# Acellera/moleculekit

Hardware: AMD Instinct MI355X
Metric: Mvoxel-channels/s (64^3 grid, 8 ch) (higher is better)
Workload: dtype f32; 1 GPU; cfg2: BASELINE.json configs[1]; channels=8, atoms_per_gpu=12800000, periodic=False, tile_k=0, pipelined_steps=True, topology_reuse=False, device=AMD Radeon Graphics, arch=gfx950:sramecc+:xnack-, compute_units=256

## Files before the change

### include/mkamd_voxel.h

```cpp
#ifndef MKAMD_VOXEL_H
#define MKAMD_VOXEL_H

#include <stddef.h>
#include <stdint.h>

#ifdef __cplusplus
extern "C" {
#endif

#define MKAMD_OK 0
#define MKAMD_EINVAL 1
#define MKAMD_EHIP 2
#define MKAMD_ENODEV 3
#define MKAMD_EOVERFLOW 4
#define MKAMD_EBOX 5
#define MKAMD_ENOMEM 6

typedef struct mkamd_ctx mkamd_ctx;

const char* mkamd_version(void);
const char* mkamd_last_error(void);
int mkamd_device_count(int* count);

int mkamd_ctx_create(int device, mkamd_ctx** ctx);
// ... 2 lines not shown
int mkamd_ctx_abandon_pending(mkamd_ctx* ctx);
int mkamd_ctx_synchronize(mkamd_ctx* ctx);
int mkamd_ctx_poll_errors(mkamd_ctx* ctx);
int mkamd_ctx_device_info(mkamd_ctx* ctx, char* name, size_t len, int* compute_units,
                          uint64_t* hbm_bytes, char* arch, size_t arch_len);
int mkamd_ctx_set_tile_k(mkamd_ctx* ctx, int k);
int mkamd_ctx_set_force_general(mkamd_ctx* ctx, int on);
int mkamd_ctx_set_lds_tier(mkamd_ctx* ctx, int tier);
int mkamd_ctx_set_prepass_mode(mkamd_ctx* ctx, int mode);
int mkamd_ctx_set_fine_cells(mkamd_ctx* ctx, int on);
int mkamd_ctx_set_direct_binning(mkamd_ctx* ctx, int mode);
int mkamd_ctx_set_value_tolerance(mkamd_ctx* ctx, double eps);
int mkamd_ctx_set_tile_team(mkamd_ctx* ctx, int mode);
int mkamd_ctx_set_tile_items(mkamd_ctx* ctx, int mode);
int mkamd_ctx_set_exact_redo(mkamd_ctx* ctx, int mode);
int mkamd_ctx_set_pipelining(mkamd_ctx* ctx, int on);
int mkamd_ctx_promise_inputs(mkamd_ctx* ctx, void* hip_event);
int mkamd_ctx_withdraw_promise(mkamd_ctx* ctx);
int mkamd_ctx_pipelined_calls(mkamd_ctx* ctx, int64_t* n);
int mkamd_ctx_last_tile_kernel(mkamd_ctx* ctx, char* name, size_t name_cap);
int mkamd_ctx_enable_kernel_timing(mkamd_ctx* ctx, int enable);
int mkamd_ctx_read_kernel_timing(mkamd_ctx* ctx, double* total_ms, int64_t* launches);
int mkamd_clock_probe_dev(mkamd_ctx* ctx, void* hip_stream, int64_t microseconds, uint64_t* d_ticks2);

int mkamd_calculate_occupancy(mkamd_ctx* ctx, const double* centers, int64_t n_centers,
                              const float* coords, int64_t n_atoms, const double* sigmas,
                              int32_t n_channels, double* results);

int mkamd_calculate_occupancy_cpu(const double* centers, int64_t n_centers, const float* coords, int64_t n_atoms,
                                  const double* sigmas, int32_t n_channels, double* results);
int mkamd_calculate_occupancy_cpu_threads(const double* centers, int64_t n_centers, const float* coords, int64_t n_atoms,
                                          const double* sigmas, int32_t n_channels, double* results, int32_t n_threads);

int mkamd_occupancy_centers_host(mkamd_ctx* ctx, const double* centers, int64_t n_centers,
                                 const float* coords, int64_t n_atoms, const void* sigmas,
                                 int sigmas_are_f64, int32_t n_channels, const double* box,
                                 float* features);
int mkamd_occupancy_centers_dev(mkamd_ctx* ctx, const double* d_centers, int64_t n_centers,
                                const float* d_coords, int64_t n_atoms, const void* d_sigmas,
                                int sigmas_are_f64, int32_t n_channels, const double* box_host,
                                float* d_features);

int mkamd_voxelize_lattice_host(mkamd_ctx* ctx, int32_t n_items, const float* coords,
                                const int64_t* atom_offsets, const void* sigmas,
                                int sigmas_are_f64, int32_t n_channels, const double* origins,
                                const int32_t* nvoxels, double voxelsize, const float* box,
                                int32_t max_images_per_atom, float* features);
int mkamd_voxelize_lattice_host_f64(mkamd_ctx* ctx, int32_t n_items, const float* coords,
                                    const int64_t* atom_offsets, const void* sigmas,
                                    int sigmas_are_f64, int32_t n_channels, const double* origins,
                                    const int32_t* nvoxels, double voxelsize, const float* box,
                                    int32_t max_images_per_atom, double* features);
int mkamd_voxelize_lattice_host_begin(mkamd_ctx* ctx, int32_t n_items, const float* coords,
                                      const int64_t* atom_offsets, const void* sigmas,
                                      int sigmas_are_f64, int32_t n_channels, const double* origins,
                                      const int32_t* nvoxels, double voxelsize, const float* box,
                                      int32_t max_images_per_atom);
int mkamd_voxelize_lattice_host_end(mkamd_ctx* ctx, float* features, double* features_f64, uint64_t n_values);
int mkamd_voxelize_lattice_dev(mkamd_ctx* ctx, int32_t n_items, const float* d_coords,
                               const int64_t* d_atom_offsets, int64_t total_atoms,
                               const void* d_sigmas, int sigmas_are_f64, int32_t n_channels,
                               const double* d_origins, const int32_t* nvoxels, double voxelsize,
                               const float* d_box, int32_t max_images_per_atom,
                               float* d_features);

int mkamd_voxelize_lattice_aug_dev(mkamd_ctx* ctx, int32_t n_items, const float* d_coords,
                                   const int64_t* d_atom_offsets, int64_t total_atoms,
                                   const void* d_sigmas, int sigmas_are_f64, int32_t n_channels,
                                   const double* d_origins, const int32_t* nvoxels, double voxelsize,
                                   const float* d_box, int32_t max_images_per_atom,
                                   const double* d_affine, float* d_features);

typedef struct mkamd_topology mkamd_topology;
int mkamd_topology_create_dev(mkamd_ctx* ctx, const void* d_sigmas, int sigmas_are_f64, int64_t n_atoms, int32_t n_channels,
                              double voxelsize, mkamd_topology** topology);
int mkamd_topology_create_host(mkamd_ctx* ctx, const void* sigmas, int sigmas_are_f64, int64_t n_atoms, int32_t n_channels,
                               double voxelsize, mkamd_topology** topology);
int mkamd_topology_destroy(mkamd_ctx* ctx, mkamd_topology* topology);
int mkamd_topology_info(const mkamd_topology* topology, int64_t* n_atoms, int32_t* n_channels, double* voxelsize, int32_t* has_wide_sigmas);
int mkamd_voxelize_lattice_topo_dev(mkamd_ctx* ctx, int32_t n_items, const float* d_coords, const int64_t* d_atom_offsets,
                                    int64_t total_atoms, const mkamd_topology* topology, const double* d_origins,
                                    const int32_t* nvoxels, double voxelsize, const float* d_box, int32_t max_images_per_atom,
                                    const double* d_affine, float* d_features);

int mkamd_grid_centers_host(mkamd_ctx* ctx, const double* bb_min, const int32_t* nvoxels,
                            double voxelsize, double* centers);
int mkamd_grid_centers_dev(mkamd_ctx* ctx, const double* bb_min, const int32_t* nvoxels,
                           double voxelsize, double* d_centers);

int mkamd_prefault(void* buffer, uint64_t bytes);
int mkamd_copy_to_host(mkamd_ctx* ctx, void* host_dst, const void* device_src, uint64_t bytes);
int mkamd_copy_dev(mkamd_ctx* ctx, void* device_dst, const void* device_src, uint64_t bytes);
int mkamd_frames_to_items_dev(mkamd_ctx* ctx, void* hip_stream, const float* d_src, int64_t rows, int64_t src_pitch,
                              int64_t n_frames, float scale, float* d_dst);

int mkamd_lattice_from_centers(const double* centers, int64_t n_centers, double* bb_min, int32_t* nvoxels, double* voxelsize);

#ifdef __cplusplus
}
#endif
#endif
```

### moleculekit_amd/_lib.py

```python
from __future__ import annotations

import ctypes
import os
import threading

import numpy as np

_HERE = os.path.dirname(os.path.abspath(__file__))
LIB_PATH = os.environ.get("MKAMD_LIB", os.path.join(_HERE, "csrc", "libmkamd.so"))

MKAMD_OK, MKAMD_EINVAL, MKAMD_EHIP, MKAMD_ENODEV, MKAMD_EOVERFLOW, MKAMD_EBOX, MKAMD_ENOMEM = range(7)

_c_int, _c_i32, _c_i64, _c_dbl, _vp = ctypes.c_int, ctypes.c_int32, ctypes.c_int64, ctypes.c_double, ctypes.c_void_p

SIGNATURES = {
    "mkamd_version": (ctypes.c_char_p, []),
    "mkamd_last_error": (ctypes.c_char_p, []),
    "mkamd_device_count": (_c_int, [ctypes.POINTER(_c_int)]),
    "mkamd_ctx_create": (_c_int, [_c_int, ctypes.POINTER(_vp)]),
    "mkamd_ctx_destroy": (_c_int, [_vp]),
    "mkamd_ctx_set_stream": (_c_int, [_vp, _vp]),
    "mkamd_ctx_synchronize": (_c_int, [_vp]),
    "mkamd_ctx_abandon_pending": (_c_int, [_vp]),
    "mkamd_ctx_poll_errors": (_c_int, [_vp]),
    "mkamd_ctx_device_info": (_c_int, [_vp, ctypes.c_char_p, ctypes.c_size_t, ctypes.POINTER(_c_int),
                                       ctypes.POINTER(ctypes.c_uint64), ctypes.c_char_p, ctypes.c_size_t]),
    "mkamd_ctx_set_tile_k": (_c_int, [_vp, _c_int]),
    "mkamd_ctx_set_force_general": (_c_int, [_vp, _c_int]),
    "mkamd_xtc_info": (_c_int, [ctypes.c_char_p, ctypes.POINTER(ctypes.c_int64), ctypes.POINTER(ctypes.c_int64)]),
    "mkamd_xtc_read": (_c_int, [ctypes.c_char_p, _vp, ctypes.c_int64, ctypes.c_int64, _vp, _vp, _vp, _vp, ctypes.c_int32]),
    "mkamd_xtc_chunk_desc": (_c_int, [ctypes.c_char_p, _vp, ctypes.c_int64, ctypes.c_int64, _vp, ctypes.POINTER(ctypes.c_int64),
                                      ctypes.POINTER(ctypes.c_int64), _vp, _vp, _vp]),
    "mkamd_xtc_copy_bytes": (_c_int, [ctypes.c_char_p, ctypes.c_int64, ctypes.c_int64, _vp, ctypes.c_int32]),
    "mkamd_xtc_byte_range": (_c_int, [ctypes.c_char_p, _vp, ctypes.c_int64, ctypes.c_int64, ctypes.POINTER(ctypes.c_int64), ctypes.POINTER(ctypes.c_int64)]),
    "mkamd_xtc_chunk_desc_mem": (_c_int, [ctypes.c_char_p, _vp, ctypes.c_int64, ctypes.c_int64, _vp, ctypes.c_int64, ctypes.c_int64, _vp,
                                          ctypes.POINTER(ctypes.c_int64), ctypes.POINTER(ctypes.c_int64), _vp, _vp, _vp]),
    "mkamd_xtc_decode_work_bytes": (ctypes.c_uint64, [ctypes.c_int64, ctypes.c_int64]),
    "mkamd_xtc_decode_dev": (_c_int, [_vp, _vp, _vp, _vp, ctypes.c_int64, ctypes.c_int64, ctypes.c_float, _vp, _vp, _vp, ctypes.c_uint64]),
    "mkamd_ctx_set_lds_tier": (_c_int, [_vp, _c_int]),
    "mkamd_ctx_set_prepass_mode": (_c_int, [_vp, _c_int]),
    "mkamd_ctx_set_pipelining": (_c_int, [_vp, _c_int]),
    "mkamd_ctx_promise_inputs": (_c_int, [_vp, _vp]),
    "mkamd_ctx_withdraw_promise": (_c_int, [_vp]),
    "mkamd_ctx_pipelined_calls": (_c_int, [_vp, ctypes.POINTER(_c_i64)]),
    "mkamd_ctx_last_tile_kernel": (_c_int, [_vp, ctypes.c_char_p, ctypes.c_size_t]),
    "mkamd_clock_probe_dev": (_c_int, [_vp, _vp, _c_i64, _vp]),
    "mkamd_frames_to_items_dev": (_c_int, [_vp, _vp, _vp, _c_i64, _c_i64, _c_i64, ctypes.c_float, _vp]),
    "mkamd_ctx_set_tile_team": (_c_int, [_vp, _c_int]),
    "mkamd_ctx_set_tile_items": (_c_int, [_vp, _c_int]),
    "mkamd_ctx_set_exact_redo": (_c_int, [_vp, _c_int]),
    "mkamd_ctx_set_fine_cells": (_c_int, [_vp, _c_int]),
    "mkamd_ctx_set_value_tolerance": (_c_int, [_vp, ctypes.c_double]),
    "mkamd_ctx_set_direct_binning": (_c_int, [_vp, _c_int]),
    "mkamd_ctx_enable_kernel_timing": (_c_int, [_vp, _c_int]),
    "mkamd_ctx_read_kernel_timing": (_c_int, [_vp, ctypes.POINTER(_c_dbl), ctypes.POINTER(_c_i64)]),
    "mkamd_calculate_occupancy": (_c_int, [_vp, _vp, _c_i64, _vp, _c_i64, _vp, _c_i32, _vp]),
    "mkamd_calculate_occupancy_cpu": (_c_int, [_vp, _c_i64, _vp, _c_i64, _vp, _c_i32, _vp]),
    "mkamd_calculate_occupancy_cpu_threads": (_c_int, [_vp, _c_i64, _vp, _c_i64, _vp, _c_i32, _vp, _c_i32]),
    "mkamd_occupancy_centers_host": (_c_int, [_vp, _vp, _c_i64, _vp, _c_i64, _vp, _c_int, _c_i32, _vp, _vp]),
    "mkamd_occupancy_centers_dev": (_c_int, [_vp, _vp, _c_i64, _vp, _c_i64, _vp, _c_int, _c_i32, _vp, _vp]),
    "mkamd_voxelize_lattice_host": (_c_int, [_vp, _c_i32, _vp, _vp, _vp, _c_int, _c_i32, _vp, _vp, _c_dbl,
                                             _vp, _c_i32, _vp]),
    "mkamd_voxelize_lattice_host_f64": (_c_int, [_vp, _c_i32, _vp, _vp, _vp, _c_int, _c_i32, _vp, _vp, _c_dbl,
                                                 _vp, _c_i32, _vp]),
    "mkamd_voxelize_lattice_host_begin": (_c_int, [_vp, _c_i32, _vp, _vp, _vp, _c_int, _c_i32, _vp, _vp, _c_dbl, _vp, _c_i32]),
    "mkamd_voxelize_lattice_host_end": (_c_int, [_vp, _vp, _vp, ctypes.c_uint64]),
    "mkamd_voxelize_lattice_dev": (_c_int, [_vp, _c_i32, _vp, _vp, _c_i64, _vp, _c_int, _c_i32, _vp, _vp,
                                            _c_dbl, _vp, _c_i32, _vp]),
    "mkamd_voxelize_lattice_aug_dev": (_c_int, [_vp, _c_i32, _vp, _vp, _c_i64, _vp, _c_int, _c_i32, _vp, _vp,
                                                _c_dbl, _vp, _c_i32, _vp, _vp]),
    "mkamd_topology_create_dev": (_c_int, [_vp, _vp, _c_int, _c_i64, _c_i32, _c_dbl, ctypes.POINTER(_vp)]),
    "mkamd_topology_create_host": (_c_int, [_vp, _vp, _c_int, _c_i64, _c_i32, _c_dbl, ctypes.POINTER(_vp)]),
    "mkamd_topology_destroy": (_c_int, [_vp, _vp]),
    "mkamd_topology_info": (_c_int, [_vp, ctypes.POINTER(_c_i64), ctypes.POINTER(_c_i32), ctypes.POINTER(_c_dbl), ctypes.POINTER(_c_i32)]),
    "mkamd_voxelize_lattice_topo_dev": (_c_int, [_vp, _c_i32, _vp, _vp, _c_i64, _vp, _vp, _vp, _c_dbl, _vp, _c_i32, _vp, _vp]),
    "mkamd_grid_centers_host": (_c_int, [_vp, _vp, _vp, _c_dbl, _vp]),
    "mkamd_grid_centers_dev": (_c_int, [_vp, _vp, _vp, _c_dbl, _vp]),
    "mkamd_lattice_from_centers": (_c_int, [_vp, ctypes.c_int64, _vp, _vp, _vp]),
    "mkamd_prefault": (_c_int, [_vp, ctypes.c_uint64]),
    "mkamd_copy_to_host": (_c_int, [_vp, _vp, _vp, ctypes.c_uint64]),
    "mkamd_copy_dev": (_c_int, [_vp, _vp, _vp, ctypes.c_uint64]),
    "mkamd_dist_count_pairs": (_c_i64, [_c_i64, _c_i64, _c_int]),
    "mkamd_dist_trajectory_host": (_c_int, [_vp, _vp, _c_i64, _c_i64, _vp, _vp, _c_i64, _vp, _c_i64, _vp, _c_int, _c_int,
                                            _c_int, _vp]),
    "mkamd_dist_trajectory_dev": (_c_int, [_vp, _vp, _c_i64, _vp, _vp, _c_i64, _vp, _c_i64, _vp, _c_int, _c_int, _c_int, _vp]),
    "mkamd_contacts_trajectory_host": (_c_int, [_vp, _vp, _c_i64, _c_i64, _vp, _vp, _c_i64, _vp, _c_i64, _vp, _c_int, _c_int,
                                                ctypes.c_float, _vp, ctypes.POINTER(_vp)]),
    "mkamd_dist_reduction_host": (_c_int, [_vp, _vp, _c_i64, _c_i64, _vp, _vp, _vp, _c_i64, _vp, _vp, _c_i64, _vp, _vp,
                                           _c_int, _c_int, _c_int, _vp, _c_int, _c_int, _vp]),
    "mkamd_contacts_trajectory_dev": (_c_int, [_vp, _vp, _c_i64, _vp, _vp, _c_i64, _vp, _c_i64, _vp, _c_int, _c_int, ctypes.c_float, _vp,
                                               ctypes.POINTER(_vp)]),
    "mkamd_dist_reduction_dev": (_c_int, [_vp, _vp, _c_i64, _c_i64, _vp, _vp, _vp, _c_i64, _c_i64, _vp, _vp, _c_i64, _vp, _vp,
                                          _c_int, _c_int, _c_int, _vp, _c_int, _c_int, _vp]),
    "mkamd_cdist_dev": (_c_int, [_vp, _vp, _c_i64, _vp, _c_i64, _c_i32, _vp]),
    "mkamd_pdist_dev": (_c_int, [_vp, _vp, _c_i64, _c_i32, _vp]),
    "mkamd_ctx_set_reduction_block": (_c_int, [_vp, _c_int]),
    "mkamd_selftest_sqrt": (_c_int, [_vp, ctypes.POINTER(ctypes.c_uint64), ctypes.POINTER(ctypes.c_uint32)]),
    "mkamd_ctx_set_dist_kernels": (_c_int, [_vp, _c_int]),
    "mkamd_ctx_last_dist_kernel": (_c_int, [_vp, ctypes.c_char_p, ctypes.c_size_t]),
    "mkamd_cdist_host": (_c_int, [_vp, _vp, _c_i64, _vp, _c_i64, _c_i32, _vp]),
    "mkamd_pdist_host": (_c_int, [_vp, _vp, _c_i64, _c_i32, _vp]),
    "mkamd_align_transforms_dev": (_c_int, [_vp, _vp, _c_i64, _c_i64, _vp, _c_i64, _c_i64, _vp, _vp, _c_i64, _vp, _c_i64, _c_i64, _c_int,
                                            _vp, _vp]),
    "mkamd_align_apply_dev": (_c_int, [_vp, _vp, _c_i64, _vp, _c_i64, _vp, _vp]),
    "mkamd_align_rmsd_dev": (_c_int, [_vp, _vp, _c_i64, _c_i64, _vp, _c_i64, _c_i64, _vp, _vp, _c_i64, _vp, _c_i64, _c_i64, _c_int, _vp,
                                      _vp]),
    "mkamd_align_host": (_c_int, [_vp, _vp, _c_i64, _c_i64, _vp, _c_i64, _c_i64, _vp, _vp, _c_i64, _vp, _c_i64, _c_i64, _c_int]),
    "mkamd_sasa_dev": (_c_int, [_vp, _vp, _c_i64, _c_i64, _vp, _c_i32, _vp, _vp, ctypes.c_float, _vp, _c_i64]),
    "mkamd_sasa_host": (_c_int, [_vp, _vp, _c_i64, _c_i64, _vp, _c_i64, _vp, _c_i32, _vp, _vp, ctypes.c_float, _vp, _c_i64]),
    "mkamd_shell_counts_dev": (_c_int, [_vp, _vp, _c_i64, _c_i64, _vp, _vp, _c_i64, _vp, _c_i64, _vp, _c_int, _c_int, _vp, _c_i64, _vp]),
    "mkamd_shell_counts_host": (_c_int, [_vp, _vp, _c_i64, _c_i64, _vp, _vp, _c_i64, _vp, _c_i64, _vp, _c_int, _c_int, _vp, _c_i64, _vp]),
    "mkamd_dihedrals_dev": (_c_int, [_vp, _vp, _c_i64, _c_i64, _vp, _c_i64, _vp, _c_i64, _c_int, _vp]),
    "mkamd_dihedrals_host": (_c_int, [_vp, _vp, _c_i64, _c_i64, _vp, _c_i64, _vp, _c_i64, _c_int, _vp]),
    "mkamd_group_moments_dev": (_c_int, [_vp, _vp, _c_i64, _c_i64, _vp, _vp, _vp, _vp, _c_i64, _c_i64, _c_i64, _c_int, _vp]),
    "mkamd_fluctuation_dev": (_c_int, [_vp, _vp, _c_i64, _c_i64, _vp, _vp, _c_i64, _vp, _c_i64, _c_i64, _vp, _vp]),
    "mkamd_group_moments_host": (_c_int, [_vp, _vp, _c_i64, _c_i64, _vp, _vp, _c_i64, _vp, _vp, _vp, _c_i64, _c_int, _vp]),
    "mkamd_fluctuation_host": (_c_int, [_vp, _vp, _c_i64, _c_i64, _vp, _vp, _c_i64, _vp, _c_i64, _vp, _c_i64, _vp, _vp]),
}

_lib = None
_lock = threading.Lock()


def load() -> ctypes.CDLL:
    global _lib
    with _lock:
        if _lib is None:
            if not os.path.exists(LIB_PATH):
                raise RuntimeError(
                    f"moleculekit_amd: HIP library not found at {LIB_PATH}. Build it with "
                    f"`python -c 'import __graft_entry__ as g; g.build()'` (hipcc --offload-arch=gfx950). "
                    f"There is no CPU fallback.")
            if os.environ.get("MKAMD_NO_TORCH_PRELOAD", "0") != "1":
                try:
                    import torch
                except Exception:
                    pass
            L = ctypes.CDLL(LIB_PATH)
            for name, (res, args) in SIGNATURES.items():
                fn = getattr(L, name)
                fn.restype, fn.argtypes = res, args
            if b"DIAGNOSTICS" in L.mkamd_version() and os.environ.get("MKAMD_ALLOW_DIAGNOSTICS", "0") != "1":
                raise RuntimeError(f"moleculekit_amd: {LIB_PATH} is a DIAGNOSTICS build ({L.mkamd_version().decode()}); "
                                   f"set MKAMD_ALLOW_DIAGNOSTICS=1 to load it for timing experiments")
            _lib = L
    return _lib


_host_lib = None


def load_host() -> ctypes.CDLL:
    global _host_lib
    with _lock:
        if _host_lib is None:
            from . import _build
            L = ctypes.CDLL(_build.build_host())
            for name in ("mkamd_calculate_occupancy_cpu", "mkamd_calculate_occupancy_cpu_threads"):
# ... 135 lines not shown
        _check(load().mkamd_ctx_last_tile_kernel(self._h, buf, 128))
        return buf.value.decode()

    def selftest_sqrt(self):
        n, first = ctypes.c_uint64(0), ctypes.c_uint32(0)
        _check(load().mkamd_selftest_sqrt(self._h, ctypes.byref(n), ctypes.byref(first)))
        return int(n.value), int(first.value)

    def set_dist_kernels(self, avoid_mask: int = 0):
        _check(load().mkamd_ctx_set_dist_kernels(self._h, int(avoid_mask)))

    def set_reduction_block(self, block: int = 0):
        _check(load().mkamd_ctx_set_reduction_block(self._h, int(block)))

    def last_dist_kernel(self) -> str:
        buf = ctypes.create_string_buffer(128)
        _check(load().mkamd_ctx_last_dist_kernel(self._h, buf, 128))
        return buf.value.decode()

    def pipelined_calls(self) -> int:
        n = _c_i64(0)
        _check(load().mkamd_ctx_pipelined_calls(self._h, ctypes.byref(n)))
        return int(n.value)

    def enable_kernel_timing(self, on=True):
        _check(load().mkamd_ctx_enable_kernel_timing(self._h, int(bool(on))))

    def read_kernel_timing(self):
        ms, n = _c_dbl(0.0), _c_i64(0)
        _check(load().mkamd_ctx_read_kernel_timing(self._h, ctypes.byref(ms), ctypes.byref(n)))
        return ms.value, n.value

    def device_info(self):
        name = ctypes.create_string_buffer(256)
        arch = ctypes.create_string_buffer(256)
        cus, mem = _c_int(0), ctypes.c_uint64(0)
        _check(load().mkamd_ctx_device_info(self._h, name, 256, ctypes.byref(cus), ctypes.byref(mem), arch, 256))
        return dict(name=name.value.decode(), arch=arch.value.decode(), compute_units=cus.value,
                    hbm_bytes=int(mem.value))

    def calculate_occupancy(self, centers, coords, sigmas, results):
        V, N, C = centers.shape[0], coords.shape[0], sigmas.shape[1]
        _check(load().mkamd_calculate_occupancy(self._h, _ptr(centers), V, _ptr(coords), N, _ptr(sigmas), C,
                                                _ptr(results)))

    def occupancy_centers_host(self, centers, coords, sigmas, sig_f64, C, box, out):
        _check(load().mkamd_occupancy_centers_host(self._h, _ptr(centers), centers.shape[0], _ptr(coords),
                                                   coords.shape[0], _ptr(sigmas), int(sig_f64), C, _ptr(box),
                                                   _ptr(out)))

    def occupancy_centers_dev(self, d_centers, V, d_coords, N, d_sigmas, sig_f64, C, box_host, d_out):
        _check(load().mkamd_occupancy_centers_dev(self._h, _ptr(d_centers), V, _ptr(d_coords), N, _ptr(d_sigmas),
                                                  int(sig_f64), C, _ptr(box_host), _ptr(d_out)))

    def voxelize_lattice_host(self, B, coords, offsets, sigmas, sig_f64, C, origins, nvox, voxelsize, box,
                              max_images, out):
        fn = load().mkamd_voxelize_lattice_host_f64 if out.dtype == np.float64 else load().mkamd_voxelize_lattice_host
        _check(fn(self._h, B, _ptr(coords), _ptr(offsets), _ptr(sigmas),
                                                  int(sig_f64), C, _ptr(origins), _ptr(nvox), float(voxelsize),
                                                  _ptr(box), int(max_images), _ptr(out)))

    def voxelize_lattice_host_begin(self, B, coords, offsets, sigmas, sig_f64, C, origins, nvox, voxelsize, box, max_images):
        _check(load().mkamd_voxelize_lattice_host_begin(self._h, B, _ptr(coords), _ptr(offsets), _ptr(sigmas), int(sig_f64), C,
                                                        _ptr(origins), _ptr(nvox), float(voxelsize), _ptr(box), int(max_images)))
        self._begun = getattr(self, "_begun", 0) + 1
        return self._begun

    def voxelize_lattice_host_end(self, out):
        if not isinstance(out, np.ndarray) or out.dtype not in (np.float32, np.float64) or not out.flags["C_CONTIGUOUS"]:
            raise ValueError("out must be a C-contiguous float32 or float64 ndarray")
        if out.dtype == np.float64:
            _check(load().mkamd_voxelize_lattice_host_end(self._h, None, _ptr(out), int(out.size)))
        else:
            _check(load().mkamd_voxelize_lattice_host_end(self._h, _ptr(out), None, int(out.size)))

    def voxelize_lattice_dev(self, B, d_coords, d_offsets, total_atoms, d_sigmas, sig_f64, C, d_origins, nvox,
                             voxelsize, d_box, max_images, d_out, d_affine=None):
        _check(load().mkamd_voxelize_lattice_aug_dev(self._h, B, _ptr(d_coords), _ptr(d_offsets), int(total_atoms),
                                                     _ptr(d_sigmas), int(sig_f64), C, _ptr(d_origins), _ptr(nvox),
                                                     float(voxelsize), _ptr(d_box), int(max_images), _ptr(d_affine),
                                                     _ptr(d_out)))

    def voxelize_lattice_topo_dev(self, B, d_coords, d_offsets, total_atoms, topology, d_origins, nvox, voxelsize, d_box, max_images, d_out,
                                  d_affine=None):
        _check(load().mkamd_voxelize_lattice_topo_dev(self._h, B, _ptr(d_coords), _ptr(d_offsets), int(total_atoms), topology._h,
                                                      _ptr(d_origins), _ptr(nvox), float(voxelsize), _ptr(d_box), int(max_images),
                                                      _ptr(d_affine), _ptr(d_out)))

    def grid_centers_host(self, bb_min, nvox, voxelsize, out):
        _check(load().mkamd_grid_centers_host(self._h, _ptr(bb_min), _ptr(nvox), float(voxelsize), _ptr(out)))

    def dist_trajectory_host(self, coords, box, sel1, sel2, chains, selfdist, pbc, squared, out):
        N, _, F = coords.shape
        _check(load().mkamd_dist_trajectory_host(self._h, _ptr(coords), N, F, _ptr(box), _ptr(sel1), sel1.shape[0], _ptr(sel2),
                                                 sel2.shape[0], _ptr(chains), int(selfdist), int(pbc), int(squared), _ptr(out)))

    def dist_trajectory_dev(self, d_coords, F, d_box, d_sel1, n1, d_sel2, n2, d_chains, selfdist, pbc, squared, d_out):
        _check(load().mkamd_dist_trajectory_dev(self._h, _ptr(d_coords), F, _ptr(d_box), _ptr(d_sel1), n1, _ptr(d_sel2), n2,
                                                _ptr(d_chains), int(selfdist), int(pbc), int(squared), _ptr(d_out)))

    def contacts_trajectory_host(self, coords, box, sel1, sel2, chains, selfdist, pbc, threshold):
        N, _, F = coords.shape
        offs = np.zeros(F + 1, dtype=np.int64)
        ptr = _vp(None)
        _check(load().mkamd_contacts_trajectory_host(self._h, _ptr(coords), N, F, _ptr(box), _ptr(sel1), sel1.shape[0], _ptr(sel2),
                                                     sel2.shape[0], _ptr(chains), int(selfdist), int(pbc), float(threshold),
                                                     _ptr(offs), ctypes.byref(ptr)))
        n = int(offs[-1])
        if n == 0 or not ptr.value:
            return offs, np.zeros((0, 2), dtype=np.uint32)
        buf = (ctypes.c_uint32 * (2 * n)).from_address(ptr.value)
        return offs, np.frombuffer(buf, dtype=np.uint32).reshape(n, 2).copy()

    def dist_reduction_host(self, coords, box, g1a, g1o, g2a, g2o, ch1, ch2, selfdist, pairs, pbc, masses, r1, r2, out):
        N, _, F = coords.shape
        _check(load().mkamd_dist_reduction_host(self._h, _ptr(coords), N, F, _ptr(box), _ptr(g1a), _ptr(g1o), g1o.shape[0] - 1,
                                                _ptr(g2a), _ptr(g2o), g2o.shape[0] - 1, _ptr(ch1), _ptr(ch2), int(selfdist),
                                                int(pairs), int(pbc), _ptr(masses), int(r1), int(r2), _ptr(out)))

    def contacts_trajectory_dev(self, d_coords, F, d_box, d_sel1, n1, d_sel2, n2, d_chains, selfdist, pbc, threshold):
        offs = np.zeros(F + 1, dtype=np.int64)
        ptr = _vp(None)
        _check(load().mkamd_contacts_trajectory_dev(self._h, _ptr(d_coords), F, _ptr(d_box), _ptr(d_sel1), n1, _ptr(d_sel2), n2, _ptr(d_chains),
                                                    int(selfdist), int(pbc), float(threshold), _ptr(offs), ctypes.byref(ptr)))
        return offs, int(ptr.value or 0), int(offs[-1])

    def dist_reduction_dev(self, d_coords, N, F, d_box, d_g1a, d_g1o, ng1, n_g1_atoms, d_g2a, d_g2o, ng2, d_ch1, d_ch2, selfdist, pairs, pbc,
                           d_masses, r1, r2, d_out):
        _check(load().mkamd_dist_reduction_dev(self._h, _ptr(d_coords), N, F, _ptr(d_box), _ptr(d_g1a), _ptr(d_g1o), ng1, n_g1_atoms, _ptr(d_g2a),
                                               _ptr(d_g2o), ng2, _ptr(d_ch1), _ptr(d_ch2), int(selfdist), int(pairs), int(pbc), _ptr(d_masses),
                                               int(r1), int(r2), _ptr(d_out)))

    def cdist_dev(self, d_c1, n1, d_c2, n2, dim, d_out):
        _check(load().mkamd_cdist_dev(self._h, _ptr(d_c1), n1, _ptr(d_c2), n2, dim, _ptr(d_out)))

    def pdist_dev(self, d_c, n, dim, d_out):
        _check(load().mkamd_pdist_dev(self._h, _ptr(d_c), n, dim, _ptr(d_out)))

    def cdist_host(self, c1, c2, out):
        _check(load().mkamd_cdist_host(self._h, _ptr(c1), c1.shape[0], _ptr(c2), c2.shape[0], c1.shape[1], _ptr(out)))

    def pdist_host(self, c, out):
        _check(load().mkamd_pdist_host(self._h, _ptr(c), c.shape[0], c.shape[1], _ptr(out)))

    def grid_centers_dev(self, bb_min, nvox, voxelsize, d_out):
        _check(load().mkamd_grid_centers_dev(self._h, _ptr(bb_min), _ptr(nvox), float(voxelsize), _ptr(d_out)))


class Topology:

    def __init__(self, ctx, sigmas, voxelsize):
        self._h = _vp(None)
        self._ctx = ctx
        h = _vp(None)
        if isinstance(sigmas, np.ndarray) or not hasattr(sigmas, "data_ptr"):
            sig = np.ascontiguousarray(sigmas)
            if sig.dtype not in (np.float32, np.float64):
                sig = sig.astype(np.float64)
            if sig.ndim != 2:
                raise ValueError("sigmas must be (natoms, nchannels)")
            _check(load().mkamd_topology_create_host(ctx._h, _ptr(sig), int(sig.dtype == np.float64), int(sig.shape[0]), int(sig.shape[1]),
                                                     float(voxelsize), ctypes.byref(h)))
            self.n_atoms, self.n_channels = int(sig.shape[0]), int(sig.shape[1])
        else:
            import torch
            if not (sigmas.is_cuda and sigmas.dim() == 2 and sigmas.is_contiguous() and sigmas.dtype in (torch.float32, torch.float64)):
                raise ValueError("sigmas must be a contiguous float32 / float64 CUDA tensor (natoms, nchannels)")
            ctx.set_stream(torch.cuda.current_stream(sigmas.device).cuda_stream)
            _check(load().mkamd_topology_create_dev(ctx._h, int(sigmas.data_ptr()), int(sigmas.dtype == torch.float64), int(sigmas.shape[0]),
                                                    int(sigmas.shape[1]), float(voxelsize), ctypes.byref(h)))
            self.n_atoms, self.n_channels = int(sigmas.shape[0]), int(sigmas.shape[1])
        self._h = h
        self.voxelsize = float(voxelsize)

    @property
    def has_wide_sigmas(self) -> bool:
        w = _c_i32(0)
        _check(load().mkamd_topology_info(self._h, None, None, None, ctypes.byref(w)))
        return bool(w.value)

    def close(self):
        if getattr(self, "_h", None) is not None and self._h.value:
            ctx = getattr(self, "_ctx", None)
            alive = ctx is not None and getattr(ctx, "_h", None) is not None and ctx._h.value
            load().mkamd_topology_destroy(ctx._h if alive else None, self._h)
            self._h = _vp(None)

    def __del__(self):
        try:
            self.close()
        except Exception:
            pass


_tls = threading.local()


def default_context(device: int | None = None) -> Context:
    if device is None:
        device = int(os.environ.get("MKAMD_DEVICE", os.environ.get("LOCAL_RANK", "0")))
        n = device_count()
        if n > 0:
            device %= n
    held = getattr(_tls, "contexts", None)
    if held is None or getattr(_tls, "pid", None) != os.getpid():
        if held:
            for c in held.values():
                c._h = _vp(None)
        held = _tls.contexts = {}
        _tls.pid = os.getpid()
    ctx = held.get(int(device))
    if ctx is None:
        ctx = held[int(device)] = Context(device)
    return ctx
```

### moleculekit_amd/batch.py

```python
from __future__ import annotations

import numpy as np

from . import _lib

CUTOFF = 5.0


def pack_items(coords_list, sigmas_list):
    ns = [int(np.asarray(c).shape[0]) for c in coords_list]
    offs = np.zeros(len(ns) + 1, dtype=np.int64)
    offs[1:] = np.cumsum(ns)
    if len(ns) == 0:
        return np.zeros((0, 3), np.float32), np.zeros((0, 1), np.float64), offs
    coords = np.concatenate([np.asarray(c, dtype=np.float32).reshape(-1, 3) for c in coords_list])
    sig = np.concatenate([np.asarray(s) for s in sigmas_list])
    return coords, sig, offs


def max_images_per_atom(box, nvoxels, voxelsize) -> int:
    box = np.asarray(box, dtype=np.float64).reshape(-1, 3)
    if box.size == 0:
        return 1
    if not np.all(box > 2 * CUTOFF):
# ... 41 lines not shown
    if dtype not in (np.dtype(np.float32), np.dtype(np.float64)):
        raise ValueError("dtype must be float32 or float64 (the library writes 4- or 8-byte floats into the result)")
    coords = np.ascontiguousarray(coords, dtype=np.float32).reshape(-1, 3)
    atom_offsets = np.ascontiguousarray(atom_offsets, dtype=np.int64)
    sigmas, sig64 = _sigma_array(sigmas)
    if sigmas.ndim != 2 or sigmas.shape[0] != coords.shape[0]:
        raise ValueError("sigmas must be (natoms, nchannels) matching coords")
    origins = np.ascontiguousarray(origins, dtype=np.float64).reshape(-1, 3)
    B = origins.shape[0]
    if atom_offsets.shape != (B + 1,) or (B >= 0 and atom_offsets[-1] != coords.shape[0]):
        raise ValueError("atom_offsets must have B+1 entries ending at the total atom count")
    nv = np.ascontiguousarray(nvoxels, dtype=np.int32).reshape(3)
    C = int(sigmas.shape[1])
    V = int(nv[0]) * int(nv[1]) * int(nv[2])
    bx = None if box is None else np.ascontiguousarray(box, dtype=np.float32).reshape(B, 3)
    ticket = ctx.voxelize_lattice_host_begin(B, coords, atom_offsets, sigmas, sig64, C, origins, nv, float(voxelsize), bx, 0)
    return _PendingHostCall(ctx, ticket, (B, V, C), dtype, (coords, atom_offsets, sigmas, origins, nv, bx))


def _abandon_host_call(ctx_ref, ticket):
    ctx = ctx_ref()
    if ctx is not None and getattr(ctx, "_begun", None) == ticket:
        try:
            ctx.abandon_pending()
        except Exception:
            pass


class _PendingHostCall:

    def __init__(self, ctx, ticket, shape, dtype, keep):
        import weakref
        self._ctx, self._shape, self._dtype, self._keep = ctx, shape, dtype, keep
        self._finalizer = weakref.finalize(self, _abandon_host_call, weakref.ref(ctx), ticket)

    def __call__(self):
        self._finalizer.detach()
        out = np.empty(self._shape, dtype=self._dtype)
        self._ctx.voxelize_lattice_host_end(out)
        return out

    def abandon(self):
        if self._finalizer.alive:
            self._finalizer()


def occupancy_centers(centers, coords, sigmas, box=None, ctx=None):
    ctx = ctx or _lib.default_context()
    centers = np.ascontiguousarray(centers, dtype=np.float64)
    coords = np.ascontiguousarray(coords, dtype=np.float32)
    sigmas, sig64 = _sigma_array(sigmas)
    if centers.ndim != 2 or centers.shape[1] != 3 or coords.ndim != 2 or coords.shape[1] != 3:
        raise ValueError("centers and coords must be (n, 3)")
    if sigmas.ndim != 2 or sigmas.shape[0] != coords.shape[0]:
        raise ValueError("sigmas must be (natoms, nchannels) matching coords")
    out = np.empty((centers.shape[0], sigmas.shape[1]), dtype=np.float32)
    bx = None if box is None else np.ascontiguousarray(box, dtype=np.float64).reshape(3)
    ctx.occupancy_centers_host(centers, coords, sigmas, sig64, int(sigmas.shape[1]), bx, out)
    return out


def grid_centers(bb_min, nvoxels, voxelsize, ctx=None):
    ctx = ctx or _lib.default_context()
    bb = np.ascontiguousarray(bb_min, dtype=np.float64).reshape(3)
    nv = np.ascontiguousarray(nvoxels, dtype=np.int32).reshape(3)
    out = np.empty((int(np.prod(nv.astype(np.int64))), 3), dtype=np.float64)
    ctx.grid_centers_host(bb, nv, float(voxelsize), out)
    return out


def rotation_affines(rotations, centers):
    from .util import rotationMatrix
    rotations = np.asarray(rotations, dtype=np.float64).reshape(-1, 3)
    centers = np.broadcast_to(np.asarray(centers, dtype=np.float64).reshape(-1, 3), rotations.shape)
    out = np.empty((rotations.shape[0], 12), dtype=np.float64)
    for b, (r, c) in enumerate(zip(rotations, centers)):
        m = rotationMatrix([0, 0, 1], r[2]) @ rotationMatrix([0, 1, 0], r[1]) @ rotationMatrix([1, 0, 0], r[0])
        out[b, :9] = m.ravel()
        out[b, 9:] = c - m @ c
    return out


def voxelize_lattice_torch(coords, atom_offsets, sigmas, origins, nvoxels, voxelsize, box=None,
                           max_images=1, out=None, ctx=None, channel_first=False, affine=None, topology=None):
    import torch

    dev = coords.device
    if dev.type != "cuda":
        raise RuntimeError("voxelize_lattice_torch needs CUDA/HIP tensors (there is no CPU path)")
    dev_index = dev.index if dev.index is not None else torch.cuda.current_device()
    if ctx is not None and ctx.device != dev_index:
        raise ValueError(f"ctx lives on GPU {ctx.device} but the tensors are on cuda:{dev_index} (kernels run on the context's device)")
    ctx = ctx or _lib.default_context(dev_index)
    if (sigmas is None) == (topology is None):
        ctx.withdraw_promise()
        raise ValueError("pass the sigmas or a topology (not both)")
    if not (coords.dtype == torch.float32 and coords.is_contiguous() and atom_offsets.dtype == torch.int64 and atom_offsets.is_contiguous()
            and (sigmas is None or (sigmas.dtype in (torch.float32, torch.float64) and sigmas.is_contiguous() and sigmas.dim() == 2))
            and origins.dtype == torch.float64 and origins.is_contiguous()):
        ctx.withdraw_promise()
        raise AssertionError("voxelize_lattice_torch: coords float32, atom_offsets int64, sigmas float32|float64 [n, C], origins float64, all contiguous")
    B = int(origins.shape[0])
    C = int(sigmas.shape[1]) if topology is None else topology.n_channels
    nv = np.ascontiguousarray(nvoxels, dtype=np.int32).reshape(3)
    V = int(np.prod(nv.astype(np.int64)))
    if out is None:
        out = torch.empty((B, V, C), dtype=torch.float32, device=dev)
    else:
        assert out.dtype == torch.float32 and out.is_contiguous() and out.numel() == B * V * C
    d_box = None
    if box is not None:
        assert box.dtype == torch.float32 and box.is_contiguous()
        d_box = box.data_ptr()
    d_aff = None
    if affine is not None:
        assert affine.dtype == torch.float64 and affine.is_contiguous() and tuple(affine.shape) == (B, 12)
        d_aff = affine.data_ptr()
    try:
        ctx.set_stream(torch.cuda.current_stream(dev).cuda_stream)
        if topology is not None:
            ctx.voxelize_lattice_topo_dev(B, coords.data_ptr(), atom_offsets.data_ptr(), int(coords.shape[0]), topology, origins.data_ptr(), nv,
                                          float(voxelsize), d_box, int(max_images), out.data_ptr(), d_aff)
        else:
            ctx.voxelize_lattice_dev(B, coords.data_ptr(), atom_offsets.data_ptr(), int(coords.shape[0]),
                                     sigmas.data_ptr(), sigmas.dtype == torch.float64, C, origins.data_ptr(), nv,
                                     float(voxelsize), d_box, int(max_images), out.data_ptr(), d_aff)
    except BaseException:
        ctx.withdraw_promise()
        raise
    out = out.view(B, V, C)
    if channel_first:
        return out.view(B, int(nv[0]), int(nv[1]), int(nv[2]), C).permute(0, 4, 1, 2, 3)
    return out


def getVoxelDescriptorsBatch(coords_list, channels_list, centers, boxsize, voxelsize=1, boxes=None, ctx=None):
    boxsize = np.array(boxsize, dtype=np.float64)
    centers = np.asarray(centers, dtype=np.float64).reshape(-1, 3)
    nvoxels = np.ceil(boxsize / voxelsize).astype(int)
    origins = centers - boxsize / 2
    coords, sig, offs = pack_items(coords_list, channels_list)
    feats = voxelize_lattice(coords, offs, sig, origins, nvoxels, voxelsize, box=boxes, ctx=ctx)
    return feats, origins, nvoxels.astype(np.int64)


def voxelizeTrajectory(coords, channels, center, boxsize, voxelsize=1, box=None, frames=None, ctx=None):
    coords = np.asarray(coords)
    if coords.ndim != 3 or coords.shape[1] != 3:
        raise ValueError("coords must be (natoms, 3, nframes)")
    fr = np.arange(coords.shape[2]) if frames is None else np.asarray(frames)
    F = len(fr)
    sig = np.asarray(channels)
    boxsize_a = np.array(boxsize, dtype=np.float64)
    nvoxels = np.ceil(boxsize_a / voxelsize).astype(int)
    origin = np.asarray(center, dtype=np.float64) - boxsize_a / 2
    V, C = int(np.prod(nvoxels.astype(np.int64))), int(sig.shape[1])
    out = np.empty((F, V, C), dtype=np.float32)
    if F == 0 or V == 0:
        return out, origin, nvoxels.astype(np.int64)
    try:
        import torch
    except ImportError:
        return _voxelizeTrajectory_packed(coords, channels, center, boxsize, voxelsize, box=box, frames=frames, ctx=ctx)
    cctx = ctx or _lib.default_context()
    _lib._check(_lib.load().mkamd_prefault(_lib._ptr(out), out.nbytes))
    chunk = int(max(1, min(F, (256 << 20) // max(V * C * 4, 1))))
    pos = 0
    lib = _lib.load()
    for idx, feats in iterVoxelizeTrajectory(coords, sig, center, boxsize, voxelsize, box=box, frames=frames, chunk=chunk,
                                             device=f"cuda:{cctx.device}", ctx=cctx):
        n = len(idx)
        feats = feats.contiguous()
        torch.cuda.current_stream(feats.device).synchronize()
        _lib._check(lib.mkamd_copy_to_host(cctx._h, out[pos:pos + n].ctypes.data, feats.data_ptr(), n * V * C * 4))
        pos += n
    return out, origin, nvoxels.astype(np.int64)


def _voxelizeTrajectory_packed(coords, channels, center, boxsize, voxelsize=1, box=None, frames=None, ctx=None):
    coords = np.asarray(coords, dtype=np.float32)
    if coords.ndim != 3 or coords.shape[1] != 3:
        raise ValueError("coords must be (natoms, 3, nframes)")
    fr = np.arange(coords.shape[2]) if frames is None else np.asarray(frames)
    F, N = len(fr), coords.shape[0]
    packed = np.ascontiguousarray(np.transpose(coords[:, :, fr], (2, 0, 1))).reshape(F * N, 3)
    sig = np.asarray(channels)
    sig_all = np.ascontiguousarray(np.broadcast_to(sig[None], (F,) + sig.shape)).reshape(F * N, sig.shape[1])
    offs = np.arange(F + 1, dtype=np.int64) * N
    boxsize = np.array(boxsize, dtype=np.float64)
    nvoxels = np.ceil(boxsize / voxelsize).astype(int)
    origin = np.asarray(center, dtype=np.float64) - boxsize / 2
    bx = None
    if box is not None:
        bx = np.ascontiguousarray(np.asarray(box, dtype=np.float32)[:, fr].T)
    feats = voxelize_lattice(packed, offs, sig_all, np.broadcast_to(origin, (F, 3)), nvoxels, voxelsize,
                             box=bx, ctx=ctx)
    return feats, origin, nvoxels.astype(np.int64)


def _chunk_images(box3n, nvoxels, voxelsize) -> int:
    return max_images_per_atom(np.ascontiguousarray(np.asarray(box3n).T), nvoxels, voxelsize)


USE_TOPOLOGY = True
_PINNED = {}
# ... 367 lines not shown
```

### moleculekit_amd/csrc/capi.hip

```cpp
#include "../../include/mkamd_voxel.h"
#include "../../include/mkamd_distance.h"
#include "../../include/mkamd_xtc.h"
#include "xtc_reader.h"
#include <atomic>
#include "pipeline.h"
#include "dist_pipeline.h"
#include "align_pipeline.h"
#include "sasa_pipeline.h"
#include "shell_pipeline.h"
#include "dihedral_pipeline.h"
#include "moments_pipeline.h"
#include "host_pack.h"
#include "xtc_gpu.h"
#include "cpu_occupancy.h"

#include <algorithm>
#include <cstring>
#include <string>
#include <utility>
#include <vector>

using namespace mkamd;

static thread_local char g_last_error[512] = "";
// ... 167 lines not shown
    {
        in_pipelined_prepass = false;
        auto await_promise = [&](hipStream_t s) {
            if (!promise_event) return;
            if (!sync_ok(hipStreamWaitEvent(s, promise_event, 0))) (void)hipEventSynchronize(promise_event);
        };
        if (!big_enough || !(pipelining || promise) || !side_stream || pipeline_broken) {
            await_promise(main_stream);
            have_pre_tile_event = false;
            return 0;
        }
        const int set = next_set;
        if (!have_pre_tile_event) {
            if (!sync_ok(hipEventRecord(ev_inputs, main_stream))) { await_promise(main_stream); return 0; }
            inputs_marker = ev_inputs;
        }
        if (!sync_ok(hipStreamWaitEvent(side_stream, inputs_marker, 0))) { await_promise(main_stream); return 0; }
        if (tile_pending[set] && !sync_ok(hipStreamWaitEvent(side_stream, tile_marker[set], 0))) { await_promise(main_stream); return 0; }
        if (promise_event && !sync_ok(hipStreamWaitEvent(side_stream, promise_event, 0))) { (void)hipEventSynchronize(promise_event); return 0; }
        next_set ^= 1;
        stream = side_stream;
        in_pipelined_prepass = true;
        ++n_pipelined;
        return set;
    }
    bool set_is_pipelined(int) const { return in_pipelined_prepass; }
    bool pipelining_possible() const { return (pipelining || promise) && side_stream && !pipeline_broken; }
    void prepass_done(int set)
    {
        if (!in_pipelined_prepass) return;
        stream = main_stream;
        if (sync_ok(hipEventRecord(ev_pre_done[set], side_stream)) && sync_ok(hipStreamWaitEvent(main_stream, ev_pre_done[set], 0)))
            have_pre_tile_event = true;
    }
    void tile_done(int set)
    {
        if (!side_stream) return;
        const bool piped = in_pipelined_prepass;
        in_pipelined_prepass = false;
        if (pipeline_broken || !piped) { last_hot_end = nullptr; return; }
        if (last_hot_end) { tile_marker[set] = last_hot_end; tile_pending[set] = true; }
        else if (sync_ok(hipEventRecord(ev_tile_done[set], main_stream))) { tile_marker[set] = ev_tile_done[set]; tile_pending[set] = true; }
        last_hot_end = nullptr;
    }
    int last_flavour = -1, last_K = 0, last_ecap = 0;
    void hot_begin(int flavour, int K, int ecap)
    {
        last_flavour = flavour; last_K = K; last_ecap = ecap;
        last_hot_end = nullptr;
        if (timing) {
            std::pair<hipEvent_t, hipEvent_t> ev;
            bool ok = true;
            if (!ev_free.empty()) { ev = ev_free.back(); ev_free.pop_back(); }
            else ok = hipEventCreate(&ev.first) == hipSuccess && hipEventCreate(&ev.second) == hipSuccess;
            if (ok && hipEventRecord(ev.first, stream) == hipSuccess) {
                cur0 = ev.first; cur1 = ev.second;
                if (in_pipelined_prepass) inputs_marker = cur0;
                return;
            }
            (void)hipGetLastError();
        }
        if (in_pipelined_prepass) {
            if (sync_ok(hipEventRecord(ev_inputs, main_stream))) inputs_marker = ev_inputs;
        }
    }
    void hot_end()
    {
        if (!timing || !cur0) return;
        if (hipEventRecord(cur1, stream) == hipSuccess) {
            ev_used.emplace_back(cur0, cur1);
            last_hot_end = cur1;
        } else {
            (void)hipGetLastError();
            ev_free.emplace_back(cur0, cur1);
        }
        cur0 = cur1 = nullptr;
    }
};

struct mkamd_topology {
    int device = 0;
    void* mem = nullptr;
    mkamd::TopologyDev dev;
};

static int check_ctx(mkamd_ctx* ctx, bool pending_ok = false)
{
    if (!ctx) return fail(MKAMD_EINVAL, "ctx is NULL");
    if (!pending_ok && ctx->pending.active)
        return fail(MKAMD_EINVAL, "a host call begun on this context (mkamd_voxelize_lattice_host_begin) has not been ended: call _end (or mkamd_ctx_abandon_pending) first");
    HIP_TRY(hipSetDevice(ctx->device));
    ctx->stream = ctx->main_stream;
    return 0;
}

static int collect_async_errors(mkamd_ctx* ctx)
{
    if (!ctx->bufs[WS_ERR]) return 0;
    if (ctx->err_mirrored && ctx->fb_host && ((volatile unsigned*)ctx->fb_host)[NTIER + 1] == 0u) return 0;
    int flag = 0;
    HIP_TRY(hipMemcpy(&flag, ctx->bufs[WS_ERR], sizeof(int), hipMemcpyDeviceToHost));
    if (flag == 0) return 0;
    HIP_TRY(hipMemset(ctx->bufs[WS_ERR], 0, sizeof(int)));
    if (flag & MK_ERR_TOPOLOGY) return fail(MKAMD_EINVAL, "a topology call was given an item that is not the topology's atom count long; results are incomplete");
    if (flag & MK_ERR_BAD_BOX) return fail(MKAMD_EBOX, "periodic box edges must be > 10 A (2 x cutoff)");
    if (flag & MK_ERR_TOO_MANY_IMAGES) return fail(MKAMD_EBOX, "periodic box much smaller than the grid (too many images)");
    return fail(MKAMD_EOVERFLOW, "more periodic images than max_images_per_atom allowed; results are incomplete");
}

static int ensure_err_flag(mkamd_ctx* ctx)
{
    if (ctx->bufs[WS_ERR]) return 0;
    void* p = nullptr;
    int st = ctx->ensure(WS_ERR, sizeof(int), &p);
    if (st) return st;
    HIP_TRY(hipMemsetAsync(p, 0, sizeof(int), ctx->stream));
    return 0;
}

__global__ void k_clock_probe(unsigned long long ref_ticks, unsigned long long* __restrict__ out)
{
    if (threadIdx.x != 0) return;
    const unsigned long long r0 = __builtin_amdgcn_s_memrealtime(), t0 = __builtin_readcyclecounter();
    unsigned long long r;
    unsigned spins = 0u;
    do { __builtin_amdgcn_s_sleep(16); r = __builtin_amdgcn_s_memrealtime(); } while (r - r0 < ref_ticks && ++spins < (1u << 25));
    const unsigned long long t1 = __builtin_readcyclecounter();
    out[0] = t1 - t0;
    out[1] = r - r0;
}


extern "C" {

#ifndef MKAMD_SRC_HASH
#define MKAMD_SRC_HASH "unstamped"
#endif
const char* mkamd_version(void) { return "moleculekit_amd 0.4.0 (gfx950, HIP) src " MKAMD_SRC_HASH MKAMD_BUILD_KIND; }

const char* mkamd_last_error(void) { return g_last_error; }

int mkamd_device_count(int* count)
try {
    if (!count) return fail(MKAMD_EINVAL, "count is NULL");
    *count = 0;
    int n = 0;
    hipError_t e = hipGetDeviceCount(&n);
    if (e != hipSuccess) return hip_fail(e, "hipGetDeviceCount");
    *count = n;
    return MKAMD_OK;
} MK_API_CATCH

int mkamd_ctx_create(int device, mkamd_ctx** out)
try {
    if (!out) return fail(MKAMD_EINVAL, "ctx out-pointer is NULL");
    *out = nullptr;
    int n = 0;
    hipError_t e = hipGetDeviceCount(&n);
    if (e != hipSuccess || n <= 0)
        return fail(MKAMD_ENODEV, std::string("no HIP device available: ") + (e != hipSuccess ? hipGetErrorString(e) : "device count is 0"));
    if (device < 0 || device >= n) return fail(MKAMD_EINVAL, "device index out of range");
    HIP_TRY(hipSetDevice(device));
    mkamd_ctx* c = new mkamd_ctx();
    c->device = device;
    { int cus = 0; if (hipDeviceGetAttribute(&cus, hipDeviceAttributeMultiprocessorCount, device) == hipSuccess && cus > 0) c->n_cus = cus; }
    e = hipStreamCreateWithFlags(&c->own_stream, hipStreamNonBlocking);
    if (e != hipSuccess) { delete c; return hip_fail(e, "hipStreamCreate"); }
    c->stream = c->main_stream = c->own_stream;
    int prio_least = 0, prio_greatest = 0;
    (void)hipDeviceGetStreamPriorityRange(&prio_least, &prio_greatest);
    bool ok = hipStreamCreateWithPriority(&c->side_stream, hipStreamNonBlocking, prio_greatest) == hipSuccess;
    ok = ok && hipEventCreateWithFlags(&c->ev_inputs, hipEventDisableTiming) == hipSuccess;
    for (int i = 0; i < 2 && ok; ++i)
        ok = hipEventCreateWithFlags(&c->ev_pre_done[i], hipEventDisableTiming) == hipSuccess &&
             hipEventCreateWithFlags(&c->ev_tile_done[i], hipEventDisableTiming) == hipSuccess;
    if (!ok) c->side_stream = nullptr;
    if (hipHostMalloc((void**)&c->fb_host, FEEDBACK_WORDS * sizeof(unsigned), hipHostMallocMapped) == hipSuccess) {
        for (int i = 0; i < FEEDBACK_WORDS; ++i) c->fb_host[i] = 0u;
        if (hipHostGetDevicePointer((void**)&c->fb_dev, c->fb_host, 0) != hipSuccess) c->fb_dev = nullptr;
    } else {
        c->fb_host = nullptr;
    }
    if (!c->fb_dev && c->fb_host) { (void)hipHostFree(c->fb_host); c->fb_host = nullptr; }
    *out = c;
    return MKAMD_OK;
} MK_API_CATCH

// ... 351 lines not shown
    if ((st = ctx->ensure(WS_H_COORDS, (size_t)N * 12, &dx))) return st;
    if ((st = ctx->ensure(WS_H_SIGMAS, (size_t)N * C * sz, &ds))) return st;
    if ((st = ctx->ensure(WS_H_OUT, (size_t)V * C * 4, &dout))) return st;
    HIP_TRY(hipMemcpyAsync(dc, centers, (size_t)V * 24, hipMemcpyHostToDevice, ctx->stream));
    if (N > 0) {
        HIP_TRY(hipMemcpyAsync(dx, coords, (size_t)N * 12, hipMemcpyHostToDevice, ctx->stream));
        HIP_TRY(hipMemcpyAsync(ds, sigmas, (size_t)N * C * sz, hipMemcpyHostToDevice, ctx->stream));
    }
    st = mkamd_occupancy_centers_dev(ctx, (const double*)dc, V, (const float*)dx, N, ds, sigmas_are_f64, C, box, (float*)dout);
    if (st) return st;
    prefault_big_result(features, (size_t)V * C * 4);
    HIP_TRY(hipMemcpyAsync(features, dout, (size_t)V * C * 4, hipMemcpyDeviceToHost, ctx->stream));
    HIP_TRY(hipStreamSynchronize(ctx->stream));
    return MKAMD_OK;
} MK_API_CATCH

static int voxelize_lattice_host_begin_impl(mkamd_ctx* ctx, int32_t B, const float* coords, const int64_t* atom_offsets,
                                            const void* sigmas, int sigmas_are_f64, int32_t C, const double* origins,
                                            const int32_t* nvoxels, double voxelsize, const float* box, int32_t max_images);
static int voxelize_lattice_host_end_impl(mkamd_ctx* ctx, float* features, double* features64, double* max_into);

int mkamd_calculate_occupancy(mkamd_ctx* ctx, const double* centers, int64_t V, const float* coords,
                              int64_t N, const double* sigmas, int32_t C, double* results)
try {
    if (V < 0 || N < 0 || C <= 0) return fail(MKAMD_EINVAL, "n_centers/n_atoms must be >= 0 and n_channels > 0");
    if (V == 0 || N == 0) return ctx ? MKAMD_OK : fail(MKAMD_EINVAL, "ctx is NULL");
    if (!results) return fail(MKAMD_EINVAL, "results pointer is NULL");
    int st0 = check_ctx(ctx);
    if (st0) return st0;
    std::vector<float>& tmp = ctx->f32_stage;
    double bb_min[3], vs = 0.0;
    int32_t nv[3];
    const bool is_lattice = mkamd::lattice_from_centers(centers, (long long)V, bb_min, nv, &vs);
    bool lattice_done = false;
    const int st = mkamd::route_calculate_occupancy(is_lattice,
        [&] { const int64_t offs[2] = {0, N};
              const int s1 = voxelize_lattice_host_begin_impl(ctx, 1, coords, offs, sigmas, 1, C, bb_min, nv, vs, nullptr, 0);
              if (s1) return s1;
              lattice_done = true;
              return voxelize_lattice_host_end_impl(ctx, nullptr, nullptr, results); },
        [&] { tmp.resize((size_t)V * C);
              return mkamd_occupancy_centers_host(ctx, centers, V, coords, N, sigmas, 1, C, nullptr, tmp.data()); });
    if (st) return st;
    if (lattice_done) return MKAMD_OK;
    const size_t nvals = (size_t)V * C;
    for (size_t i = 0; i < nvals; ++i) {
        const double v = (double)tmp[i];
        if (v > results[i]) results[i] = v;
    }
    return MKAMD_OK;
} MK_API_CATCH

int mkamd_calculate_occupancy_cpu_threads(const double* centers, int64_t V, const float* coords, int64_t N, const double* sigmas,
                                          int32_t C, double* results, int32_t n_threads)
try {
    if (V < 0 || N < 0 || C <= 0) return fail(MKAMD_EINVAL, "n_centers/n_atoms must be >= 0 and n_channels > 0");
    if (V == 0 || N == 0) return MKAMD_OK;
    if (!centers || !coords || !sigmas || !results) return fail(MKAMD_EINVAL, "centers/coords/sigmas/results pointer is NULL");
    if (N > 0xFFFFFFF0LL) return fail(MKAMD_EINVAL, "more than 2^32 atoms");
    mkamd::cpu::calculate_occupancy(centers, V, coords, N, sigmas, C, results, (int)n_threads);
    return MKAMD_OK;
} MK_API_CATCH

int mkamd_calculate_occupancy_cpu(const double* centers, int64_t V, const float* coords, int64_t N, const double* sigmas,
                                  int32_t C, double* results)
try {
    return mkamd_calculate_occupancy_cpu_threads(centers, V, coords, N, sigmas, C, results, 0);
} MK_API_CATCH

int mkamd_voxelize_lattice_dev(mkamd_ctx* ctx, int32_t B, const float* d_coords,
                               const int64_t* d_atom_offsets, int64_t total_atoms, const void* d_sigmas,
                               int sigmas_are_f64, int32_t C, const double* d_origins,
                               const int32_t* nvoxels, double voxelsize, const float* d_box,
                               int32_t max_images, float* d_features)
try {
    return mkamd_voxelize_lattice_aug_dev(ctx, B, d_coords, d_atom_offsets, total_atoms, d_sigmas, sigmas_are_f64, C,
                                          d_origins, nvoxels, voxelsize, d_box, max_images, nullptr, d_features);
} MK_API_CATCH

static int voxelize_lattice_dev_impl(mkamd_ctx* ctx, int32_t B, const float* d_coords,
                                     const int64_t* d_atom_offsets, int64_t total_atoms, const void* d_sigmas,
                                     int sigmas_are_f64, int32_t C, const double* d_origins,
                                     const int32_t* nvoxels, double voxelsize, const float* d_box,
                                     int32_t max_images, const double* d_affine, float* d_features, const mkamd_topology* topo)
{
    int st = check_ctx(ctx);
    if (st) return st;
    if (!nvoxels) return fail(MKAMD_EINVAL, "nvoxels pointer is NULL");
    if (B > 0 && (!d_atom_offsets || !d_origins || !d_features)) return fail(MKAMD_EINVAL, "atom_offsets/origins/features pointer is NULL");
    if (total_atoms > 0 && (!d_coords || (!d_sigmas && !topo))) return fail(MKAMD_EINVAL, "coords/sigmas pointer is NULL");
    if (topo && topo->device != ctx->device) return fail(MKAMD_EINVAL, "the topology lives on another device than the context");
    if ((st = ensure_err_flag(ctx))) return st;
    LatticeProblem P;
    P.B = B; P.total_atoms = total_atoms; P.C = C; P.sigmas_f64 = sigmas_are_f64;
    P.nvox[0] = nvoxels[0]; P.nvox[1] = nvoxels[1]; P.nvox[2] = nvoxels[2];
    P.voxelsize = voxelsize; P.pbc = d_box ? 1 : 0; P.max_images = d_box ? max_images : 1;
    P.tile_k = ctx->tile_k; P.force_general = ctx->force_general; P.lds_tier = ctx->lds_tier; P.prepass_mode = ctx->prepass_mode; P.tile_team = ctx->tile_team; P.tile_items = ctx->tile_items; P.exact_redo_list = ctx->exact_redo; P.fine_cells = ctx->fine_cells; P.value_tol = ctx->value_tol; P.direct = ctx->direct; P.seq = ctx->seq_next; ctx->seq_next = 0u;
    P.coords = d_coords; P.atom_offsets = (const long long*)d_atom_offsets; P.sigmas = d_sigmas;
    P.origins = d_origins; P.box = d_box; P.affine = d_affine; P.out = d_features;
    P.topo = topo ? &topo->dev : nullptr;
    std::string err;
    st = run_lattice(*ctx, P, err);
    ctx->promise = false; ctx->promise_event = nullptr;
    if (st && !err.empty()) return fail(st, err);
    return st;
}

int mkamd_voxelize_lattice_aug_dev(mkamd_ctx* ctx, int32_t B, const float* d_coords,
                                   const int64_t* d_atom_offsets, int64_t total_atoms, const void* d_sigmas,
                                   int sigmas_are_f64, int32_t C, const double* d_origins,
                                   const int32_t* nvoxels, double voxelsize, const float* d_box,
                                   int32_t max_images, const double* d_affine, float* d_features)
try {
    return voxelize_lattice_dev_impl(ctx, B, d_coords, d_atom_offsets, total_atoms, d_sigmas, sigmas_are_f64, C, d_origins, nvoxels, voxelsize,
                                     d_box, max_images, d_affine, d_features, nullptr);
} MK_API_CATCH

int mkamd_topology_create_dev(mkamd_ctx* ctx, const void* d_sigmas, int sigmas_are_f64, int64_t n_atoms, int32_t C, double voxelsize,
                              mkamd_topology** out)
try {
    if (!out) return fail(MKAMD_EINVAL, "topology out-pointer is NULL");
    *out = nullptr;
    int st = check_ctx(ctx);
    if (st) return st;
    if (n_atoms <= 0 || C <= 0 || !d_sigmas) return fail(MKAMD_EINVAL, "a topology needs n_atoms > 0, n_channels > 0 and the sigmas");
    if (n_atoms > 0x7fffffffLL) return fail(MKAMD_EINVAL, "a topology holds at most 2^31 atoms");
    const int G = ceil_div(C, CHG);
    const size_t a256 = 255, sig_bytes = (size_t)n_atoms * C * (sigmas_are_f64 ? 8 : 4);
    const size_t o_cw = (sig_bytes + a256) & ~a256, o_ids = (o_cw + (size_t)n_atoms * G * sizeof(uint2) + a256) & ~a256,
                 o_tab = (o_ids + (size_t)n_atoms * G * sizeof(unsigned) + a256) & ~a256, o_flags = o_tab + 256, o_wide = o_flags + 256,
                 total = o_wide + (size_t)n_atoms * sizeof(unsigned);
    mkamd_topology* t = new mkamd_topology();
    t->device = ctx->device;
    hipError_t e = hipMalloc(&t->mem, total);
    if (e != hipSuccess) { delete t; return hip_fail(e, "hipMalloc(topology)"); }
    char* m = (char*)t->mem;
    auto drop = [&](int code) { (void)hipStreamSynchronize(ctx->stream); (void)hipFree(t->mem); delete t; return code; };
    if ((e = hipMemcpyAsync(m, d_sigmas, sig_bytes, hipMemcpyDeviceToDevice, ctx->stream)) != hipSuccess) return drop(hip_fail(e, "hipMemcpyAsync(topology sigmas)"));
    if ((e = hipMemsetAsync(m + o_flags, 0, 256, ctx->stream)) != hipSuccess) return drop(hip_fail(e, "hipMemsetAsync(topology flags)"));
    std::string err;
    st = run_topology_build(*ctx, m, sigmas_are_f64, (long long)n_atoms, C, voxelsize, (uint2*)(m + o_cw), (unsigned*)(m + o_ids),
                            (unsigned*)(m + o_tab), (int*)(m + o_flags), (unsigned*)(m + o_wide), err);
    if (st) return drop(err.empty() ? st : fail(st, err));
    unsigned table[CLS_TABLE_WORDS];
    int flags2[2] = {0, 0};
    if ((e = hipMemcpyAsync(table, m + o_tab, sizeof table, hipMemcpyDeviceToHost, ctx->stream)) != hipSuccess ||
        (e = hipMemcpyAsync(flags2, m + o_flags, sizeof flags2, hipMemcpyDeviceToHost, ctx->stream)) != hipSuccess ||
        (e = hipStreamSynchronize(ctx->stream)) != hipSuccess) return drop(hip_fail(e, "topology read-back"));
    const int flags = flags2[0];
    const unsigned n_wide = (unsigned)flags2[1];
    if (n_wide > 1u) {
        std::vector<unsigned> wl(n_wide);
        if ((e = hipMemcpyAsync(wl.data(), m + o_wide, (size_t)n_wide * 4, hipMemcpyDeviceToHost, ctx->stream)) != hipSuccess ||
            (e = hipStreamSynchronize(ctx->stream)) != hipSuccess) return drop(hip_fail(e, "topology read-back (wide atoms)"));
        std::sort(wl.begin(), wl.end());
        if ((e = hipMemcpyAsync(m + o_wide, wl.data(), (size_t)n_wide * 4, hipMemcpyHostToDevice, ctx->stream)) != hipSuccess ||
            (e = hipStreamSynchronize(ctx->stream)) != hipSuccess) return drop(hip_fail(e, "topology write-back (wide atoms)"));
    }
    if (table[CLS_OVERFLOW] != CLS_EMPTY)
        return drop(fail(MKAMD_EINVAL, "more than 15 distinct sigma values: no class ids to reuse (use the plain entry point)"));
    t->dev.n = (long long)n_atoms; t->dev.C = C; t->dev.G = G; t->dev.sigmas_f64 = sigmas_are_f64; t->dev.voxelsize = voxelsize;
    t->dev.sigmas = m; t->dev.cw = (const uint2*)(m + o_cw); t->dev.ids = (const unsigned*)(m + o_ids); t->dev.table = (const unsigned*)(m + o_tab);
    t->dev.overflow = false; t->dev.wide = (flags & 1) != 0;
    t->dev.wide_list = (const unsigned*)(m + o_wide); t->dev.n_wide = n_wide;
    *out = t;
    return MKAMD_OK;
} MK_API_CATCH

int mkamd_topology_create_host(mkamd_ctx* ctx, const void* sigmas, int sigmas_are_f64, int64_t n_atoms, int32_t C, double voxelsize,
                               mkamd_topology** out)
try {
    if (!out) return fail(MKAMD_EINVAL, "topology out-pointer is NULL");
    *out = nullptr;
    int st = check_ctx(ctx);
    if (st) return st;
    if (n_atoms <= 0 || C <= 0 || !sigmas) return fail(MKAMD_EINVAL, "a topology needs n_atoms > 0, n_channels > 0 and the sigmas");
    void* ds = nullptr;
    const size_t bytes = (size_t)n_atoms * C * (sigmas_are_f64 ? 8 : 4);
    if ((st = ctx->ensure(WS_H_SIGMAS, bytes, &ds))) return st;
    HIP_TRY(hipMemcpyAsync(ds, sigmas, bytes, hipMemcpyHostToDevice, ctx->stream));
    return mkamd_topology_create_dev(ctx, ds, sigmas_are_f64, n_atoms, C, voxelsize, out);
} MK_API_CATCH

int mkamd_topology_destroy(mkamd_ctx* ctx, mkamd_topology* topo)
try {
    if (!topo) return MKAMD_OK;
    if (ctx) {
        (void)hipSetDevice(ctx->device);
        if (ctx->side_stream) (void)hipStreamSynchronize(ctx->side_stream);
        (void)hipStreamSynchronize(ctx->main_stream);
    } else {
        (void)hipSetDevice(topo->device);
        (void)hipDeviceSynchronize();
    }
    if (topo->mem) (void)hipFree(topo->mem);
    delete topo;
    return MKAMD_OK;
} MK_API_CATCH

int mkamd_topology_info(const mkamd_topology* topo, int64_t* n_atoms, int32_t* n_channels, double* voxelsize, int32_t* has_wide_sigmas)
try {
    if (!topo) return fail(MKAMD_EINVAL, "topology is NULL");
    if (n_atoms) *n_atoms = (int64_t)topo->dev.n;
    if (n_channels) *n_channels = topo->dev.C;
    if (voxelsize) *voxelsize = topo->dev.voxelsize;
    if (has_wide_sigmas) *has_wide_sigmas = topo->dev.wide ? 1 : 0;
    return MKAMD_OK;
} MK_API_CATCH

int mkamd_voxelize_lattice_topo_dev(mkamd_ctx* ctx, int32_t B, const float* d_coords, const int64_t* d_atom_offsets, int64_t total_atoms,
                                    const mkamd_topology* topo, const double* d_origins, const int32_t* nvoxels, double voxelsize,
                                    const float* d_box, int32_t max_images, const double* d_affine, float* d_features)
try {
    if (!topo) return fail(MKAMD_EINVAL, "topology is NULL");
    return voxelize_lattice_dev_impl(ctx, B, d_coords, d_atom_offsets, total_atoms, nullptr, topo->dev.sigmas_f64, topo->dev.C, d_origins, nvoxels,
                                     voxelsize, d_box, max_images, d_affine, d_features, topo);
} MK_API_CATCH

static hipError_t wait_for_small_call(hipStream_t s, hipEvent_t done = nullptr)
{
    for (int i = 0; i < 2000; ++i) {
        const hipError_t e = done ? hipEventQuery(done) : hipStreamQuery(s);
        if (e != hipErrorNotReady) {
            if (i != 0 && e == hipSuccess) (void)hipGetLastError();
            return e;
        }
    }
    (void)hipGetLastError();
    return done ? hipEventSynchronize(done) : hipStreamSynchronize(s);
}

__attribute__((target("avx2"))) static void widen_avx2(const float* __restrict__ src, double* __restrict__ dst, size_t n)
{
    for (size_t i = 0; i < n; ++i) dst[i] = (double)src[i];
}
__attribute__((target("avx512f"))) static void widen_avx512(const float* __restrict__ src, double* __restrict__ dst, size_t n)
{
    size_t i = 0;
    for (; i + 16 <= n; i += 16) {
        __builtin_prefetch(src + i + 512, 0, 0);
        typedef float v16f __attribute__((vector_size(64), aligned(4)));
        typedef double v8d __attribute__((vector_size(64), aligned(8)));
        typedef float v8f __attribute__((vector_size(32)));
        const v16f v = *(const v16f*)(src + i);
        const v8f lo = __builtin_shufflevector(v, v, 0, 1, 2, 3, 4, 5, 6, 7), hi = __builtin_shufflevector(v, v, 8, 9, 10, 11, 12, 13, 14, 15);
        *(v8d*)(dst + i) = __builtin_convertvector(lo, v8d);
        *(v8d*)(dst + i + 8) = __builtin_convertvector(hi, v8d);
    }
    for (; i < n; ++i) dst[i] = (double)src[i];
}
static void widen(const float* __restrict__ src, double* __restrict__ dst, size_t n)
{
    static const bool avx512 = __builtin_cpu_supports("avx512f") && getenv("MKAMD_NO_AVX512") == nullptr;
    if (avx512) { widen_avx512(src, dst, n); return; }
    static const bool avx2 = __builtin_cpu_supports("avx2");
    if (avx2) { widen_avx2(src, dst, n); return; }
    for (size_t i = 0; i < n; ++i) dst[i] = (double)src[i];
}


static int voxelize_lattice_host_begin_impl(mkamd_ctx* ctx, int32_t B, const float* coords, const int64_t* atom_offsets,
                                            const void* sigmas, int sigmas_are_f64, int32_t C, const double* origins,
                                            const int32_t* nvoxels, double voxelsize, const float* box, int32_t max_images)
{
    int st = check_ctx(ctx, true);
    if (st) return st;
    if (ctx->pending.active) {
        (void)hipStreamSynchronize(ctx->stream);
        ctx->pending.active = false;
    }
    if (B < 0 || C <= 0) return fail(MKAMD_EINVAL, "n_items must be >= 0 and n_channels > 0");
    if (!nvoxels) return fail(MKAMD_EINVAL, "nvoxels pointer is NULL");
    if (nvoxels[0] < 0 || nvoxels[1] < 0 || nvoxels[2] < 0) return fail(MKAMD_EINVAL, "nvoxels must be >= 0");
    const long long V = (long long)nvoxels[0] * nvoxels[1] * nvoxels[2];
    if (B == 0 || V == 0) { ctx->pending = mkamd_ctx::PendingHostCall{}; ctx->pending.active = true; return MKAMD_OK; }
    if (!atom_offsets || !origins) return fail(MKAMD_EINVAL, "atom_offsets/origins pointer is NULL");
    if (atom_offsets[0] != 0) return fail(MKAMD_EINVAL, "atom_offsets[0] must be 0");
    for (int b = 0; b < B; ++b)
        if (atom_offsets[b + 1] < atom_offsets[b]) return fail(MKAMD_EINVAL, "atom_offsets must be non-decreasing");
    const int64_t N = atom_offsets[B];
    if (N > 0 && (!coords || !sigmas)) return fail(MKAMD_EINVAL, "coords/sigmas pointer is NULL");
    if (box && max_images <= 0) {
        std::string err;
        const int nv[3] = {nvoxels[0], nvoxels[1], nvoxels[2]};
        max_images = max_images_from_boxes(box, B, nv, voxelsize, err);
        if (max_images < 0) return fail(MKAMD_EBOX, err);
    }
    const size_t sz = sigmas_are_f64 ? 8 : 4;
    const size_t out_bytes = (size_t)B * (size_t)V * (size_t)C * 4;
    void *dx = nullptr, *ds = nullptr, *doff = nullptr, *dorg = nullptr, *dbox = nullptr, *dout = nullptr;
    constexpr size_t OUT_HOST_BYTES = (size_t)1 << 20;
    bool mapped_out = out_bytes <= OUT_HOST_BYTES;
    if (mapped_out && !ctx->out_host) {
        if (hipHostMalloc(&ctx->out_host, OUT_HOST_BYTES, hipHostMallocMapped) != hipSuccess ||
            hipHostGetDevicePointer(&ctx->out_host_dev, ctx->out_host, 0) != hipSuccess) {
            if (ctx->out_host) (void)hipHostFree(ctx->out_host);
            ctx->out_host = nullptr;
            (void)hipGetLastError();
            mapped_out = false;
// ... 1170 lines not shown
```

### moleculekit_amd/csrc/kernels.h

```cpp
#pragma once
#ifndef MK_DEVICE_API_PROVIDED
#include "mk_device.h"
#endif

#include "mk_affine.h"
#include "mk_diagnostics.h"

namespace mkamd {

constexpr int CHG = 8;
constexpr int NCLS = 15;
constexpr int NSLOT = 16;
constexpr int NBUCKET = CHG * NSLOT;
constexpr int NTIER = 3;
constexpr int ECAP_TIER[NTIER] = {640, 768, 1024};
constexpr int DENSE_WORDS = 1 + NTIER;
constexpr int FEEDBACK_WORDS = NTIER + 4;
constexpr int FB_TILES_DONE = NTIER + 2, FB_TAIL_WROTE = NTIER + 3;
constexpr int TRAV_BATCH = 4;
constexpr int SURV_BATCH = 2;
constexpr int NXR = 3;
constexpr int NBUCKET3 = NBUCKET * NXR;
constexpr unsigned CLS_EMPTY = 0xffffffffu;
constexpr int CLS_OVERFLOW = NCLS;
constexpr int CLS_TABLE_WORDS = NCLS + 1;

struct GridDesc {
    int nx, ny, nz;
    int tnx, tny, tnz, ntiles;
    int K;
    int cs_log2, cs;
    int h;
    int ncx, ncy, ncz, ncell;
    int cstride;
    int cls_per_item;
    int rint;
    int C, G;
    int B;
    int pbc;
    int force_general;
    float R2;
    float R2cull;
    double inv_res;
    double w_scale;
    double Rp;
    long long V;
    unsigned M;
    int img_cap;
    int prepass_hurry;
    double res;
    float w_exact_max;
    float reach_tau;
    int cell_cap;
    unsigned spill_base, spill_cap;
    const unsigned* direct_words;
    int cnt_shift;
    long long topo_n;
    unsigned topo_wide;
};
enum { DIRECT_FAILED = 0, DIRECT_SPILLED = 1, DIRECT_WORDS = 4, DIRECT_HEAD = 32  };
constexpr float REACH_STEP = 0.17f;

MK_DEV float reach_r2(const GridDesc& g, float r2, int packed_cell)
{
    if (g.reach_tau > 0.f) {
        mk_stay_in_branch();
        r2 *= 1.f - REACH_STEP * (float)((unsigned)packed_cell >> 30);
    }
    return r2;
}

MK_DEV bool direct_layout(const GridDesc& g)
{
    return g.direct_words != nullptr && mk_uniform(g.direct_words[DIRECT_FAILED]) == 0u;
}

constexpr float MK_W_MAX = 3.0e38f;
constexpr double CUTOFF2_A = 25.0;
constexpr double CUTOFF_A_KERNEL = 5.0;

enum { MK_ERR_RECORD_OVERFLOW = 1, MK_ERR_BAD_BOX = 2, MK_ERR_TOO_MANY_IMAGES = 4, MK_ERR_TOPOLOGY = 8  };

template <typename SigT>
MK_DEV float sigma_to_w(SigT sigma, double w_scale)
{
    const double s = (double)sigma;
    const float t = (float)(w_scale / (s * s));
    return (s != 0.0 && t == t) ? fminf(t, MK_W_MAX) : mk_inf();
}

constexpr unsigned ATOM_MULTI_SIGMA = 0xffffffffu;

template <typename SigT>
MK_DEV void load_channel_sigmas(const SigT* __restrict__ row, int c0, int C, SigT (&s)[CHG])
{
    struct alignas(16) Vec16 { SigT v[16 / sizeof(SigT)]; };
    constexpr int PER = 16 / (int)sizeof(SigT);
    if (c0 + CHG <= C && (reinterpret_cast<uintptr_t>(row + c0) & (uintptr_t)15) == 0) {
#pragma unroll
        for (int i = 0; i < CHG / PER; ++i) {
            const Vec16 v = reinterpret_cast<const Vec16*>(row + c0)[i];
#pragma unroll
            for (int j = 0; j < PER; ++j) s[i * PER + j] = v.v[j];
        }
    } else {
#pragma unroll
        for (int j = 0; j < CHG; ++j) s[j] = (c0 + j < C) ? row[c0 + j] : (SigT)0;
    }
}

template <typename SigT>
MK_DEV uint2 channel_w_of(const SigT (&s)[CHG], double w_scale, float (&w)[CHG])
{
    SigT s0 = (SigT)0;
#pragma unroll
    for (int j = CHG - 1; j >= 0; --j) s0 = (s[j] != (SigT)0) ? s[j] : s0;
    const float w0 = sigma_to_w(s0, w_scale);
    bool other = false;
    unsigned nib = 0u;
#pragma unroll
    for (int j = 0; j < CHG; ++j) {
        w[j] = (s[j] == s0) ? w0 : mk_inf();
        nib |= (s[j] == s0) ? (1u << (4 * j)) : 0u;
        other |= (s[j] != s0) && (s[j] != (SigT)0);
    }
    if (other) {
#pragma unroll
        for (int j = 0; j < CHG; ++j)
            if ((s[j] != s0) && (s[j] != (SigT)0)) w[j] = sigma_to_w(s[j], w_scale);
    }
    const bool none = !(w0 < mk_inf());
    return make_uint2(none ? CLS_EMPTY : mk_float_bits(w0), other ? ATOM_MULTI_SIGMA : (none ? 0u : nib));
}

template <typename SigT>
MK_DEV uint2 atom_channel_w(const SigT* __restrict__ row, int c0, int C, double w_scale, float (&w)[CHG])
{
    SigT s[CHG];
    load_channel_sigmas(row, c0, C, s);
    return channel_w_of(s, w_scale, w);
}

// ... 85 lines not shown

MK_KERNEL(256) void k_merge_classes(const unsigned* __restrict__ rows, unsigned nrows, unsigned row_words,
                                    unsigned rows_per_block, unsigned* __restrict__ out_sets,
                                    unsigned* __restrict__ cls_table )
{
    mk_wave_priority_high();
    merge_classes_block(rows, nrows, row_words, rows_per_block, out_sets, cls_table, blockIdx.x);
}

constexpr unsigned TMP_UNUSED = 0xffffffffu;

constexpr int WAVE_RANK_ROUNDS = 8;

MK_DEV unsigned wave_rank_in_cell(bool want, unsigned cell, unsigned* __restrict__ cell_count)
{
    const int lane = threadIdx.x & (WAVE - 1);
    const unsigned long long below = (1ull << lane) - 1ull;
    unsigned long long todo = mk_ballot(want);
    int leader_lane = lane;
    unsigned offset = 0u, group = 1u;
    int grouped = 0;
    for (int it = 0; it < WAVE_RANK_ROUNDS && todo != 0ull; ++it) {
        const int l0 = mk_ctz64(todo);
        const unsigned c0 = mk_readlane(cell, l0);
        const unsigned long long m = mk_ballot(want && cell == c0) & todo;
        if ((m >> lane) & 1ull) {
            leader_lane = l0;
            offset = (unsigned)mk_popc64(m & below);
            group = (unsigned)mk_popc64(m);
        }
        todo &= ~m;
        grouped += mk_popc64(m) - 1;
        if (it == 1 && grouped == 0) break;
    }
    unsigned base = 0u;
    if (want && leader_lane == lane) base = mk_atomic_add(&cell_count[cell], group);
    base = mk_shfl(base, leader_lane);
    return base + offset;
}

MK_DEV int item_of_atom(const long long* __restrict__ atom_offsets, int B, long long a, int lo)
{
    int hi = B;
    while (hi - lo > 1) {
        const int mid = (lo + hi) >> 1;
        if (atom_offsets[mid] <= a) lo = mid; else hi = mid;
    }
    return lo;
}

MK_DEV void items_of_block(const long long* __restrict__ atom_offsets, int B, long long total_atoms, long long a_first,
                           long long a_last, int& b_lo, int& b_hi)
{
    if (B == 1) { b_lo = b_hi = 0; return; }
    int b = (int)((float)a_first * ((float)B * mk_rcp((float)(total_atoms > 0 ? total_atoms : 1))));
    b = b < 0 ? 0 : (b > B - 1 ? B - 1 : b);
    const long long o0 = atom_offsets[b], o1 = atom_offsets[b + 1];
    long long next = o1;
    if (o0 <= a_first && a_first < o1) b_lo = b;
    else { b_lo = item_of_atom(atom_offsets, B, a_first, 0); next = atom_offsets[b_lo + 1]; }
    b_hi = a_last < next ? b_lo : item_of_atom(atom_offsets, B, a_last, b_lo);
}

template <typename SigT, int PBC, bool TOPO = false, class RankOne, class RankWave>
MK_DEV void bin_atom(const GridDesc& g, long long a, bool act, int b_lo, int b_hi, const float* __restrict__ coords,
                     const long long* __restrict__ atom_offsets, const SigT* __restrict__ sigmas,
                     const double* __restrict__ origins, const float* __restrict__ box, const double* __restrict__ affine,
                     float4* __restrict__ tmp_pos, uint2* __restrict__ tmp_idx, uint2* __restrict__ tmp_cls,
                     int* __restrict__ err_flag,
                     bool classes, unsigned* s_set, unsigned* s_full, RankOne&& rank_one, RankWave&& rank_wave)
{
    const bool pbc = PBC < 0 ? (g.pbc != 0) : (PBC != 0);
    bool any = false;
    int b = 0;
    if constexpr (TOPO) {
        if (act) {
            int lo = b_lo, hi = b_hi + 1;
            while (hi - lo > 1) {
                const int mid = (lo + hi) >> 1;
                if (atom_offsets[mid] <= a) lo = mid; else hi = mid;
            }
            b = lo;
            const long long first = atom_offsets[b];
            if (atom_offsets[b + 1] - first != g.topo_n) {
                mk_atomic_or(err_flag, MK_ERR_TOPOLOGY);
            } else {
                const unsigned* __restrict__ ids = reinterpret_cast<const unsigned*>(sigmas) + (size_t)(a - first) * g.G;
                unsigned* __restrict__ park_ids = reinterpret_cast<unsigned*>(tmp_cls) + (size_t)a * g.G;
                for (int gq = 0; gq < g.G; ++gq) {
                    const unsigned v = ids[gq];
                    any |= v != 0u;
                    mk_tmp_store(&park_ids[gq], v);
                }
            }
        }
    }
    for (int c0 = 0; !TOPO && c0 < g.C; c0 += CHG) {
        unsigned wb[CHG];
        float w[CHG];
#pragma unroll
        for (int j = 0; j < CHG; ++j) w[j] = mk_inf();
        uint2 cw = make_uint2(CLS_EMPTY, 0u);
        if (act) {
            cw = atom_channel_w(sigmas + (size_t)a * g.C, c0, g.C, g.w_scale, w);
            mk_tmp_store(&tmp_cls[(size_t)a * g.G + (c0 / CHG)], cw);
        }
        const bool multi = cw.y == ATOM_MULTI_SIGMA;
#pragma unroll
        for (int j = 0; j < CHG; ++j) wb[j] = (w[j] < mk_inf()) ? mk_float_bits(w[j]) : CLS_EMPTY;
        any |= cw.x != CLS_EMPTY;
        if (multi) {
#pragma unroll
            for (int j = 0; j < CHG; ++j) any |= wb[j] != CLS_EMPTY;
        }
        if (classes) wave_register_classes(cw.x, multi, wb, s_set, s_full);
    }

    const size_t t0 = (size_t)(act ? a : 0) * (size_t)g.img_cap;
    int used = 0;
    bool drop = !act || !any;
    double p[3] = {0.0, 0.0, 0.0}, Lv[3] = {0.0, 0.0, 0.0};
    int k0[3] = {0, 0, 0}, k1[3] = {0, 0, 0};
    if (!drop) {
        if constexpr (!TOPO) {
            int lo = b_lo, hi = b_hi + 1;
            while (hi - lo > 1) {
                const int mid = (lo + hi) >> 1;
                if (atom_offsets[mid] <= a) lo = mid; else hi = mid;
            }
            b = lo;
        }
        const int nvox[3] = {g.nx, g.ny, g.nz};
        float xyz[3] = {coords[3 * a + 0], coords[3 * a + 1], coords[3 * a + 2]};
        if (affine != nullptr) {
            MK_AFFINE_APPLY(affine + 12 * (size_t)b, xyz);
        }
#pragma unroll
        for (int ax = 0; ax < 3; ++ax) {
            p[ax] = ((double)xyz[ax] - origins[3 * (size_t)b + ax]) * g.inv_res;
            if (pbc) {
                const double L = (double)box[3 * (size_t)b + ax] * g.inv_res;
                if (!(L > 2.0 * (g.Rp - 1e-3))) { mk_atomic_or(err_flag, MK_ERR_BAD_BOX); drop = true; }
                Lv[ax] = L;
                const double invL = (double)mk_rcp((float)L);
                const double n0 = -g.Rp - p[ax], n1 = (double)(nvox[ax] - 1) + g.Rp - p[ax];
                double q0 = n0 * invL, q1 = n1 * invL;
                if (!(fabs(q0 - rint(q0)) > 1e-5 * (1.0 + fabs(q0))) || !(fabs(q1 - rint(q1)) > 1e-5 * (1.0 + fabs(q1)))) { q0 = n0 / L; q1 = n1 / L; }
                const double a0 = ceil(q0);
                const double a1 = floor(q1);
                if (a1 - a0 > 64.0) { mk_atomic_or(err_flag, MK_ERR_TOO_MANY_IMAGES); drop = true; }
                k0[ax] = (int)a0; k1[ax] = (int)a1;
            } else {
                if (p[ax] < -g.Rp || p[ax] > (double)(nvox[ax] - 1) + g.Rp) drop = true;
            }
        }
    }
    const double cmid = 0.5 * (double)(g.cs - 1);
    const int nc[3] = {g.ncx, g.ncy, g.ncz};
    auto locate = [&](const double (&q)[3], int (&pc)[3], float (&rel)[3]) {
        bool inside = true;
#pragma unroll
        for (int ax = 0; ax < 3; ++ax) {
            const int ci = (int)floor(ldexp(q[ax] + 0.5, -g.cs_log2));
            pc[ax] = ci + g.h;
            inside &= (pc[ax] >= 0) && (pc[ax] < nc[ax]);
            rel[ax] = (float)(q[ax] - ((double)ci * (double)g.cs + cmid));
        }
        return inside;
    };
    auto park = [&](const int (&pc)[3], const float (&rel)[3], size_t cell, unsigned rank) {
// ... 1786 lines not shown
    __shared__ unsigned char s_grp[ITEM_ECAP + 2];
    const int nchunk = (g.ntiles + tiles_per_block - 1) / tiles_per_block;
    const int b = (int)blockIdx.x / nchunk, gq = (int)blockIdx.y;
    const int t_begin = ((int)blockIdx.x - b * nchunk) * tiles_per_block;
    const int t_end = t_begin + tiles_per_block < g.ntiles ? t_begin + tiles_per_block : g.ntiles;
    const int tid = (int)threadIdx.x, lane = tid & (WAVE - 1);
    const int wv = (int)mk_uniform((unsigned)(tid >> 6));
    const unsigned* __restrict__ table = cls_table + (g.cls_per_item ? (size_t)b * CLS_TABLE_WORDS : (size_t)0);
    const unsigned table_word = (lane < CLS_TABLE_WORDS) ? table[lane] : CLS_EMPTY;
    const unsigned my_class_w = (lane < NCLS) ? table_word : 0x7f800000u;
    const size_t cbase = (size_t)b * (size_t)g.cstride;
    const unsigned r0 = cell_start[cbase], r1 = cell_start[cbase + (size_t)g.ncell];
    const unsigned* __restrict__ clsp = rec_cls + (size_t)gq * g.M;
    bool fits = !g.force_general && mk_readlane(table_word, CLS_OVERFLOW) == CLS_EMPTY && (r1 - r0) <= (unsigned)ITEM_MAX_RECORDS;
    if (fits) {
        if (tid < NBUCKET) s_cnt[tid] = 0u;
        mk_block_sync();
        for (unsigned r = r0 + (unsigned)tid; r < r1; r += blockDim.x)
            for_each_present_channel(clsp[r], [&](int c, unsigned id) { (void)mk_lds_add(&s_cnt[c * NSLOT + (int)id - 1], 1u); });
        mk_block_sync();
        if (wv == 0) {
            const unsigned c0 = s_cnt[2 * lane], c1 = s_cnt[2 * lane + 1];
            const unsigned p0 = (c0 + 1u) & ~1u, p1 = (c1 + 1u) & ~1u;
            const unsigned incl = wave_scan_inclusive(p0 + p1);
            const unsigned st0 = incl - p0 - p1, st1 = st0 + p0;
            s_gstart[2 * lane] = st0 | (c0 & 1u);
            s_gstart[2 * lane + 1] = st1 | (c1 & 1u);
            s_cnt[2 * lane] = st0; s_cnt[2 * lane + 1] = st1;
            if (lane == WAVE - 1) { s_gstart[NBUCKET] = incl; s_total = incl; }
            const unsigned long long ne0 = mk_ballot(c0 != 0u), ne1 = mk_ballot(c1 != 0u);
            if (lane < CHG) {
                const unsigned e = (unsigned)(ne0 >> (8 * lane)) & 0xffu, o = (unsigned)(ne1 >> (8 * lane)) & 0xffu;
                unsigned bits = 0;
                for (int j = 0; j < 8; ++j) bits |= (((e >> j) & 1u) << (2 * j)) | (((o >> j) & 1u) << (2 * j + 1));
                s_cbits[lane] = bits;
            }
        }
        mk_block_sync();
        fits = s_total <= (unsigned)ITEM_ECAP;
    }
    if (fits) {
        for (int i = tid; i < ITEM_ECAP + 2; i += (int)blockDim.x) s_grp[i] = 0xffu;
        mk_block_sync();
        for (unsigned r = r0 + (unsigned)tid; r < r1; r += blockDim.x) {
            const float4 P = rec_pos[r];
            for_each_present_channel(clsp[r], [&](int c, unsigned id) {
                const unsigned pos = mk_lds_add(&s_cnt[c * NSLOT + (int)id - 1], 1u);
                s_ent[pos] = P;
                s_grp[pos] = (unsigned char)(c * NSLOT + (int)id - 1);
            });
        }
        mk_block_sync();
        const unsigned total = s_total;
        for (int t = t_begin + wv; t < t_end; t += TILE_TEAM)
            voxelize_item_tile<K>(g, b, t, gq, s_ent, total, s_gstart, s_cbits, s_grp, s_cur[wv], my_class_w, s_stage[wv], out);
        return;
    }
    const bool carries_w = g.force_general || mk_readlane(table_word, CLS_OVERFLOW) != CLS_EMPTY;
    for (int t = t_begin + wv; t < t_end; t += TILE_TEAM)
        voxelize_item_tile_unsorted<K>(g, b, t, gq, r0, r1, rec_pos, clsp, rec_w + (size_t)(gq * 2) * g.M, carries_w, table, s_stage[wv], out);
}

constexpr double EXACT_BAND_REL = 8e-6;

constexpr int EXACT_BATCH = 8, EXACT_CH = 4, EXACT_LIST = 2 * WAVE * EXACT_BATCH;
template <bool B> struct ExactFull { static constexpr bool value = B; };
template <typename SigT>
MK_DEV void exact_recompute(const GridDesc& g, int b, int ix, int iy, int iz, unsigned long long chs , int nch,
                            const float* __restrict__ coords,
                            const long long* __restrict__ atom_offsets, const SigT* __restrict__ sigmas,
                            const double* __restrict__ origins, const float* __restrict__ box,
                            const double* __restrict__ affine, float* __restrict__ out, double* s_best, unsigned* s_near ,
                            long long s_lo = 0, long long s_hi = 0x7fffffffffffffffLL ,
                            bool accumulate = false )
{
    const int lane = threadIdx.x & (WAVE - 1);
    const double cx = mk_dadd_rn(mk_dmul_rn((double)ix, g.res), origins[3 * (size_t)b + 0]);
    const double cy = mk_dadd_rn(mk_dmul_rn((double)iy, g.res), origins[3 * (size_t)b + 1]);
    const double cz = mk_dadd_rn(mk_dmul_rn((double)iz, g.res), origins[3 * (size_t)b + 2]);
    double L[3] = {1.0, 1.0, 1.0};
    if (g.pbc) { L[0] = (double)box[3 * (size_t)b]; L[1] = (double)box[3 * (size_t)b + 1]; L[2] = (double)box[3 * (size_t)b + 2]; }
    const long long a_lo = atom_offsets[b], a_end = atom_offsets[b + 1];
    const long long a_hi = a_end - a_lo > s_hi ? a_lo + s_hi : a_end;
    const long long sshift = g.topo_n ? a_lo : 0;
    const float fcx = (float)cx, fcy = (float)cy, fcz = (float)cz;
    const float fL[3] = {(float)L[0], (float)L[1], (float)L[2]};
    const float fiL[3] = {1.0f / fL[0], 1.0f / fL[1], 1.0f / fL[2]};
    double best[EXACT_CH];
#pragma unroll
    for (int k = 0; k < EXACT_CH; ++k) best[k] = 0.0;
    unsigned cnt = 0;
    auto flush = [&]() {
        mk_wave_sync();
        for (unsigned i0 = 0; i0 < cnt; i0 += WAVE) {
            const unsigned i = i0 + (unsigned)lane;
            if (i >= cnt) continue;
            const long long a = a_lo + (long long)s_near[i];
            float xyz[3] = {coords[3 * a + 0], coords[3 * a + 1], coords[3 * a + 2]};
            if (affine != nullptr) {
                MK_AFFINE_APPLY(affine + 12 * (size_t)b, xyz);
            }
            double dx = (double)xyz[0] - cx, dy = (double)xyz[1] - cy, dz = (double)xyz[2] - cz;
            if (g.pbc) {
                dx -= L[0] * round(dx / L[0]);
                dy -= L[1] * round(dy / L[1]);
                dz -= L[2] * round(dz / L[2]);
            }
            const double d2 = dx * dx + dy * dy + dz * dz;
            if (d2 < CUTOFF2_A) {
                const double root = sqrt(d2);
#pragma unroll
                for (int k = 0; k < EXACT_CH; ++k) {
                    if (k >= nch) break;
                    const double sg = (double)sigmas[(size_t)(a - sshift) * g.C + (size_t)((chs >> (16 * k)) & 0xffffull)];
                    if (!(sg != 0.0) || sg != sg) continue;
                    const double x = sg / root;
                    const double x3 = x * x * x;
                    const double val = 1.0 - exp(-(x3 * x3 * x3 * x3));
                    if (val > best[k]) best[k] = val;
                }
            }
        }
        mk_wave_sync();
        cnt = 0;
    };
    auto scan = [&](long long base, auto full_) {
        constexpr bool FULL = decltype(full_)::value;
        float X[EXACT_BATCH], Y[EXACT_BATCH], Z[EXACT_BATCH];
        const float* __restrict__ p0 = coords + 3 * (base + lane);
#pragma unroll
        for (int u = 0; u < EXACT_BATCH; ++u) {
            if constexpr (FULL) {
                X[u] = p0[3 * WAVE * u + 0]; Y[u] = p0[3 * WAVE * u + 1]; Z[u] = p0[3 * WAVE * u + 2];
            } else {
                const long long a = base + (long long)u * WAVE + lane, ai = a < a_hi ? a : a_hi - 1;
                X[u] = coords[3 * ai + 0]; Y[u] = coords[3 * ai + 1]; Z[u] = coords[3 * ai + 2];
            }
        }
#pragma unroll
        for (int u = 0; u < EXACT_BATCH; ++u) {
            const long long a = base + (long long)u * WAVE + lane;
            bool near = FULL || a < a_hi;
            if (affine == nullptr) {
                float fx = X[u] - fcx, fy = Y[u] - fcy, fz = Z[u] - fcz;
                if (g.pbc) { fx -= fL[0] * mk_rint(fx * fiL[0]); fy -= fL[1] * mk_rint(fy * fiL[1]); fz -= fL[2] * mk_rint(fz * fiL[2]); }
                near = near && (fx * fx + fy * fy + fz * fz <= 25.5f);
            }
            const unsigned long long m = mk_ballot(near);
            if (m == 0ull) continue;
            if (near) s_near[cnt + (unsigned)mk_rank_in_mask(m)] = (unsigned)(a - a_lo);
            cnt += (unsigned)mk_popc64(m);
        }
        if (cnt > (unsigned)(EXACT_LIST - WAVE * EXACT_BATCH)) flush();
    };
    long long base = a_lo + s_lo;
    for (; base + (long long)WAVE * EXACT_BATCH <= a_hi; base += (long long)WAVE * EXACT_BATCH) scan(base, ExactFull<true>{});
    for (; base < a_hi; base += (long long)WAVE * EXACT_BATCH) scan(base, ExactFull<false>{});
    flush();
#pragma unroll
    for (int k = 0; k < EXACT_CH; ++k) {
        if (k >= nch) break;
        s_best[lane] = best[k];
        mk_block_sync();
        if (lane == 0) {
            double m = s_best[0];
            for (int j = 1; j < WAVE; ++j) m = s_best[j] > m ? s_best[j] : m;
            const size_t vox = (size_t)b * (size_t)g.V + ((size_t)ix * g.ny + iy) * g.nz + iz;
// ... 34 lines not shown
            Lv[ax] = Lx;
            const double i0 = ceil((-Rb - p[ax]) / Lx), i1 = floor(((double)(nvox[ax] - 1) + Rb - p[ax]) / Lx);
            if (!(i1 - i0 <= 64.0)) skip = true;
            k0[ax] = (int)i0; k1[ax] = (int)i1;
        }
        if (!(p[ax] == p[ax])) skip = true;
    }
    if (skip) return;
    for (int kx = k0[0]; kx <= k1[0]; ++kx)
    for (int ky = k0[1]; ky <= k1[1]; ++ky)
    for (int kz = k0[2]; kz <= k1[2]; ++kz) {
        const double qx = p[0] + kx * Lv[0], qy = p[1] + ky * Lv[1], qz = p[2] + kz * Lv[2];
        const double fx0 = ceil(qx - Rb), fx1 = floor(qx + Rb), fy0 = ceil(qy - Rb), fy1 = floor(qy + Rb);
        const int x_lo = fx0 > 0.0 ? (int)fx0 : 0, x_hi = fx1 < (double)(g.nx - 1) ? (int)fx1 : g.nx - 1;
        const int y_lo = fy0 > 0.0 ? (int)fy0 : 0, y_hi = fy1 < (double)(g.ny - 1) ? (int)fy1 : g.ny - 1;
        if (x_hi < x_lo || y_hi < y_lo) continue;
        const int nyr = y_hi - y_lo + 1, ncol = (x_hi - x_lo + 1) * nyr;
        for (int cb = 0; cb < ncol; cb += WAVE) {
            const int col = cb + lane;
            const int ix = x_lo + (col < ncol ? col / nyr : 0), iy = y_lo + (col < ncol ? col % nyr : 0);
            const double dx = (double)ix - qx, dy = (double)iy - qy, r2 = R2 - dx * dx - dy * dy;
            const double zr = sqrt(r2 > 0.0 ? r2 : 0.0);
            const long long ia = (long long)floor(qz - zr + 0.5), ib = (long long)floor(qz + zr + 0.5);
            for (int s = 0; s < 6; ++s) {
                const long long iz = s < 3 ? ia - 1 + s : ib - 1 + (s - 3);
                const double dz = (double)iz - qz, d2 = dx * dx + dy * dy + dz * dz;
                const bool hit = col < ncol && r2 >= -band && iz >= 0 && iz < (long long)g.nz && (s < 3 || iz > ia + 1) &&
                                 fabs(d2 - R2) <= band;
                unsigned long long hits = mk_ballot(hit);
                while (hits) {
                    const int hl = mk_ctz64(hits);
                    hits &= hits - 1ull;
                    const int vx = (int)mk_readlane((unsigned)ix, hl), vy = (int)mk_readlane((unsigned)iy, hl);
                    const int vz = (int)mk_readlane((unsigned)(int)iz, hl);
                    if (feedback != nullptr && lane == 0) feedback[FB_TAIL_WROTE] = seq;
                    unsigned long long chs = 0ull;
                    int nch = 0;
                    for (int c = 0; c < g.C; ++c) {
                        if (sigma_to_w(sigmas[(size_t)srow * g.C + c], g.w_scale) < wmax) { chs |= (unsigned long long)(c & 0xffff) << (16 * nch); ++nch; }
                        if (nch == EXACT_CH || (c == g.C - 1 && nch)) {
                            bool listed = false;
                            if (redo_list != nullptr) {
                                unsigned slot = 0u;
                                if (lane == 0) slot = mk_atomic_add(&redo_list[REDO_COUNT], 1u);
                                slot = mk_uniform(mk_shfl(slot, 0));
                                if (slot < redo_cap) {
                                    const size_t vox = (size_t)b * (size_t)g.V + ((size_t)vx * g.ny + vy) * g.nz + vz;
                                    if (lane == 0) {
                                        unsigned* e = redo_list + REDO_HEAD + (size_t)slot * REDO_ENTRY;
                                        e[0] = (unsigned)b; e[1] = (unsigned)vx; e[2] = (unsigned)vy; e[3] = (unsigned)vz;
                                        e[4] = (unsigned)(chs & 0xffffffffull); e[5] = (unsigned)(chs >> 32); e[6] = (unsigned)nch; e[7] = 0u;
                                    }
                                    if (lane < nch) out[vox * (size_t)g.C + (size_t)((chs >> (16 * lane)) & 0xffffull)] = 0.f;
                                    listed = true;
                                }
                            }
                            if constexpr (LIST_ONLY) {
                                if (!listed && lane == 0) redo_list[REDO_OVERFLOW] = 1u;
                            } else {
                                if (!listed)
                                    exact_recompute<SigT>(g, b, vx, vy, vz, chs, nch, coords, atom_offsets, sigmas, origins, box, affine, out, s_best, s_near);
                            }
                            chs = 0ull; nch = 0;
                        }
                    }
                }
            }
        }
    }
}

template <typename SigT, int LIST_ONLY = 0>
MK_DEV void exact_fixup_block(const GridDesc& g, const unsigned blk, int per_item, const unsigned* __restrict__ summary,
                              const float* __restrict__ coords, const long long* __restrict__ atom_offsets,
                              long long total_atoms, const SigT* __restrict__ sigmas, const double* __restrict__ origins,
                              const float* __restrict__ box, const double* __restrict__ affine,
                              const uint2* __restrict__ tmp_cls, float* __restrict__ out, double* s_best, unsigned* s_near,
                              unsigned* __restrict__ feedback = nullptr, unsigned seq = 0u,
                              unsigned* __restrict__ redo_list = nullptr, unsigned redo_cap = 0u)
{
    const int lane = threadIdx.x;
    const float wmax = g.w_exact_max;
    auto wide_bits = [&](unsigned bits) { return bits != CLS_EMPTY && mk_uint_as_float(bits) < wmax; };
    if (per_item == 2) {
        const int b = (int)(blk / g.topo_wide);
        const long long k = (long long)summary[blk % g.topo_wide];
        const long long a_lo = atom_offsets[b], a_hi = atom_offsets[b + 1];
        if (a_hi - a_lo != (long long)g.topo_n || k >= (long long)g.topo_n) return;
        exact_fixup_atom<SigT, LIST_ONLY>(g, b, a_lo + k, k, coords, atom_offsets, sigmas, origins, box, affine, out, s_best, s_near, feedback, seq,
                                          redo_list, redo_cap);
        return;
    }
    long long a_lo, a_hi;
    if (per_item) {
        const int b = (int)blk;
        a_lo = atom_offsets[b]; a_hi = atom_offsets[b + 1];
        if (summary != nullptr) {
            const unsigned t = lane < CLS_TABLE_WORDS ? summary[(size_t)b * CLS_TABLE_WORDS + lane] : CLS_EMPTY;
            const bool maybe = lane == CLS_OVERFLOW ? t != CLS_EMPTY : wide_bits(t);
            if (mk_ballot(maybe) == 0ull) return;
        }
    } else {
        a_lo = (long long)blk * 256;
        a_hi = a_lo + 256 < total_atoms ? a_lo + 256 : total_atoms;
        if (summary != nullptr) {
            const unsigned t = lane < CLS_BLOCK_SET ? summary[(size_t)blk * CLS_BLOCK_SET + lane] : CLS_EMPTY;
            if (mk_ballot(t == CLS_TOO_MANY || wide_bits(t)) == 0ull) return;
        }
    }
    int b_hint = per_item ? (int)blk : item_of_atom(atom_offsets, g.B, a_lo, 0);
    for (long long base = a_lo; base < a_hi; base += WAVE) {
        const long long a_mine = base + lane;
        bool wide = false;
        if (a_mine < a_hi) {
            for (int gq = 0; gq < g.G; ++gq) {
                const uint2 cw = tmp_cls[(size_t)a_mine * g.G + gq];
                if (cw.y == ATOM_MULTI_SIGMA) {
                    for (int c = gq * CHG; c < g.C && c < gq * CHG + CHG; ++c)
                        wide |= sigma_to_w(sigmas[(size_t)a_mine * g.C + c], g.w_scale) < wmax;
                } else wide |= wide_bits(cw.x);
            }
        }
        unsigned long long todo = mk_ballot(wide);
        while (todo) {
            const int l = mk_ctz64(todo);
            todo &= todo - 1ull;
            const long long a = base + l;
            const int b = per_item ? (int)blk : item_of_atom(atom_offsets, g.B, a, b_hint);
            b_hint = b;
            exact_fixup_atom<SigT>(g, b, a, a, coords, atom_offsets, sigmas, origins, box, affine, out, s_best, s_near, feedback, seq);
        }
    }
}

template <int K, int ECAP, typename SigT>
MK_KERNEL(64) void k_tail(GridDesc g, unsigned dense_wgs, const unsigned* __restrict__ cell_start,
                          const float4* __restrict__ rec_pos, const unsigned* __restrict__ rec_cls,
                          const unsigned* __restrict__ cls_table, float* __restrict__ out,
                          unsigned* __restrict__ dense_words, unsigned* __restrict__ other_words,
                          const unsigned* __restrict__ dense_list, unsigned* __restrict__ feedback, const int* __restrict__ err_flag,
                          int per_item, const unsigned* __restrict__ summary, const float* __restrict__ coords,
                          const long long* __restrict__ atom_offsets, long long total_atoms, const SigT* __restrict__ sigmas,
                          const double* __restrict__ origins, const float* __restrict__ box, const double* __restrict__ affine,
                          const uint2* __restrict__ tmp_cls,
                          unsigned* __restrict__ solo_counts , unsigned solo_n,
                          unsigned* __restrict__ solo_table, unsigned seq ,
                          unsigned fix_jobs )
{
    __shared__ double s_best[WAVE];
    __shared__ unsigned s_near[EXACT_LIST];
    const unsigned n = dense_words[0], total_tiles = (unsigned)g.B * (unsigned)g.ntiles;
    if (blockIdx.x == 0) {
        if (threadIdx.x <= (unsigned)DENSE_WORDS + 1u) other_words[threadIdx.x] = 0u;
        if (feedback && threadIdx.x == 0) {
            mk_threadfence_system();
            if (n != 0u) feedback[FB_TAIL_WROTE] = seq;
            feedback[FB_TILES_DONE] = seq;
#pragma unroll
            for (int t = 0; t < NTIER; ++t) feedback[t] = dense_words[1 + t];
            feedback[NTIER] = total_tiles * (unsigned)g.G;
            feedback[NTIER + 1] = (unsigned)*err_flag;
        }
    }
    unsigned role = blockIdx.x;
    if (n != 0u) {
        if (threadIdx.x == 0) role = mk_atomic_add(&dense_words[DENSE_WORDS + 1], 1u);
        role = mk_uniform(mk_shfl(role, 0));
    }
    if (role < dense_wgs) {
        for (unsigned i = role; i < n; i += dense_wgs) {
            const unsigned e = dense_list[i];
            voxelize_tile<K, true, ECAP>(g, e % total_tiles, (int)(e / total_tiles), cell_start, rec_pos, nullptr, rec_cls, cls_table, out, nullptr, nullptr);
            mk_block_sync();
        }
        if (n != 0u) {
            mk_threadfence();
            mk_block_sync();
            if (threadIdx.x == 0) (void)mk_atomic_add(&dense_words[DENSE_WORDS], 1u);
        }
        return;
    }
    if (n != 0u) {
        if (threadIdx.x == 0)
            while (mk_load_relaxed(&dense_words[DENSE_WORDS]) < dense_wgs) mk_sleep();
        mk_block_sync();
        mk_threadfence();
    }
    if (solo_counts != nullptr) {
        const unsigned me = role - dense_wgs, nfix = gridDim.x - dense_wgs;
        for (unsigned i = me * WAVE + threadIdx.x; i < solo_n; i += nfix * WAVE) solo_counts[i] = 0u;
        const unsigned overflow_word = cls_table[CLS_OVERFLOW];
        mk_wave_sync();
        if (me == 0u && threadIdx.x < (unsigned)CLS_TABLE_WORDS && overflow_word != CLS_EMPTY) solo_table[threadIdx.x] = CLS_EMPTY;
    }
    for (unsigned job = role - dense_wgs; job < fix_jobs; job += gridDim.x - dense_wgs)
        exact_fixup_block<SigT>(g, job, per_item, summary, coords, atom_offsets, total_atoms, sigmas, origins, box, affine,
                                tmp_cls, out, s_best, s_near, feedback, seq);
}

template <typename SigT>
MK_KERNEL(64) void k_exact_redo(GridDesc g, unsigned* __restrict__ redo_list, unsigned redo_cap, const float* __restrict__ coords,
                                const long long* __restrict__ atom_offsets, const SigT* __restrict__ sigmas,
                                const double* __restrict__ origins, const float* __restrict__ box, const double* __restrict__ affine,
                                float* __restrict__ out)
{
    __shared__ double s_best[WAVE];
    __shared__ unsigned s_near[EXACT_LIST];
    unsigned count = redo_list[REDO_COUNT];
    count = count < redo_cap ? count : redo_cap;
    const unsigned slices = (unsigned)((g.topo_n + REDO_SLICE - 1) / REDO_SLICE);
    const unsigned long long jobs = (unsigned long long)count * slices;
    for (unsigned long long job = blockIdx.x; job < jobs; job += gridDim.x) {
        const unsigned* e = redo_list + REDO_HEAD + (size_t)(job / slices) * REDO_ENTRY;
        const long long s_lo = (long long)(job % slices) * REDO_SLICE;
        const unsigned long long chs = (unsigned long long)e[4] | ((unsigned long long)e[5] << 32);
        exact_recompute<SigT>(g, (int)e[0], (int)e[1], (int)e[2], (int)e[3], chs, (int)e[6], coords, atom_offsets, sigmas, origins, box, affine, out,
                              s_best, s_near, s_lo, s_lo + REDO_SLICE, true);
    }
}

template <typename SigT, bool INPLACE>
MK_KERNEL(64) void k_exact_shells(GridDesc g, unsigned fix_jobs, const unsigned* __restrict__ summary, const float* __restrict__ coords,
                                  const long long* __restrict__ atom_offsets, long long total_atoms, const SigT* __restrict__ sigmas,
                                  const double* __restrict__ origins, const float* __restrict__ box, const double* __restrict__ affine,
                                  const uint2* __restrict__ tmp_cls, float* __restrict__ out, unsigned* __restrict__ redo_list, unsigned redo_cap)
{
    __shared__ double s_best[WAVE];
    __shared__ unsigned s_near[EXACT_LIST];
    if constexpr (INPLACE) {
        if (redo_list[REDO_OVERFLOW] == 0u) return;
        for (unsigned job = blockIdx.x; job < fix_jobs; job += gridDim.x)
            exact_fixup_block<SigT, 0>(g, job, 2, summary, coords, atom_offsets, total_atoms, sigmas, origins, box, affine, tmp_cls, out, s_best, s_near);
    } else {
        for (unsigned job = blockIdx.x; job < fix_jobs; job += gridDim.x)
            exact_fixup_block<SigT, 1>(g, job, 2, summary, coords, atom_offsets, total_atoms, sigmas, origins, box, affine, tmp_cls, out, s_best, s_near,
                                       nullptr, 0u, redo_list, redo_cap);
    }
}

MK_KERNEL(64) void k_zero_words(unsigned* __restrict__ p, unsigned n)
{
    for (unsigned i = threadIdx.x; i < n; i += blockDim.x) p[i] = 0u;
}

constexpr int EXPL_CENTERS = 64;
constexpr int EXPL_MAX_WAVES = 16;

MK_KERNEL(EXPL_MAX_WAVES * WAVE) void k_occupancy_centers(const double* __restrict__ centers, long long V,
                                                 const float* __restrict__ coords, long long N,
                                                 const float4* __restrict__ w ,
                                                 int C, int use_box, double bx, double by, double bz,
                                                 float* __restrict__ out)
{
    __shared__ float4 s_pos[EXPL_MAX_WAVES * WAVE];
    __shared__ float4 s_w0[EXPL_MAX_WAVES * WAVE];
    __shared__ float4 s_w1[EXPL_MAX_WAVES * WAVE];
    __shared__ unsigned s_q[CHG][EXPL_CENTERS];
    const int gq = blockIdx.y;
    const int nth = (int)blockDim.x, tid = (int)threadIdx.x, lane = tid & (WAVE - 1), wv = tid >> 6;
    const long long v0 = (long long)blockIdx.x * EXPL_CENTERS, v = v0 + lane;
    const bool active = v < V;
    double cx = 0, cy = 0, cz = 0;
    if (active) { cx = centers[3 * v]; cy = centers[3 * v + 1]; cz = centers[3 * v + 2]; }
    const float INF = mk_inf();
    unsigned q[CHG];
#pragma unroll
    for (int c = 0; c < CHG; ++c) q[c] = 0x7f800000u;
    for (int i = tid; i < CHG * EXPL_CENTERS; i += nth) s_q[i / EXPL_CENTERS][i % EXPL_CENTERS] = 0x7f800000u;
    mk_block_sync();

    for (long long a0 = 0; a0 < N; a0 += nth) {
        const long long a = a0 + tid;
        if (a < N) {
            s_pos[tid] = make_float4(coords[3 * a], coords[3 * a + 1], coords[3 * a + 2], 0.f);
            s_w0[tid] = w[(size_t)(gq * 2 + 0) * N + a];
            s_w1[tid] = w[(size_t)(gq * 2 + 1) * N + a];
        }
        mk_block_sync();
        const long long left = N - a0 - (long long)wv * WAVE;
        const int cnt = left < 0 ? 0 : (left < WAVE ? (int)left : WAVE);
        for (int k = 0; k < cnt; ++k) {
            const int i = wv * WAVE + k;
            const float4 p = s_pos[i];
            double dx = (double)p.x - cx, dy = (double)p.y - cy, dz = (double)p.z - cz;
            if (use_box) {
                dx -= bx * round(dx / bx);
                dy -= by * round(dy / by);
                dz -= bz * round(dz / bz);
            }
            const double d2 = dx * dx + dy * dy + dz * dz;
            const bool in = d2 < 25.0;
            const float d2f = (float)d2;
            const float4 w0 = s_w0[i], w1 = s_w1[i];
            const float wc[CHG] = {w0.x, w0.y, w0.z, w0.w, w1.x, w1.y, w1.z, w1.w};
#pragma unroll
            for (int c = 0; c < CHG; ++c)
                q[c] = mk_min_bits(q[c], in ? d2f * wc[c] : INF);
// ... 69 lines not shown
```

### moleculekit_amd/csrc/pipeline.h

```cpp
#pragma once
#include "kernels.h"

#include <algorithm>
#include <cmath>
#include <cstdio>
#include <string>
#include <cstdlib>
#include <type_traits>

namespace mkamd {

constexpr int SOLO_CNT_SHIFT = 3;

enum Status { ST_OK = 0, ST_EINVAL = 1, ST_EHIP = 2, ST_ENODEV = 3, ST_EOVERFLOW = 4, ST_EBOX = 5 };

enum WsSlot {
    WS_CELL_COUNT = 0, WS_CELL_START, WS_SCAN_CHUNKS, WS_REC_POS, WS_REC_W, WS_REC_CLS, WS_CLS_TABLE, WS_CLS_BLOCKS, WS_CLS_L1, WS_TMP_POS, WS_TMP_IDX, WS_TMP_CLS, WS_DENSE_LIST, WS_ERR, WS_W_EXPLICIT, WS_DENSE_WORDS, WS_DIRECT_COUNT, WS_REDO_LIST,
    WS_H_COORDS, WS_H_SIGMAS, WS_H_OFFSETS, WS_H_ORIGINS, WS_H_BOX, WS_H_OUT, WS_H_CENTERS, WS_H_STAGE,
    WS_D_PA, WS_D_PB, WS_D_WRAP, WS_D_COM1, WS_D_COM2, WS_D_SEL1, WS_D_SEL2, WS_D_CHAINS, WS_D_CHAINS2, WS_D_G1A, WS_D_G1O,
    WS_D_G2A, WS_D_G2O, WS_D_MASS, WS_D_CNT, WS_D_TOT, WS_D_BASE, WS_D_CONTACTS, WS_D_MASK,
    WS_A_REFPART, WS_A_PART, WS_A_RPART, WS_A_FOLD, WS_A_REFFOLD, WS_A_SLAB, WS_A_XYZ, WS_A_REF, WS_A_SEL, WS_A_REFSEL, WS_A_FRAMES, WS_A_AFFINE,
    WS_S_POINTS, WS_S_PACK, WS_S_AREA, WS_S_ERR, WS_S_SLAB, WS_S_XYZ, WS_S_RADII, WS_S_MAP, WS_S_MASK, WS_S_OUT,
    WS_M_PART, WS_M_REF, WS_M_ATOMS, WS_M_OFFS, WS_M_W, WS_M_REFIN,
    WS_NSLOTS
};

constexpr double CUTOFF_A = 5.0;

struct TopologyDev {
    long long n = 0;
    int C = 0, G = 0, sigmas_f64 = 0;
    double voxelsize = 0.0;
    const unsigned* ids = nullptr;
    const uint2* cw = nullptr;
    const void* sigmas = nullptr;
    const unsigned* table = nullptr;
    bool overflow = false;
    bool wide = false;
    const unsigned* wide_list = nullptr;
    unsigned n_wide = 0;
};

struct LatticeProblem {
    int B = 0;
    long long total_atoms = 0;
    int C = 0;
    int sigmas_f64 = 0;
    int nvox[3] = {0, 0, 0};
    double voxelsize = 1.0;
    int pbc = 0;
    int max_images = 1;
    int tile_k = 0;
    int force_general = 0;
    int lds_tier = -1;
    int prepass_mode = -1;
    int fine_cells = 0;
    double value_tol = 0.0;
    int direct = -1;
    int cell_cap = 0;
    unsigned spill_cap = 0;
    unsigned seq = 0;
    int tile_team = -1;
    int tile_items = -1;
    int exact_redo_list = 0;
    const float* coords = nullptr;
    const long long* atom_offsets = nullptr;
    const void* sigmas = nullptr;
    const double* origins = nullptr;
    const float* box = nullptr;
    const double* affine = nullptr;
    float* out = nullptr;
    const TopologyDev* topo = nullptr;
};

inline int ceil_div(long long a, long long b) { return (int)((a + b - 1) / b); }

inline int plan_lattice(const LatticeProblem& P, GridDesc& g, std::string& err)
{
    char buf[256];
    if (P.B < 0 || P.total_atoms < 0 || P.C <= 0) { err = "n_items/total_atoms must be >= 0 and n_channels > 0"; return ST_EINVAL; }
    if (!(P.voxelsize > 0.0) || !std::isfinite(P.voxelsize)) { err = "voxelsize must be a positive finite number"; return ST_EINVAL; }
    for (int ax = 0; ax < 3; ++ax)
        if (P.nvox[ax] < 0) { err = "nvoxels must be >= 0"; return ST_EINVAL; }
    g = GridDesc{};
    g.nx = P.nvox[0]; g.ny = P.nvox[1]; g.nz = P.nvox[2];
    g.V = (long long)g.nx * g.ny * g.nz;
    g.C = P.C; g.G = ceil_div(P.C, CHG);
    g.B = P.B; g.pbc = P.pbc ? 1 : 0; g.force_general = P.force_general ? 1 : 0;
    g.inv_res = 1.0 / P.voxelsize;
    g.w_scale = P.voxelsize * P.voxelsize;
    const double R = CUTOFF_A / P.voxelsize;
    g.R2 = (float)(R * R);
    g.R2cull = (float)(R * R * 1.0002 + 1e-3);
    g.res = P.voxelsize;
    g.w_exact_max = (float)(7.647 / (R * R));
    g.cell_cap = 0; g.spill_base = 0u; g.spill_cap = 0u; g.direct_words = nullptr; g.cnt_shift = 0;
    g.reach_tau = (P.value_tol > 0.0) ? (float)std::pow(std::min(P.value_tol, 1e-5), -1.0 / 6.0) : 0.f;
    g.Rp = R + 1e-3;
    g.rint = (int)std::ceil(R);
    if (g.rint > 512) { err = "voxelsize too small (cutoff spans > 512 voxels)"; return ST_EINVAL; }
    g.cs_log2 = 3;
    while ((1 << g.cs_log2) < g.rint && g.cs_log2 < 9) ++g.cs_log2;
    if (g.cs_log2 > 2 && P.fine_cells) --g.cs_log2;
    g.cs = 1 << g.cs_log2;
    g.h = ceil_div((long long)g.rint + 1, g.cs);
    g.ncx = ceil_div(g.nx, g.cs) + 2 * g.h;
    g.ncy = ceil_div(g.ny, g.cs) + 2 * g.h;
    g.ncz = ceil_div(g.nz, g.cs) + 2 * g.h;
    if (g.ncx > 1023 || g.ncy > 1023 || g.ncz > 1023) { err = "grid too large (more than 1023 cells per axis)"; return ST_EINVAL; }
    const long long ncell = (long long)g.ncx * g.ncy * g.ncz;
    if ((ncell + 1) * (long long)(P.B > 0 ? P.B : 1) > 0xFFFF0000LL) {
        snprintf(buf, sizeof buf, "batch too large: %lld cells x %d items exceeds 2^32; split the batch", ncell, P.B);
        err = buf; return ST_EINVAL;
    }
    g.ncell = (int)ncell;
    g.cstride = (int)ncell + 1;
    g.cls_per_item = 0;
    g.prepass_hurry = 1;

    int K = P.tile_k;
    if (K != 4 && K != 8) {
        const long long pad8 = (long long)ceil_div(g.nx, 8) * 8, pad4 = (long long)ceil_div(g.nx, 4) * 4;
        const long long tiles8 = (long long)ceil_div(g.nx, 8) * ceil_div(g.ny, 8) * ceil_div(g.nz, 8) * P.B * g.G;
        K = (pad4 < pad8 || tiles8 < 2048) ? 4 : 8;
    }
    g.K = K;
    g.tnx = ceil_div(g.nx, K); g.tny = ceil_div(g.ny, 8); g.tnz = ceil_div(g.nz, 8);
    const long long ntiles = (long long)g.tnx * g.tny * g.tnz;
    if (ntiles * (long long)(P.B > 0 ? P.B : 1) > 0x7FFFFF00LL) { err = "batch too large: more than 2^31 tiles; split the batch"; return ST_EINVAL; }
    g.ntiles = (int)ntiles;

    long long images = 1;
    if (g.pbc) {
        if (P.max_images < 1) { err = "max_images_per_atom must be >= 1 for periodic items"; return ST_EINVAL; }
        images = P.max_images;
    }
    const long long M = P.total_atoms * images;
    if (M > 0xFFFF0000LL) { err = "batch too large: more than 2^32 atom records; split the batch"; return ST_EINVAL; }
    g.M = (unsigned)(M > 0 ? M : 1);
    g.img_cap = (int)images;
    return ST_OK;
}

inline int max_images_from_boxes(const float* box, int B, const int* nvox, double voxelsize, std::string& err)
{
    long long worst = 1;
    for (int b = 0; b < B; ++b) {
        long long m = 1;
        for (int ax = 0; ax < 3; ++ax) {
            const double L = (double)box[3 * b + ax];
            if (!(L > 2.0 * CUTOFF_A)) { err = "periodic box edges must be > 10 A (2 x cutoff)"; return -1; }
            const double span = (double)(nvox[ax] > 0 ? nvox[ax] - 1 : 0) * voxelsize + 2.0 * CUTOFF_A + 2e-3 * voxelsize;
            m *= (long long)std::floor(span / L) + 1;
        }
        if (m > worst) worst = m;
    }
    if (worst > 4096) { err = "periodic box much smaller than the grid (more than 4096 images per atom)"; return -1; }
    return (int)worst;
}

template <class BE>
int run_scan(BE& be, unsigned* counts , size_t n, unsigned* starts , int set = 0)
{
    const size_t nchunks = (n + 1 + SCAN_CHUNK - 1) / SCAN_CHUNK;
    void* chunks = nullptr;
    int st = be.ensure(WS_SCAN_CHUNKS, nchunks * sizeof(unsigned), &chunks, set);
    if (st) return st;
    if ((st = be.launch(k_scan_chunk_sums, dim3((unsigned)nchunks), dim3(SCAN_THREADS), (const unsigned*)counts, n, (unsigned*)chunks))) return st;
    if ((st = be.launch(k_scan_sums_inplace, dim3(1), dim3(SCAN_THREADS), (unsigned*)chunks, (unsigned)nchunks))) return st;
    return be.launch(k_scan_finish, dim3((unsigned)nchunks), dim3(SCAN_THREADS), counts, n, (const unsigned*)chunks, starts, (const unsigned*)nullptr);
}

inline int choose_tier(int forced, const volatile unsigned* feedback)
{
    if (forced >= 0) return forced < NTIER ? forced : NTIER - 1;
    if (!feedback) return 0;
    const unsigned tiles = feedback[NTIER];
    if (tiles == 0) return 0;
    int tier = 0;
    while (tier < NTIER - 1 && (unsigned long long)feedback[tier] * 20ull > tiles) ++tier;
    return tier;
}

enum TileFlavour { TILES_PLAIN = 0, TILES_LEAN = 1, TILES_TEAM = 2, TILES_ITEMS = 3 };

constexpr unsigned REDO_BLOCKS = 4096;
constexpr unsigned SHELL_BLOCKS = 16384;
constexpr unsigned REDO_CAP = 32768;
constexpr unsigned CLS_ROWS_PER_BLOCK = 128;
constexpr long long PIPELINE_MIN_ATOMS = 200000;

template <class Ptr> using sigma_of = std::remove_const_t<std::remove_pointer_t<Ptr>>;
template <class F>
inline int with_sigmas(const void* sigmas, int f64, F&& launch) { return f64 ? launch((const double*)sigmas) : launch((const float*)sigmas); }

struct CounterState { void* ptr = nullptr; size_t clean = 0; void* wptr = nullptr; bool wclean = false; unsigned parity = 0;
                      void* dptr = nullptr; size_t dclean = 0; void* tptr = nullptr; };
constexpr int DENSE_SET_WORDS = DENSE_WORDS + 2;

struct LatticePath {
    enum PrePass { PRE_CHAIN, PRE_CHAIN_TOPO, PRE_ITEMS, PRE_SOLO } prepass = PRE_CHAIN;
    bool pipelined_wanted = false;
    bool team = false;
    bool ligand_items = false;
    bool direct_geom = false;
    int direct_cap = 128; unsigned spill = 0; unsigned long long direct_slots = 0;
    int team_waves = TILE_TEAM;
    unsigned fix_jobs = 0, fix_waves = 0, dense_wgs = 0;
    bool split_exact_fixup = false;
    unsigned redo_cap = REDO_CAP;
    bool direct_layout = false;
    bool direct_first = false;
    bool small_scan = false;
    int flavour = TILES_PLAIN;

    bool topo() const { return prepass == PRE_CHAIN_TOPO; }
    bool solo() const { return prepass == PRE_SOLO; }
    bool per_item() const { return prepass == PRE_ITEMS; }
};

inline LatticePath choose_lattice_path(const LatticeProblem& P, const GridDesc& g, bool pipelining_possible)
{
    LatticePath L;
    const bool topo = P.topo != nullptr;
    const long long B = g.B;
    const bool big = P.total_atoms >= PIPELINE_MIN_ATOMS;
    const bool chain_pays = pipelining_possible && big && P.total_atoms > 1024LL * B;
    const unsigned long long tile_waves = (unsigned long long)g.B * (unsigned)g.ntiles * (unsigned)g.G;
    L.team = P.tile_team > 0 || (P.tile_team < 0 && tile_waves <= 1024ull);
    if (g.K == 4) L.team_waves = (P.tile_team == 8 || P.tile_team == 16) ? P.tile_team : (P.tile_team != 4 && tile_waves <= 256ull) ? 8 : TILE_TEAM;
    auto span = [&](int width) {
        int best = 0;
        for (int x0 = 0; x0 < std::max(g.cs, width); x0 += width)
            best = std::max(best, ((x0 + width - 1 + g.rint) >> g.cs_log2) - ((x0 - g.rint) >> g.cs_log2) + 1);
        return best;
    };
    static const int env_cap = [] { const char* e = std::getenv("MKAMD_CELL_CAP"); return e ? std::atoi(e) : 0; }();
    L.direct_cap = P.cell_cap > 0 ? P.cell_cap : (env_cap > 0 ? env_cap : 128);
    L.direct_geom = !g.pbc && g.G == 1 && !g.force_general && P.total_atoms > 0 && L.direct_cap <= (1 << SURV_OFF_BITS) &&
                    span(g.K) * span(8) * span(8) <= WAVE - 1;
    L.ligand_items = P.tile_items != 0 && P.total_atoms <= 96LL * B && g.ntiles <= 512;
    const bool hist_fits = g.ncell + 1 <= ITEM_HIST;
    const bool solo = !topo && L.direct_geom && (unsigned long long)P.total_atoms * (unsigned)g.B <= (1ull << 22) &&
                      (P.direct == 2 || (P.direct != 0 && P.prepass_mode < 0 && L.team && !(L.ligand_items && P.tile_team <= 0 && hist_fits)));
    const bool per_item = !topo && !solo && hist_fits && P.prepass_mode != 0 &&
                          (P.prepass_mode == 1 || (P.total_atoms <= 4096LL * B && !chain_pays));
    L.prepass = topo ? LatticePath::PRE_CHAIN_TOPO : solo ? LatticePath::PRE_SOLO : per_item ? LatticePath::PRE_ITEMS : LatticePath::PRE_CHAIN;
    L.pipelined_wanted = big && !per_item && !solo;
    L.spill = solo ? (unsigned)P.total_atoms : P.spill_cap > 0 ? P.spill_cap : (unsigned)std::max<long long>(1024, P.total_atoms / (8LL * B));
    L.direct_slots = (unsigned long long)((size_t)g.B * (size_t)g.cstride) * (unsigned)L.direct_cap + (unsigned long long)L.spill * (unsigned)g.B;
    L.fix_jobs = topo ? (unsigned)(B * P.topo->n_wide) : per_item ? (unsigned)g.B : P.total_atoms > 0 ? (unsigned)ceil_div(P.total_atoms, 256) : 0u;
    L.fix_waves = L.fix_jobs < 8192u ? L.fix_jobs : 8192u;
    L.dense_wgs = g.force_general ? 0u : (unsigned)(tile_waves < 4096ull ? tile_waves : 4096ull);
    L.split_exact_fixup = topo && P.topo->n_wide != 0u && P.seq == 0u && !g.force_general && P.exact_redo_list >= 0;
    L.redo_cap = P.exact_redo_list > 0 && (unsigned)P.exact_redo_list < REDO_CAP ? (unsigned)P.exact_redo_list : REDO_CAP;
    return L;
}

inline void settle_lattice_path(LatticePath& L, const LatticeProblem& P, GridDesc& g, bool set_is_pipelined)
{
    g.prepass_hurry = !(set_is_pipelined && !g.pbc && (double)g.B * (double)g.V >= 4.0 * (double)P.total_atoms) ? 1 : 0;
    const bool direct_big = L.prepass == LatticePath::PRE_CHAIN && L.direct_geom &&
                            (P.direct == 1 || (P.direct < 0 && !set_is_pipelined && P.total_atoms >= PIPELINE_MIN_ATOMS));
    L.direct_layout = (L.solo() || direct_big) && L.direct_slots <= 0xFFFF0000ull;
    L.direct_first = L.direct_layout && !L.solo();
    L.small_scan = !L.direct_layout && (size_t)g.B * (size_t)g.cstride <= SMALL_PREPASS_MAX_CELLS &&
                   (unsigned)ceil_div(P.total_atoms > 0 ? P.total_atoms : 1, 256) <= SMALL_PREPASS_MAX_BLOCKS;
    L.flavour = L.team ? TILES_TEAM : (set_is_pipelined ? TILES_LEAN : TILES_PLAIN);
    if (P.tile_items > 0 ? !L.team : (L.ligand_items && P.tile_team <= 0 && L.per_item())) L.flavour = TILES_ITEMS;
}

struct LatticeWorkspace {
    size_t ncells = 0, count_bytes = 0, direct_bytes = 0;
    unsigned *dense_count = nullptr, *dense_other = nullptr;
    unsigned *cell_count = nullptr, *cell_start = nullptr, *direct_count = nullptr, *rec_cls = nullptr, *cls_table = nullptr;
    float4 *rec_pos = nullptr, *rec_w = nullptr, *tmp_pos = nullptr;
    uint2 *tmp_idx = nullptr, *tmp_cls = nullptr;
    int* err_flag = nullptr;
    unsigned *cls_blocks = nullptr, *cls_l1 = nullptr;
    unsigned *dense_list = nullptr, *redo_list = nullptr;
    CounterState* cs = nullptr; size_t clean_after = 0; void* table_before = nullptr;
};

template <class T, class BE>
int ensure_as(BE& be, int slot, size_t bytes, T*& p, int set)
{
    void* v = nullptr;
    const int st = be.ensure(slot, bytes, &v, set);
    return p = static_cast<T*>(v), st;
}

template <class BE>
int acquire_lattice_workspace(BE& be, const LatticeProblem& P, const LatticePath& L, GridDesc& g, int set, LatticeWorkspace& W)
{
    int st;
    const size_t ncells = W.ncells = (size_t)g.B * (size_t)g.cstride;
    W.count_bytes = (ncells * sizeof(unsigned) + 255) & ~(size_t)255;
    unsigned* dwords_all = nullptr;
    if ((st = ensure_as(be, WS_DENSE_WORDS, 2 * DENSE_SET_WORDS * sizeof(unsigned), dwords_all, set))) return st;
    if ((st = ensure_as(be, WS_CELL_COUNT, W.count_bytes, W.cell_count, set))) return st;
    if ((st = ensure_as(be, WS_CELL_START, (ncells + 1) * sizeof(unsigned), W.cell_start, set))) return st;
    size_t mrec = (size_t)g.M;
    CounterState& cs = *(W.cs = &be.counter_state(set));
    if (L.direct_layout) {
        g.cell_cap = L.direct_cap; g.spill_base = (unsigned)(ncells * (size_t)L.direct_cap); g.spill_cap = L.spill;
        mrec = std::max<size_t>(mrec, (size_t)L.direct_slots);
        g.cnt_shift = (L.solo() && ncells <= (1u << 16)) ? SOLO_CNT_SHIFT : 0;
        W.direct_bytes = (((size_t)DIRECT_HEAD + (ncells << g.cnt_shift)) * sizeof(unsigned) + 255) & ~(size_t)255;
        if ((st = ensure_as(be, WS_DIRECT_COUNT, W.direct_bytes, W.direct_count, set))) return st;
        if (cs.dptr != W.direct_count) { cs.dptr = W.direct_count; cs.dclean = 0; }
        if (cs.dclean < W.direct_bytes && (st = be.fill(W.direct_count, 0, W.direct_bytes))) return st;
        cs.dclean = 0;
        g.direct_words = W.direct_count;
    }
    if ((st = ensure_as(be, WS_REC_POS, mrec * sizeof(float4), W.rec_pos, set))) return st;
    if ((st = ensure_as(be, WS_REC_W, (L.solo() ? mrec : (size_t)g.M) * sizeof(float4) * 2 * g.G, W.rec_w, set))) return st;
    if ((st = ensure_as(be, WS_REC_CLS, (g.G == 1 ? mrec : (size_t)g.M) * sizeof(unsigned) * g.G, W.rec_cls, set))) return st;
    if ((st = ensure_as(be, WS_CLS_TABLE, (L.per_item() ? (size_t)g.B : (size_t)1) * CLS_TABLE_WORDS * sizeof(unsigned), W.cls_table, set))) return st;
    if ((st = ensure_as(be, WS_ERR, sizeof(int), W.err_flag, 0))) return st;
    if ((st = ensure_as(be, WS_TMP_POS, (size_t)g.M * sizeof(float4), W.tmp_pos, set))) return st;
    if ((st = ensure_as(be, WS_TMP_IDX, (size_t)g.M * sizeof(uint2), W.tmp_idx, set))) return st;
    if ((st = ensure_as(be, WS_TMP_CLS, (size_t)(P.total_atoms > 0 ? P.total_atoms : 1) * g.G * sizeof(uint2), W.tmp_cls, set))) return st;

    if (L.solo()) {
        g.M = (unsigned)mrec;
        if (cs.tptr != W.cls_table && (st = be.fill(W.cls_table, 0xff, CLS_TABLE_WORDS * sizeof(unsigned)))) return st;
    }
    W.table_before = cs.tptr;
    cs.tptr = nullptr;
    if (cs.ptr != W.cell_count) { cs.ptr = W.cell_count; cs.clean = 0; }
    W.clean_after = cs.clean;
    cs.clean = 0;
    if (cs.wptr != dwords_all || !cs.wclean) {
        if ((st = be.fill(dwords_all, 0, 2 * DENSE_SET_WORDS * sizeof(unsigned)))) return st;
        cs.wptr = dwords_all;
    }
    cs.wclean = false;
    W.dense_count = dwords_all + cs.parity * DENSE_SET_WORDS;
    W.dense_other = dwords_all + (cs.parity ^ 1u) * DENSE_SET_WORDS;
    if (L.per_item()) return ST_OK;
    if (W.clean_after < W.count_bytes) {
        if ((st = be.fill(W.cell_count, 0, W.count_bytes))) return st;
        W.clean_after = W.count_bytes;
    }
    const unsigned nblk = (unsigned)ceil_div(P.total_atoms > 0 ? P.total_atoms : 1, 256);
    if ((st = ensure_as(be, WS_CLS_BLOCKS, (size_t)nblk * CLS_BLOCK_SET * sizeof(unsigned), W.cls_blocks, set))) return st;
    return ensure_as(be, WS_CLS_L1, (size_t)ceil_div(nblk, CLS_ROWS_PER_BLOCK) * MERGE_SET * sizeof(unsigned), W.cls_l1, set);
}
// ... 60 lines not shown
                            (unsigned)W.ncells, W.cell_start))) return st;
    } else {
        const size_t nchunks = (W.ncells + 1 + SCAN_CHUNK - 1) / SCAN_CHUNK;
        unsigned* chunks = nullptr;
        if ((st = ensure_as(be, WS_SCAN_CHUNKS, nchunks * sizeof(unsigned), chunks, set))) return st;
        const unsigned nl1_eff = do_classes ? nl1 : 0u;
        if ((st = be.launch(k_prepass_reduce1, dim3(nl1_eff + (unsigned)nchunks), dim3(256), W.cls_blocks, nblk, (unsigned)CLS_ROWS_PER_BLOCK, nl1_eff, W.cls_l1,
                            W.cell_count, W.ncells, chunks, dfail))) return st;
        if ((st = be.launch(k_prepass_reduce2, dim3(do_classes ? 2u : 1u), dim3(256), W.cls_l1, nl1_eff, W.cls_table, chunks, (unsigned)nchunks, dfail))) return st;
        if ((st = be.launch(k_scan_finish, dim3((unsigned)nchunks), dim3(SCAN_THREADS), W.cell_count, W.ncells, chunks, W.cell_start, dfail))) return st;
    }
    if (P.total_atoms <= 0) return ST_OK;
    auto fill = [&](auto kern, auto* sig) {
        return be.launch(kern, fgrid, ablk, g, sig, W.cell_start, W.tmp_pos, W.tmp_idx, W.tmp_cls, W.rec_pos, W.rec_w, W.rec_cls, W.cls_table, nfblk);
    };
    if (topo) return fill(k_bin_fill<float, false, true>, (const float*)nullptr);
    return with_sigmas(P.sigmas, P.sigmas_f64, [&](auto* sig) {
        using S = sigma_of<decltype(sig)>;
        return L.direct_first ? fill(k_bin_fill<S, true>, sig) : fill(k_bin_fill<S>, sig);
    });
}

template <int K, int T, class BE>
int launch_tiles_tier(BE& be, const LatticeProblem& P, const LatticePath& L, const GridDesc& g, const LatticeWorkspace& W)
{
    constexpr int E = ECAP_TIER[T];
    int st;
    const unsigned total_tiles = (unsigned)g.B * (unsigned)g.ntiles;
    auto tiles = [&](auto kern, unsigned waves) {
        return be.launch(kern, dim3(((total_tiles + 7u) / 8u) * 8u, (unsigned)g.G), dim3(WAVE * waves), g, W.cell_start, W.rec_pos, W.rec_w, W.rec_cls,
                         W.cls_table, P.out, W.dense_count, W.dense_list);
    };
    if (L.flavour == TILES_ITEMS) {
        long long nchunk = (1024 + g.B - 1) / g.B;
        const long long max_chunk = (g.ntiles + TILE_TEAM - 1) / TILE_TEAM;
        nchunk = nchunk < 1 ? 1 : (nchunk > max_chunk ? max_chunk : nchunk);
        int tpb = (int)((g.ntiles + nchunk - 1) / nchunk);
        tpb = ((tpb + TILE_TEAM - 1) / TILE_TEAM) * TILE_TEAM;
        const unsigned blocks_per_item = (unsigned)((g.ntiles + tpb - 1) / tpb);
        st = be.launch(k_voxelize_items<K>, dim3((unsigned)g.B * blocks_per_item, (unsigned)g.G), dim3(WAVE * TILE_TEAM), g, W.cell_start, W.rec_pos, W.rec_w,
                       W.rec_cls, W.cls_table, P.out, tpb);
    } else if (L.flavour == TILES_TEAM) {
        if constexpr (K == 4) {
            st = L.team_waves == 16 ? tiles(k_voxelize_tiles_team<K, E, 16>, 16u) : L.team_waves == 8 ? tiles(k_voxelize_tiles_team<K, E, 8>, 8u)
                                                                                                  : tiles(k_voxelize_tiles_team<K, E, TILE_TEAM>, (unsigned)TILE_TEAM);
        } else st = tiles(k_voxelize_tiles_team<K, E, TILE_TEAM>, (unsigned)TILE_TEAM);
    } else if constexpr (T <= 1) {
        st = L.flavour == TILES_LEAN ? tiles(k_voxelize_tiles_lean<K, E>, 1u) : tiles(k_voxelize_tiles<K, E>, 1u);
    } else {
        st = tiles(k_voxelize_tiles<K, E>, 1u);
    }
    if (st || L.dense_wgs + L.fix_waves == 0u) return st;
    const bool split = L.split_exact_fixup;
    const unsigned tail_fix_waves = split ? 1u : L.fix_waves, tail_fix_jobs = split ? 0u : L.fix_jobs;
    const bool topo = L.topo();
    const unsigned* summary = topo ? P.topo->wide_list : g.force_general ? nullptr : L.per_item() ? W.cls_table : W.cls_blocks;
    const uint2* cw = topo ? P.topo->cw : W.tmp_cls;
    return with_sigmas(topo ? P.topo->sigmas : P.sigmas, topo ? P.topo->sigmas_f64 : P.sigmas_f64, [&](auto* sig) {
        using S = sigma_of<decltype(sig)>;
        int s = be.launch(k_tail<K, E, S>, dim3(L.dense_wgs + tail_fix_waves), dim3(WAVE), g, L.dense_wgs, W.cell_start, W.rec_pos, W.rec_cls, W.cls_table, P.out,
                          W.dense_count, W.dense_other, W.dense_list, g.force_general ? (unsigned*)nullptr : be.feedback_dev(), W.err_flag,
                          topo ? 2 : L.per_item() ? 1 : 0, summary, P.coords, P.atom_offsets, P.total_atoms, sig, P.origins, P.box, P.affine, cw,
                          L.solo() ? W.direct_count : nullptr, L.solo() ? (unsigned)(DIRECT_HEAD + (W.ncells << g.cnt_shift)) : 0u, W.cls_table,
                          g.force_general ? 0u : P.seq, tail_fix_jobs);
        if (s || !split) return s;
        auto shells = [&](auto kern, unsigned max_blocks) {
            return be.launch(kern, dim3(L.fix_jobs < max_blocks ? L.fix_jobs : max_blocks), dim3(WAVE), g, L.fix_jobs, summary, P.coords, P.atom_offsets,
                             P.total_atoms, sig, P.origins, P.box, P.affine, cw, P.out, W.redo_list, L.redo_cap);
        };
        if ((s = shells(k_exact_shells<S, false>, SHELL_BLOCKS))) return s;
        if ((s = be.launch(k_exact_redo<S>, dim3(REDO_BLOCKS), dim3(WAVE), g, W.redo_list, L.redo_cap, P.coords, P.atom_offsets, sig, P.origins, P.box,
                           P.affine, P.out))) return s;
        return shells(k_exact_shells<S, true>, 8192u);
    });
}

template <int K, class BE>
int launch_tiles(BE& be, int tier, const LatticeProblem& P, const LatticePath& L, const GridDesc& g, const LatticeWorkspace& W)
{
    return tier == 0 ? launch_tiles_tier<K, 0>(be, P, L, g, W) : tier == 1 ? launch_tiles_tier<K, 1>(be, P, L, g, W) : launch_tiles_tier<K, 2>(be, P, L, g, W);
}

template <class BE>
int run_lattice(BE& be, const LatticeProblem& P, std::string& err)
{
    GridDesc g;
    int st = plan_lattice(P, g, err);
    if (st) return st;
    if (P.B == 0 || g.V == 0) return ST_OK;
    if (const TopologyDev* t = P.topo) {
        if (t->overflow || g.force_general || g.reach_tau > 0.f) {
            err = "a topology call takes the class-sorted path only: not with more than 15 distinct sigmas, force_general or a value tolerance (use the plain entry point)";
            return ST_EINVAL;
        }
        if (t->C != P.C || t->voxelsize != P.voxelsize || t->n <= 0 || P.total_atoms != (long long)P.B * t->n) {
            err = "the topology was built for another channel count / voxel size, or the call is not n_items x its atom count long";
            return ST_EINVAL;
        }
        if ((unsigned long long)g.B * t->n_wide > 0xffffffffull) { err = "too many (item, wide atom) fix-up jobs (>= 2^32): split the batch"; return ST_EINVAL; }
        g.topo_n = t->n; g.topo_wide = t->n_wide;
    }
    LatticePath L = choose_lattice_path(P, g, be.pipelining_possible());
    g.cls_per_item = L.per_item() ? 1 : 0;
    const int set = be.acquire_set(L.pipelined_wanted);
    settle_lattice_path(L, P, g, be.set_is_pipelined(set));
    if (L.solo() && !L.direct_layout) { err = "internal: the one-launch pre-pass does not fit its record slots"; return ST_EINVAL; }

    LatticeWorkspace W;
    if ((st = acquire_lattice_workspace(be, P, L, g, set, W))) return st;
    st = L.per_item() ? prepass_items(be, P, g, W) : L.solo() ? prepass_solo(be, P, g, W) : prepass_chain(be, P, L, g, W, set);
    if (st) return st;
    be.prepass_done(set);

    const unsigned long long tile_waves = (unsigned long long)g.B * (unsigned)g.ntiles * (unsigned)g.G;
    if (tile_waves > 0xFFFF0000ull) { err = "batch too large: more than 2^32 tiles x channel groups; split the batch"; return ST_EINVAL; }
    if ((st = ensure_as(be, WS_DENSE_LIST, (size_t)tile_waves * sizeof(unsigned), W.dense_list, set))) return st;
    const int tier = choose_tier(P.lds_tier, be.feedback_host());
    if (L.topo()) W.cls_table = const_cast<unsigned*>(P.topo->table);
    if (L.split_exact_fixup) {
        if ((st = ensure_as(be, WS_REDO_LIST, (size_t)(REDO_HEAD + (size_t)REDO_CAP * REDO_ENTRY) * sizeof(unsigned), W.redo_list, set))) return st;
        if ((st = be.launch(k_zero_words, dim3(1), dim3(WAVE), W.redo_list, (unsigned)REDO_HEAD))) return st;
    }
    be.hot_begin(L.flavour, g.K, ECAP_TIER[tier]);
    st = g.K == 8 ? launch_tiles<8>(be, tier, P, L, g, W) : launch_tiles<4>(be, tier, P, L, g, W);
    be.hot_end();
    const bool tail_ran = L.dense_wgs + L.fix_waves != 0u;
    if (!st) {
        CounterState& cs = *W.cs;
        cs.clean = W.clean_after;
        cs.wclean = true;
        cs.tptr = L.topo() ? W.table_before : W.cls_table;
        if (L.solo()) cs.dclean = W.direct_bytes;
        if (tail_ran) cs.parity ^= 1u;
    }
    const bool tail_mirrors = !st && !g.force_general && be.feedback_dev() != nullptr;
    be.note_error_flag_mirrored(tail_mirrors && L.dense_wgs != 0u);
    be.note_tail_reports(tail_mirrors && tail_ran && P.seq != 0u);
    be.tile_done(set);
    return st;
}

template <class BE>
int run_topology_build(BE& be, const void* d_sigmas, int sigmas_f64, long long n, int C, double voxelsize, uint2* cw, unsigned* ids,
                       unsigned* table, int* flags , unsigned* wide_list , std::string& err)
{
    if (n <= 0 || C <= 0) { err = "a topology needs n_atoms > 0 and n_channels > 0"; return ST_EINVAL; }
    if (!(voxelsize > 0.0) || !std::isfinite(voxelsize)) { err = "voxelsize must be a positive finite number"; return ST_EINVAL; }
    const int G = ceil_div(C, CHG);
    const double w_scale = voxelsize * voxelsize, R = CUTOFF_A / voxelsize;
    const float w_exact_max = (float)(7.647 / (R * R));
    const unsigned nblk = (unsigned)ceil_div(n, 256), nl1 = (unsigned)ceil_div(nblk, CLS_ROWS_PER_BLOCK);
    unsigned *bsets = nullptr, *l1sets = nullptr;
    int st;
    if ((st = ensure_as(be, WS_CLS_BLOCKS, (size_t)nblk * CLS_BLOCK_SET * sizeof(unsigned), bsets, 0))) return st;
    if ((st = ensure_as(be, WS_CLS_L1, (size_t)nl1 * MERGE_SET * sizeof(unsigned), l1sets, 0))) return st;
    return with_sigmas(d_sigmas, sigmas_f64, [&](auto* sig) {
        using S = sigma_of<decltype(sig)>;
        int s;
        if ((s = be.launch(k_topology_classes<S>, dim3(nblk), dim3(256), sig, n, C, G, w_scale, cw, bsets))) return s;
        if ((s = be.launch(k_merge_classes, dim3(nl1), dim3(256), bsets, nblk, (unsigned)CLS_BLOCK_SET, CLS_ROWS_PER_BLOCK, l1sets, (unsigned*)nullptr))) return s;
        if ((s = be.launch(k_merge_classes, dim3(1), dim3(256), l1sets, nl1, (unsigned)MERGE_SET, nl1, (unsigned*)nullptr, table))) return s;
        return be.launch(k_topology_ids<S>, dim3(nblk), dim3(256), sig, cw, table, n, C, G, w_scale, w_exact_max, ids, flags, wide_list);
    });
}

template <class BE>
int run_centers(BE& be, const double* d_centers, long long V, const float* d_coords, long long N,
                const void* d_sigmas, int sigmas_f64, int C, const double* box_host, float* d_out,
                std::string& err)
{
    if (V < 0 || N < 0 || C <= 0) { err = "n_centers/n_atoms must be >= 0 and n_channels > 0"; return ST_EINVAL; }
    if (V == 0) return ST_OK;
    if (box_host)
        for (int ax = 0; ax < 3; ++ax)
            if (!(box_host[ax] > 2.0 * CUTOFF_A)) { err = "periodic box edges must be > 10 A (2 x cutoff)"; return ST_EBOX; }
    const int G = ceil_div(C, CHG);
    float4* w = nullptr;
    int st = ensure_as(be, WS_W_EXPLICIT, (size_t)(N > 0 ? N : 1) * sizeof(float4) * 2 * G, w, 0);
    if (st) return st;
    if (N > 0) {
        st = with_sigmas(d_sigmas, sigmas_f64, [&](auto* sig) {
            return be.launch(k_sigma_to_w<sigma_of<decltype(sig)>>, dim3((unsigned)ceil_div(N, 256)), dim3(256), sig, N, C, G, 1.0, w);
        });
        if (st) return st;
    }
    const long long wgs = ceil_div(V, EXPL_CENTERS) * G;
    int waves = 4;
    while (waves < EXPL_MAX_WAVES && wgs * waves < 4096) waves *= 2;
// ... 74 lines not shown
```

### moleculekit_amd/distributed.py

```python
from __future__ import annotations

import os

import numpy as np


P2P_MAX_BYTES = 1 << 30


def world(group=None):
    try:
        import torch.distributed as dist

        if dist.is_available() and dist.is_initialized():
            return dist.get_rank(group), dist.get_world_size(group)
    except Exception:
        pass
    return int(os.environ.get("RANK", "0")), int(os.environ.get("WORLD_SIZE", "1"))


def shard_bounds(n_items: int, world_size: int, weights=None):
    if world_size <= 0:
        raise ValueError("world_size must be positive")
    if weights is None:
# ... 42 lines not shown
        if all(int(s) == bmax for s in sizes):
            return full
        parts = [full[r * bmax: r * bmax + int(sizes[r])] for r in range(ws)]
        return torch.cat(parts, dim=0)
    recv = [torch.empty_like(padded) for _ in range(ws)] if rank == dst else None
    dist.gather(padded, recv, dst=dst, group=group)
    if rank != dst:
        return None
    return torch.cat([recv[r][: int(sizes[r])] for r in range(ws)], dim=0)


class ShardedVoxelizer:

    def __init__(self, n_items, bounds, shard, nvoxels, voxelsize, device=None, compute=None, group=None, ctx=None,
                 pipelined=True, shared_sigmas=False):
        import torch


        self.pipelined = bool(pipelined)
        self.group = group
        self.rank, self.world = world(group)
        self.n_items = int(n_items)
        self.bounds = np.asarray(bounds, dtype=np.int64)
        self.lo, self.hi = int(self.bounds[self.rank]), int(self.bounds[self.rank + 1])
        self.nvoxels = np.ascontiguousarray(nvoxels, dtype=np.int32).reshape(3)
        self.V = int(np.prod(self.nvoxels.astype(np.int64)))
        self.voxelsize = float(voxelsize)
        self._compute = compute
        self._ctx = ctx
        coords, offs, sigmas, origins, box = shard
        self.n_local = int(len(offs) - 1)
        assert self.n_local == self.hi - self.lo, "the shard does not match this rank's bounds"
        self.C = int(np.asarray(sigmas).shape[1]) if np.asarray(sigmas).ndim == 2 else 0
        self._offs_host = np.ascontiguousarray(offs, dtype=np.int64)
        self.max_images = 1
        if compute is None:
            if device is None:
                device = torch.device("cuda", int(os.environ.get("LOCAL_RANK", self.rank)) % max(torch.cuda.device_count(), 1))
            self.device = torch.device(device)
            if self.device.type != "cuda":
                raise RuntimeError("ShardedVoxelizer needs a HIP device (there is no CPU path); tests inject `compute`")
            if box is not None and len(box):
                from . import batch
                self.max_images = batch.max_images_per_atom(box, self.nvoxels, self.voxelsize)
        else:
            self.device = torch.device("cpu" if device is None else device)
        sig = np.asarray(sigmas)
        sig_dt = np.float64 if sig.dtype == np.float64 else np.float32
        self._topo = None
        self._shared = False
        if shared_sigmas and self.n_local > 0:
            sizes = np.diff(self._offs_host)
            n0 = int(sizes[0])
            if n0 > 0 and np.all(sizes == n0):
                if sig.shape[0] == n0 * self.n_local:
                    rows = sig.reshape(self.n_local, n0, -1)
                    if not all(np.array_equal(rows[0], r) for r in rows[1:]):
                        raise ValueError("shared_sigmas: the items' sigma rows differ (not frames of one molecule)")
                    sig = np.ascontiguousarray(rows[0])
                elif sig.shape[0] != n0:
                    raise ValueError("shared_sigmas: pass the molecule's [n, C] matrix or its repeat per item")
                if compute is None:
                    self._shared = True
                else:
                    sig = np.tile(sig, (self.n_local, 1))
            else:
                raise ValueError("shared_sigmas: every item must have the molecule's atom count")
        self._d = self._upload(dict(coords=(coords, np.float32), offs=(self._offs_host, np.int64), sigmas=(sig, sig_dt),
                                    origins=(np.asarray(origins, dtype=np.float64).reshape(-1, 3), np.float64),
                                    box=(box, np.float32)))
        self._chunk_offs = {}
        if self._shared:
            from . import _lib
            tctx = self._ctx or _lib.default_context(self.device.index if self.device.index is not None else 0)
            if not getattr(tctx, "_force_general", False) and not getattr(tctx, "_value_tol", 0.0):
                torch.cuda.current_stream(self.device).synchronize()
                try:
                    self._topo = _lib.Topology(tctx, self._d["sigmas"], self.voxelsize)
                except ValueError:
                    self._topo = None
            if self._topo is None:
                self._d["sigmas"] = self._d["sigmas"].repeat(self.n_local, 1).contiguous()
                self._shared = False

    @classmethod
    def from_host(cls, coords, atom_offsets, sigmas, origins, nvoxels, voxelsize, box=None, balance_by_atoms=True, **kw):
        rank, ws = world(kw.get("group"))
        atom_offsets = np.asarray(atom_offsets)
        B = len(atom_offsets) - 1
        weights = np.diff(atom_offsets) + 1.0 if balance_by_atoms else None
        bounds = shard_bounds(B, ws, weights)
        shard = shard_packed(np.asarray(coords), atom_offsets, np.asarray(sigmas),
                             np.asarray(origins, dtype=np.float64).reshape(-1, 3),
                             None if box is None else np.asarray(box), int(bounds[rank]), int(bounds[rank + 1]))
        return cls(B, bounds, shard, nvoxels, voxelsize, **kw)

    @classmethod
    def from_loader(cls, n_items, loader, nvoxels, voxelsize, weights=None, **kw):
        rank, ws = world(kw.get("group"))
        bounds = shard_bounds(int(n_items), ws, weights)
        return cls(n_items, bounds, tuple(loader(int(bounds[rank]), int(bounds[rank + 1]))), nvoxels, voxelsize, **kw)

    def _upload(self, arrays):
        import torch

        out = {}
        if self.device.type != "cuda":
            for k, (a, dt) in arrays.items():
                out[k] = None if a is None else torch.from_numpy(np.ascontiguousarray(a, dtype=dt))
            return out
        copy = torch.cuda.Stream(device=self.device)
        keep = []
        with torch.cuda.stream(copy):
            for k, (a, dt) in arrays.items():
                if a is None:
                    out[k] = None
                    continue
                a = np.asarray(a)
                pinned = torch.empty(a.shape, dtype=getattr(torch, np.dtype(dt).name), pin_memory=True)
                np.copyto(pinned.numpy(), a, casting="same_kind")
                out[k] = pinned.to(self.device, non_blocking=True)
                keep.append(pinned)
        ev = torch.cuda.Event()
        ev.record(copy)
        torch.cuda.current_stream(self.device).wait_event(ev)
        for t in out.values():
            if t is not None:
                t.record_stream(torch.cuda.current_stream(self.device))
        copy.synchronize()
        return out

    def _run(self, coords, offs, sigmas, origins, box, out=None):
        if self._compute is not None:
            t = lambda x: None if x is None else x.numpy()
            res = self._compute(t(coords), t(offs), t(sigmas), t(origins), self.nvoxels, self.voxelsize, t(box))
            if out is not None:
                out.copy_(res)
                return out
            return res
        from . import _lib, batch

        ctx = self._ctx or _lib.default_context(self.device.index if self.device.index is not None else 0)
        if self.pipelined:
            ctx.promise_inputs(None)
        return batch.voxelize_lattice_torch(coords, offs, None if self._topo is not None else sigmas, origins, self.nvoxels, self.voxelsize,
                                            box=box, max_images=self.max_images, out=out, ctx=ctx, topology=self._topo)

    def _items(self, lo, hi):
        import torch

        d = self._d
        a0, a1 = int(self._offs_host[lo]), int(self._offs_host[hi])
        if (lo, hi) == (0, self.n_local):
            offs = d["offs"]
        else:
            offs = self._chunk_offs.get((lo, hi))
            if offs is None:
                offs = torch.as_tensor(self._offs_host[lo:hi + 1] - a0, device=self.device)
                self._chunk_offs[(lo, hi)] = offs
        sig = d["sigmas"] if self._shared else d["sigmas"][a0:a1]
        return d["coords"][a0:a1], offs, sig, d["origins"][lo:hi], None if d["box"] is None else d["box"][lo:hi]

    def voxelize(self, out=None):
        return self._run(*self._items(0, self.n_local), out=out)

    def _collectives(self):
        try:
            import torch.distributed as dist
            return dist.is_available() and dist.is_initialized()
        except Exception:
            return False

    def gather(self, local, dst=None):
        return gather_features(local, self.bounds, group=self.group, dst=dst) if self._collectives() else local

    def voxelize_gather(self, nchunks=4, dst=None, timings=None, exchange="auto", loopback=False):
        import torch
        import torch.distributed as dist

        if not self._collectives():
            return self.voxelize()
        ws, rank = self.world, self.rank
        sizes = np.diff(self.bounds)
        if exchange == "auto":
            exchange = "p2p" if dst is None else "allgather"
        if exchange == "p2p" and dst is not None:
            raise ValueError("the point-to-point exchange is an all-gather (dst=None)")
        self.last_exchange = exchange
        cb = [chunk_bounds(int(s), nchunks) for s in sizes]
        tail = (self.V, self.C)
        cuda = self.device.type == "cuda"
        comm = torch.cuda.Stream(device=self.device) if cuda else None
        main = torch.cuda.current_stream(self.device) if cuda else None

        if exchange == "p2p":
            full = torch.empty((self.n_items,) + tail, dtype=torch.float32, device=self.device)
            row = lambda r, c: int(self.bounds[r] + cb[r][c])
            rows_per_msg = max(1, P2P_MAX_BYTES // max(1, self.V * self.C * 4))

            def pieces(r0, r1):
                return [(a, min(a + rows_per_msg, r1)) for a in range(r0, r1, rows_per_msg)]
            for c in range(len(cb[rank]) - 1):
                lo, hi = int(cb[rank][c]), int(cb[rank][c + 1])
                if hi > lo:
                    self._run(*self._items(lo, hi), out=full[row(rank, c):row(rank, c + 1)])
                if ws == 1 and not loopback:
                    continue
                ev = None
                if cuda:
                    ev = torch.cuda.Event()
                    ev.record(main)
                with (torch.cuda.stream(comm) if cuda else _null()):
                    if cuda:
                        comm.wait_event(ev)
                    ops, check = [], None
                    for k in range(1, ws):
                        to, frm = (rank + k) % ws, (rank - k) % ws
                        if hi > lo:
                            for a, b in pieces(row(rank, c), row(rank, c + 1)):
                                ops.append(dist.P2POp(dist.isend, full[a:b], self._global_rank(to), group=self.group))
                        if cb[frm][c + 1] > cb[frm][c]:
                            for a, b in pieces(row(frm, c), row(frm, c + 1)):
                                ops.append(dist.P2POp(dist.irecv, full[a:b], self._global_rank(frm), group=self.group))
                    if ws == 1 and hi > lo:
                        check = torch.empty_like(full[row(rank, c):row(rank, c + 1)])
                        ops = []
                        for a, b in pieces(row(rank, c), row(rank, c + 1)):
                            ops.append(dist.P2POp(dist.isend, full[a:b], self._global_rank(rank), group=self.group))
                            ops.append(dist.P2POp(dist.irecv, check[a - row(rank, c):b - row(rank, c)], self._global_rank(rank), group=self.group))
                    if ops:
                        for req in dist.batch_isend_irecv(ops):
                            req.wait()
                    if check is not None and not torch.equal(check, full[row(rank, c):row(rank, c + 1)]):
                        raise RuntimeError("loopback exchange returned different data")
            if cuda:
                main.wait_stream(comm)
                full.record_stream(comm)
            return full

        want = dst is None or rank == dst
        full = torch.empty((self.n_items,) + tail, dtype=torch.float32, device=self.device) if want else None
        local = torch.empty((self.n_local,) + tail, dtype=torch.float32, device=self.device)
        for c in range(len(cb[rank]) - 1):
            lo, hi = int(cb[rank][c]), int(cb[rank][c + 1])
# ... 234 lines not shown
```

Before: 253,400 Mvoxel-channels/s.

## Add batch topologies that precompute sigma class tables for heterogeneous item batches

Adds a batch topology that precomputes per-atom sigma class/weight tables over a whole batch of differently sized items, with per-item offsets and a sorted wide-atom list. The distributed voxelizer builds it by default (env MKAMD_BATCH_TOPOLOGY) when items are not repeats of one molecule and a probe reports the topology path would be used. Calls then take the class-sorted topology path for a range of items, slicing the precomputed tables. This avoids re-deriving sigma classes each call, in exchange for setup cost, extra device memory, and more path-selection complexity.

```diff
diff --git a/include/mkamd_voxel.h b/include/mkamd_voxel.h
--- a/include/mkamd_voxel.h
+++ b/include/mkamd_voxel.h
@@ -108,6 +108,17 @@
                                     int64_t total_atoms, const mkamd_topology* topology, const double* d_origins,
                                     const int32_t* nvoxels, double voxelsize, const float* d_box, int32_t max_images_per_atom,
                                     const double* d_affine, float* d_features);
+int mkamd_topology_create_batch_dev(mkamd_ctx* ctx, const void* d_sigmas, int sigmas_are_f64, int64_t total_atoms, int32_t n_channels,
+                                    double voxelsize, const int64_t* atom_offsets_host, int32_t n_items, mkamd_topology** topology);
+int mkamd_topology_create_batch_host(mkamd_ctx* ctx, const void* sigmas, int sigmas_are_f64, int64_t total_atoms, int32_t n_channels,
+                                     double voxelsize, const int64_t* atom_offsets_host, int32_t n_items, mkamd_topology** topology);
+int mkamd_topology_batch_info(const mkamd_topology* topology, int32_t* n_items, int64_t* longest_item);
+int mkamd_topology_batch_used(mkamd_ctx* ctx, const mkamd_topology* topology, int32_t first_item, int32_t n_items, const int32_t* nvoxels,
+                              int32_t periodic, int32_t max_images_per_atom, int32_t promised, int32_t* used);
+int mkamd_voxelize_lattice_topo_range_dev(mkamd_ctx* ctx, int32_t n_items, const float* d_coords, const int64_t* d_atom_offsets,
+                                          int64_t total_atoms, const mkamd_topology* topology, int32_t first_item, const double* d_origins,
+                                          const int32_t* nvoxels, double voxelsize, const float* d_box, int32_t max_images_per_atom,
+                                          const double* d_affine, float* d_features);
 
 int mkamd_grid_centers_host(mkamd_ctx* ctx, const double* bb_min, const int32_t* nvoxels,
                             double voxelsize, double* centers);
diff --git a/moleculekit_amd/_lib.py b/moleculekit_amd/_lib.py
--- a/moleculekit_amd/_lib.py
+++ b/moleculekit_amd/_lib.py
@@ -74,6 +74,11 @@
     "mkamd_topology_destroy": (_c_int, [_vp, _vp]),
     "mkamd_topology_info": (_c_int, [_vp, ctypes.POINTER(_c_i64), ctypes.POINTER(_c_i32), ctypes.POINTER(_c_dbl), ctypes.POINTER(_c_i32)]),
     "mkamd_voxelize_lattice_topo_dev": (_c_int, [_vp, _c_i32, _vp, _vp, _c_i64, _vp, _vp, _vp, _c_dbl, _vp, _c_i32, _vp, _vp]),
+    "mkamd_topology_create_batch_dev": (_c_int, [_vp, _vp, _c_int, _c_i64, _c_i32, _c_dbl, _vp, _c_i32, ctypes.POINTER(_vp)]),
+    "mkamd_topology_create_batch_host": (_c_int, [_vp, _vp, _c_int, _c_i64, _c_i32, _c_dbl, _vp, _c_i32, ctypes.POINTER(_vp)]),
+    "mkamd_topology_batch_info": (_c_int, [_vp, ctypes.POINTER(_c_i32), ctypes.POINTER(_c_i64)]),
+    "mkamd_topology_batch_used": (_c_int, [_vp, _vp, _c_i32, _c_i32, _vp, _c_i32, _c_i32, _c_i32, ctypes.POINTER(_c_i32)]),
+    "mkamd_voxelize_lattice_topo_range_dev": (_c_int, [_vp, _c_i32, _vp, _vp, _c_i64, _vp, _c_i32, _vp, _vp, _c_dbl, _vp, _c_i32, _vp, _vp]),
     "mkamd_grid_centers_host": (_c_int, [_vp, _vp, _vp, _c_dbl, _vp]),
     "mkamd_grid_centers_dev": (_c_int, [_vp, _vp, _vp, _c_dbl, _vp]),
     "mkamd_lattice_from_centers": (_c_int, [_vp, ctypes.c_int64, _vp, _vp, _vp]),
@@ -375,7 +380,14 @@
                                                      _ptr(d_out)))
 
     def voxelize_lattice_topo_dev(self, B, d_coords, d_offsets, total_atoms, topology, d_origins, nvox, voxelsize, d_box, max_images, d_out,
-                                  d_affine=None):
+                                  d_affine=None, first_item=0):
+        if topology.n_items:
+            _check(load().mkamd_voxelize_lattice_topo_range_dev(self._h, B, _ptr(d_coords), _ptr(d_offsets), int(total_atoms), topology._h,
+                                                                int(first_item), _ptr(d_origins), _ptr(nvox), float(voxelsize), _ptr(d_box),
+                                                                int(max_images), _ptr(d_affine), _ptr(d_out)))
+            return
+        if first_item:
+            raise ValueError("first_item names a range of a BATCH topology's items")
         _check(load().mkamd_voxelize_lattice_topo_dev(self._h, B, _ptr(d_coords), _ptr(d_offsets), int(total_atoms), topology._h,
                                                       _ptr(d_origins), _ptr(nvox), float(voxelsize), _ptr(d_box), int(max_images),
                                                       _ptr(d_affine), _ptr(d_out)))
@@ -442,29 +454,46 @@
 
 class Topology:
 
-    def __init__(self, ctx, sigmas, voxelsize):
+    def __init__(self, ctx, sigmas, voxelsize, atom_offsets=None):
         self._h = _vp(None)
         self._ctx = ctx
+        self.n_items = 0
         h = _vp(None)
+        offs = None
+        if atom_offsets is not None:
+            offs = np.ascontiguousarray(atom_offsets, dtype=np.int64).reshape(-1)
+            if offs.size < 2:
+                raise ValueError("a batch topology needs at least one item")
+        batch_args = () if offs is None else (_ptr(offs), int(offs.size - 1))
         if isinstance(sigmas, np.ndarray) or not hasattr(sigmas, "data_ptr"):
             sig = np.ascontiguousarray(sigmas)
             if sig.dtype not in (np.float32, np.float64):
                 sig = sig.astype(np.float64)
             if sig.ndim != 2:
                 raise ValueError("sigmas must be (natoms, nchannels)")
-            _check(load().mkamd_topology_create_host(ctx._h, _ptr(sig), int(sig.dtype == np.float64), int(sig.shape[0]), int(sig.shape[1]),
-                                                     float(voxelsize), ctypes.byref(h)))
+            create = load().mkamd_topology_create_host if offs is None else load().mkamd_topology_create_batch_host
+            _check(create(ctx._h, _ptr(sig), int(sig.dtype == np.float64), int(sig.shape[0]), int(sig.shape[1]),
+                          float(voxelsize), *batch_args, ctypes.byref(h)))
             self.n_atoms, self.n_channels = int(sig.shape[0]), int(sig.shape[1])
         else:
             import torch
             if not (sigmas.is_cuda and sigmas.dim() == 2 and sigmas.is_contiguous() and sigmas.dtype in (torch.float32, torch.float64)):
                 raise ValueError("sigmas must be a contiguous float32 / float64 CUDA tensor (natoms, nchannels)")
             ctx.set_stream(torch.cuda.current_stream(sigmas.device).cuda_stream)
-            _check(load().mkamd_topology_create_dev(ctx._h, int(sigmas.data_ptr()), int(sigmas.dtype == torch.float64), int(sigmas.shape[0]),
-                                                    int(sigmas.shape[1]), float(voxelsize), ctypes.byref(h)))
+            create = load().mkamd_topology_create_dev if offs is None else load().mkamd_topology_create_batch_dev
+            _check(create(ctx._h, int(sigmas.data_ptr()), int(sigmas.dtype == torch.float64), int(sigmas.shape[0]),
+                          int(sigmas.shape[1]), float(voxelsize), *batch_args, ctypes.byref(h)))
             self.n_atoms, self.n_channels = int(sigmas.shape[0]), int(sigmas.shape[1])
         self._h = h
         self.voxelsize = float(voxelsize)
+        self.n_items = 0 if offs is None else int(offs.size - 1)
+
+    def used_for(self, first_item, n_items, nvoxels, periodic=False, max_images=1, promised=False) -> bool:
+        nv = np.ascontiguousarray(nvoxels, dtype=np.int32).reshape(3)
+        u = _c_i32(0)
+        _check(load().mkamd_topology_batch_used(self._ctx._h, self._h, int(first_item), int(n_items), _ptr(nv), int(bool(periodic)),
+                                                int(max_images), int(bool(promised)), ctypes.byref(u)))
+        return bool(u.value)
 
     @property
     def has_wide_sigmas(self) -> bool:
diff --git a/moleculekit_amd/batch.py b/moleculekit_amd/batch.py
--- a/moleculekit_amd/batch.py
+++ b/moleculekit_amd/batch.py
@@ -147,7 +147,7 @@
 
 
 def voxelize_lattice_torch(coords, atom_offsets, sigmas, origins, nvoxels, voxelsize, box=None,
-                           max_images=1, out=None, ctx=None, channel_first=False, affine=None, topology=None):
+                           max_images=1, out=None, ctx=None, channel_first=False, affine=None, topology=None, topology_first_item=0):
     import torch
 
     dev = coords.device
@@ -185,7 +185,7 @@
         ctx.set_stream(torch.cuda.current_stream(dev).cuda_stream)
         if topology is not None:
             ctx.voxelize_lattice_topo_dev(B, coords.data_ptr(), atom_offsets.data_ptr(), int(coords.shape[0]), topology, origins.data_ptr(), nv,
-                                          float(voxelsize), d_box, int(max_images), out.data_ptr(), d_aff)
+                                          float(voxelsize), d_box, int(max_images), out.data_ptr(), d_aff, first_item=int(topology_first_item))
         else:
             ctx.voxelize_lattice_dev(B, coords.data_ptr(), atom_offsets.data_ptr(), int(coords.shape[0]),
                                      sigmas.data_ptr(), sigmas.dtype == torch.float64, C, origins.data_ptr(), nv,
diff --git a/moleculekit_amd/csrc/capi.hip b/moleculekit_amd/csrc/capi.hip
--- a/moleculekit_amd/csrc/capi.hip
+++ b/moleculekit_amd/csrc/capi.hip
@@ -273,6 +273,8 @@
     int device = 0;
     void* mem = nullptr;
     mkamd::TopologyDev dev;
+    std::vector<long long> h_offsets;
+    std::vector<unsigned> h_wide;
 };
 
 static int check_ctx(mkamd_ctx* ctx, bool pending_ok = false)
@@ -293,7 +295,7 @@
     HIP_TRY(hipMemcpy(&flag, ctx->bufs[WS_ERR], sizeof(int), hipMemcpyDeviceToHost));
     if (flag == 0) return 0;
     HIP_TRY(hipMemset(ctx->bufs[WS_ERR], 0, sizeof(int)));
-    if (flag & MK_ERR_TOPOLOGY) return fail(MKAMD_EINVAL, "a topology call was given an item that is not the topology's atom count long; results are incomplete");
+    if (flag & MK_ERR_TOPOLOGY) return fail(MKAMD_EINVAL, "a topology call was given an item that is not the topology's atom count long (a batch topology: not the atoms of its item); results are incomplete");
     if (flag & MK_ERR_BAD_BOX) return fail(MKAMD_EBOX, "periodic box edges must be > 10 A (2 x cutoff)");
     if (flag & MK_ERR_TOO_MANY_IMAGES) return fail(MKAMD_EBOX, "periodic box much smaller than the grid (too many images)");
     return fail(MKAMD_EOVERFLOW, "more periodic images than max_images_per_atom allowed; results are incomplete");
@@ -811,7 +813,8 @@
                                      const int64_t* d_atom_offsets, int64_t total_atoms, const void* d_sigmas,
                                      int sigmas_are_f64, int32_t C, const double* d_origins,
                                      const int32_t* nvoxels, double voxelsize, const float* d_box,
-                                     int32_t max_images, const double* d_affine, float* d_features, const mkamd_topology* topo)
+                                     int32_t max_images, const double* d_affine, float* d_features, const mkamd_topology* topo,
+                                     int32_t topo_first_item = 0)
 {
     int st = check_ctx(ctx);
     if (st) return st;
@@ -828,6 +831,7 @@
     P.coords = d_coords; P.atom_offsets = (const long long*)d_atom_offsets; P.sigmas = d_sigmas;
     P.origins = d_origins; P.box = d_box; P.affine = d_affine; P.out = d_features;
     P.topo = topo ? &topo->dev : nullptr;
+    P.topo_first_item = topo_first_item;
     std::string err;
     st = run_lattice(*ctx, P, err);
     ctx->promise = false; ctx->promise_event = nullptr;
@@ -845,20 +849,30 @@
                                      d_box, max_images, d_affine, d_features, nullptr);
 } MK_API_CATCH
 
-int mkamd_topology_create_dev(mkamd_ctx* ctx, const void* d_sigmas, int sigmas_are_f64, int64_t n_atoms, int32_t C, double voxelsize,
-                              mkamd_topology** out)
-try {
+static int topology_create_impl(mkamd_ctx* ctx, const void* d_sigmas, int sigmas_are_f64, int64_t n_atoms, int32_t C, double voxelsize,
+                                const int64_t* h_offsets, int32_t n_items, mkamd_topology** out)
+{
     if (!out) return fail(MKAMD_EINVAL, "topology out-pointer is NULL");
     *out = nullptr;
     int st = check_ctx(ctx);
     if (st) return st;
     if (n_atoms <= 0 || C <= 0 || !d_sigmas) return fail(MKAMD_EINVAL, "a topology needs n_atoms > 0, n_channels > 0 and the sigmas");
     if (n_atoms > 0x7fffffffLL) return fail(MKAMD_EINVAL, "a topology holds at most 2^31 atoms");
+    long long max_item = 0;
+    if (h_offsets) {
+        if (n_items <= 0 || h_offsets[0] != 0 || h_offsets[n_items] != n_atoms)
+            return fail(MKAMD_EINVAL, "a batch topology needs n_items > 0 and atom offsets that start at 0 and end at total_atoms");
+        for (int32_t b = 0; b < n_items; ++b) {
+            if (h_offsets[b + 1] < h_offsets[b]) return fail(MKAMD_EINVAL, "a batch topology's atom offsets must not decrease");
+            max_item = std::max<long long>(max_item, h_offsets[b + 1] - h_offsets[b]);
+        }
+    }
     const int G = ceil_div(C, CHG);
     const size_t a256 = 255, sig_bytes = (size_t)n_atoms * C * (sigmas_are_f64 ? 8 : 4);
     const size_t o_cw = (sig_bytes + a256) & ~a256, o_ids = (o_cw + (size_t)n_atoms * G * sizeof(uint2) + a256) & ~a256,
                  o_tab = (o_ids + (size_t)n_atoms * G * sizeof(unsigned) + a256) & ~a256, o_flags = o_tab + 256, o_wide = o_flags + 256,
-                 total = o_wide + (size_t)n_atoms * sizeof(unsigned);
+                 o_offs = (o_wide + (size_t)n_atoms * sizeof(unsigned) + a256) & ~a256,
+                 total = o_offs + (h_offsets ? (size_t)n_items + 1 : 0) * sizeof(long long);
     mkamd_topology* t = new mkamd_topology();
     t->device = ctx->device;
     hipError_t e = hipMalloc(&t->mem, total);
@@ -878,8 +892,9 @@
         (e = hipStreamSynchronize(ctx->stream)) != hipSuccess) return drop(hip_fail(e, "topology read-back"));
     const int flags = flags2[0];
     const unsigned n_wide = (unsigned)flags2[1];
-    if (n_wide > 1u) {
-        std::vector<unsigned> wl(n_wide);
+    std::vector<unsigned>& wl = t->h_wide;
+    wl.resize(n_wide);
+    if (n_wide > 1u || (n_wide != 0u && h_offsets)) {
         if ((e = hipMemcpyAsync(wl.data(), m + o_wide, (size_t)n_wide * 4, hipMemcpyDeviceToHost, ctx->stream)) != hipSuccess ||
             (e = hipStreamSynchronize(ctx->stream)) != hipSuccess) return drop(hip_fail(e, "topology read-back (wide atoms)"));
         std::sort(wl.begin(), wl.end());
@@ -892,8 +907,43 @@
     t->dev.sigmas = m; t->dev.cw = (const uint2*)(m + o_cw); t->dev.ids = (const unsigned*)(m + o_ids); t->dev.table = (const unsigned*)(m + o_tab);
     t->dev.overflow = false; t->dev.wide = (flags & 1) != 0;
     t->dev.wide_list = (const unsigned*)(m + o_wide); t->dev.n_wide = n_wide;
+    if (h_offsets) {
+        t->h_offsets.assign(h_offsets, h_offsets + n_items + 1);
+        if ((e = hipMemcpyAsync(m + o_offs, t->h_offsets.data(), ((size_t)n_items + 1) * sizeof(long long), hipMemcpyHostToDevice, ctx->stream)) != hipSuccess ||
+            (e = hipStreamSynchronize(ctx->stream)) != hipSuccess) return drop(hip_fail(e, "topology upload (atom offsets)"));
+        t->dev.batch = true; t->dev.n_items = n_items; t->dev.max_item = max_item;
+        t->dev.offsets = (const long long*)(m + o_offs); t->dev.h_offsets = t->h_offsets.data(); t->dev.h_wide_list = t->h_wide.data();
+    }
     *out = t;
     return MKAMD_OK;
+}
+
+int mkamd_topology_create_dev(mkamd_ctx* ctx, const void* d_sigmas, int sigmas_are_f64, int64_t n_atoms, int32_t C, double voxelsize,
+                              mkamd_topology** out)
+try {
+    return topology_create_impl(ctx, d_sigmas, sigmas_are_f64, n_atoms, C, voxelsize, nullptr, 0, out);
+} MK_API_CATCH
+
+int mkamd_topology_create_batch_dev(mkamd_ctx* ctx, const void* d_sigmas, int sigmas_are_f64, int64_t total_atoms, int32_t C, double voxelsize,
+                                    const int64_t* atom_offsets_host, int32_t n_items, mkamd_topology** out)
+try {
+    if (!atom_offsets_host) { if (out) *out = nullptr; return fail(MKAMD_EINVAL, "a batch topology needs the batch's atom offsets (host memory)"); }
+    return topology_create_impl(ctx, d_sigmas, sigmas_are_f64, total_atoms, C, voxelsize, atom_offsets_host, n_items, out);
+} MK_API_CATCH
+
+int mkamd_topology_create_batch_host(mkamd_ctx* ctx, const void* sigmas, int sigmas_are_f64, int64_t total_atoms, int32_t C, double voxelsize,
+                                     const int64_t* atom_offsets_host, int32_t n_items, mkamd_topology** out)
+try {
+    if (!out) return fail(MKAMD_EINVAL, "topology out-pointer is NULL");
+    *out = nullptr;
+    int st = check_ctx(ctx);
+    if (st) return st;
+    if (total_atoms <= 0 || C <= 0 || !sigmas) return fail(MKAMD_EINVAL, "a topology needs n_atoms > 0, n_channels > 0 and the sigmas");
+    void* ds = nullptr;
+    const size_t bytes = (size_t)total_atoms * C * (sigmas_are_f64 ? 8 : 4);
+    if ((st = ctx->ensure(WS_H_SIGMAS, bytes, &ds))) return st;
+    HIP_TRY(hipMemcpyAsync(ds, sigmas, bytes, hipMemcpyHostToDevice, ctx->stream));
+    return mkamd_topology_create_batch_dev(ctx, ds, sigmas_are_f64, total_atoms, C, voxelsize, atom_offsets_host, n_items, out);
 } MK_API_CATCH
 
 int mkamd_topology_create_host(mkamd_ctx* ctx, const void* sigmas, int sigmas_are_f64, int64_t n_atoms, int32_t C, double voxelsize,
@@ -944,6 +994,50 @@
     if (!topo) return fail(MKAMD_EINVAL, "topology is NULL");
     return voxelize_lattice_dev_impl(ctx, B, d_coords, d_atom_offsets, total_atoms, nullptr, topo->dev.sigmas_f64, topo->dev.C, d_origins, nvoxels,
                                      voxelsize, d_box, max_images, d_affine, d_features, topo);
+} MK_API_CATCH
+
+int mkamd_voxelize_lattice_topo_range_dev(mkamd_ctx* ctx, int32_t B, const float* d_coords, const int64_t* d_atom_offsets, int64_t total_atoms,
+                                          const mkamd_topology* topo, int32_t first_item, const double* d_origins, const int32_t* nvoxels,
+                                          double voxelsize, const float* d_box, int32_t max_images, const double* d_affine, float* d_features)
+try {
+    if (!topo) return fail(MKAMD_EINVAL, "topology is NULL");
+    if (!topo->dev.batch) return fail(MKAMD_EINVAL, "a range of items is a call on a batch topology (mkamd_topology_create_batch_*)");
+    return voxelize_lattice_dev_impl(ctx, B, d_coords, d_atom_offsets, total_atoms, nullptr, topo->dev.sigmas_f64, topo->dev.C, d_origins, nvoxels,
+                                     voxelsize, d_box, max_images, d_affine, d_features, topo, first_item);
+} MK_API_CATCH
+
+int mkamd_topology_batch_info(const mkamd_topology* topo, int32_t* n_items, int64_t* longest_item)
+try {
+    if (!topo) return fail(MKAMD_EINVAL, "topology is NULL");
+    if (n_items) *n_items = topo->dev.batch ? topo->dev.n_items : 0;
+    if (longest_item) *longest_item = topo->dev.batch ? (int64_t)topo->dev.max_item : 0;
+    return MKAMD_OK;
+} MK_API_CATCH
+
+int mkamd_topology_batch_used(mkamd_ctx* ctx, const mkamd_topology* topo, int32_t first_item, int32_t n_items, const int32_t* nvoxels,
+                              int32_t periodic, int32_t max_images, int32_t promised, int32_t* used)
+try {
+    if (!ctx || !topo || !nvoxels || !used) return fail(MKAMD_EINVAL, "ctx / topology / nvoxels / used is NULL");
+    *used = 0;
+    const TopologyDev& t = topo->dev;
+    if (!t.batch) return fail(MKAMD_EINVAL, "not a batch topology");
+    if (first_item < 0 || n_items < 0 || (long long)first_item + n_items > (long long)t.n_items) return fail(MKAMD_EINVAL, "not a range of the batch topology's items");
+    LatticeProblem P;
+    P.B = n_items; P.total_atoms = t.h_offsets[first_item + n_items] - t.h_offsets[first_item]; P.C = t.C; P.sigmas_f64 = t.sigmas_f64;
+    P.nvox[0] = nvoxels[0]; P.nvox[1] = nvoxels[1]; P.nvox[2] = nvoxels[2];
+    P.voxelsize = t.voxelsize; P.pbc = periodic ? 1 : 0; P.max_images = periodic ? max_images : 1;
+    P.tile_k = ctx->tile_k; P.force_general = ctx->force_general; P.lds_tier = ctx->lds_tier; P.prepass_mode = ctx->prepass_mode; P.tile_team = ctx->tile_team; P.tile_items = ctx->tile_items; P.exact_redo_list = ctx->exact_redo; P.fine_cells = ctx->fine_cells; P.value_tol = ctx->value_tol; P.direct = ctx->direct;
+    P.topo = &t; P.topo_first_item = first_item;
+    GridDesc g;
+    std::string err;
+    int st = plan_lattice(P, g, err);
+    if (st) return fail(st, err);
+    if (P.B == 0 || g.V == 0 || P.total_atoms == 0 || g.force_general || g.reach_tau > 0.f) return MKAMD_OK;
+    const bool may_pipeline = (ctx->pipelining || promised) && ctx->side_stream && !ctx->pipeline_broken;
+    LatticePath L = choose_lattice_path(P, g, may_pipeline);
+    settle_lattice_path(L, P, g, may_pipeline && L.pipelined_wanted);
+    *used = L.topo() ? 1 : 0;
+    return MKAMD_OK;
 } MK_API_CATCH
 
 static hipError_t wait_for_small_call(hipStream_t s, hipEvent_t done = nullptr)
diff --git a/moleculekit_amd/csrc/kernels.h b/moleculekit_amd/csrc/kernels.h
--- a/moleculekit_amd/csrc/kernels.h
+++ b/moleculekit_amd/csrc/kernels.h
@@ -57,7 +57,13 @@
     int cnt_shift;
     long long topo_n;
     unsigned topo_wide;
+    const long long* topo_offsets;
+    long long topo_base;
 };
+MK_DEV bool topo_batch_item_ok(const GridDesc& g, const long long* __restrict__ atom_offsets, int b)
+{
+    return g.topo_offsets[b] == g.topo_base + atom_offsets[b] && g.topo_offsets[b + 1] == g.topo_base + atom_offsets[b + 1];
+}
 enum { DIRECT_FAILED = 0, DIRECT_SPILLED = 1, DIRECT_WORDS = 4, DIRECT_HEAD = 32  };
 constexpr float REACH_STEP = 0.17f;
 
@@ -309,10 +315,11 @@
             }
             b = lo;
             const long long first = atom_offsets[b];
-            if (atom_offsets[b + 1] - first != g.topo_n) {
+            const bool batch = g.topo_offsets != nullptr;
+            if (batch ? !topo_batch_item_ok(g, atom_offsets, b) : atom_offsets[b + 1] - first != g.topo_n) {
                 mk_atomic_or(err_flag, MK_ERR_TOPOLOGY);
             } else {
-                const unsigned* __restrict__ ids = reinterpret_cast<const unsigned*>(sigmas) + (size_t)(a - first) * g.G;
+                const unsigned* __restrict__ ids = reinterpret_cast<const unsigned*>(sigmas) + (size_t)(batch ? a : a - first) * g.G;
                 unsigned* __restrict__ park_ids = reinterpret_cast<unsigned*>(tmp_cls) + (size_t)a * g.G;
                 for (int gq = 0; gq < g.G; ++gq) {
                     const unsigned v = ids[gq];
@@ -2265,7 +2272,7 @@
     if (g.pbc) { L[0] = (double)box[3 * (size_t)b]; L[1] = (double)box[3 * (size_t)b + 1]; L[2] = (double)box[3 * (size_t)b + 2]; }
     const long long a_lo = atom_offsets[b], a_end = atom_offsets[b + 1];
     const long long a_hi = a_end - a_lo > s_hi ? a_lo + s_hi : a_end;
-    const long long sshift = g.topo_n ? a_lo : 0;
+    const long long sshift = (g.topo_n && g.topo_offsets == nullptr) ? a_lo : 0;
     const float fcx = (float)cx, fcy = (float)cy, fcz = (float)cz;
     const float fL[3] = {(float)L[0], (float)L[1], (float)L[2]};
     const float fiL[3] = {1.0f / fL[0], 1.0f / fL[1], 1.0f / fL[2]};
@@ -2466,6 +2473,15 @@
     const int lane = threadIdx.x;
     const float wmax = g.w_exact_max;
     auto wide_bits = [&](unsigned bits) { return bits != CLS_EMPTY && mk_uint_as_float(bits) < wmax; };
+    if (per_item == 2 && g.topo_offsets != nullptr) {
+        const long long a = (long long)summary[blk] - g.topo_base;
+        if (a < 0 || a >= total_atoms) return;
+        const int b = item_of_atom(atom_offsets, g.B, a, 0);
+        if (!topo_batch_item_ok(g, atom_offsets, b)) return;
+        exact_fixup_atom<SigT, LIST_ONLY>(g, b, a, a, coords, atom_offsets, sigmas, origins, box, affine, out, s_best, s_near, feedback, seq,
+                                          redo_list, redo_cap);
+        return;
+    }
     if (per_item == 2) {
         const int b = (int)(blk / g.topo_wide);
         const long long k = (long long)summary[blk % g.topo_wide];
@@ -2597,6 +2613,7 @@
     for (unsigned long long job = blockIdx.x; job < jobs; job += gridDim.x) {
         const unsigned* e = redo_list + REDO_HEAD + (size_t)(job / slices) * REDO_ENTRY;
         const long long s_lo = (long long)(job % slices) * REDO_SLICE;
+        if (g.topo_offsets != nullptr && s_lo >= atom_offsets[e[0] + 1] - atom_offsets[e[0]]) continue;
         const unsigned long long chs = (unsigned long long)e[4] | ((unsigned long long)e[5] << 32);
         exact_recompute<SigT>(g, (int)e[0], (int)e[1], (int)e[2], (int)e[3], chs, (int)e[6], coords, atom_offsets, sigmas, origins, box, affine, out,
                               s_best, s_near, s_lo, s_lo + REDO_SLICE, true);
diff --git a/moleculekit_amd/csrc/pipeline.h b/moleculekit_amd/csrc/pipeline.h
--- a/moleculekit_amd/csrc/pipeline.h
+++ b/moleculekit_amd/csrc/pipeline.h
@@ -39,6 +39,12 @@
     bool wide = false;
     const unsigned* wide_list = nullptr;
     unsigned n_wide = 0;
+    bool batch = false;
+    int n_items = 0;
+    const long long* offsets = nullptr;
+    const long long* h_offsets = nullptr;
+    const unsigned* h_wide_list = nullptr;
+    long long max_item = 0;
 };
 
 struct LatticeProblem {
@@ -71,6 +77,7 @@
     const double* affine = nullptr;
     float* out = nullptr;
     const TopologyDev* topo = nullptr;
+    int topo_first_item = 0;
 };
 
 inline int ceil_div(long long a, long long b) { return (int)((a + b - 1) / b); }
@@ -219,10 +226,19 @@
     bool per_item() const { return prepass == PRE_ITEMS; }
 };
 
+inline void choose_exact_fixup(LatticePath& L, const LatticeProblem& P, const GridDesc& g)
+{
+    const bool topo = L.topo();
+    const unsigned topo_jobs = !topo ? 0u : P.topo->batch ? g.topo_wide : (unsigned)((long long)g.B * P.topo->n_wide);
+    L.fix_jobs = topo ? topo_jobs : L.per_item() ? (unsigned)g.B : P.total_atoms > 0 ? (unsigned)ceil_div(P.total_atoms, 256) : 0u;
+    L.fix_waves = L.fix_jobs < 8192u ? L.fix_jobs : 8192u;
+    L.split_exact_fixup = topo && topo_jobs != 0u && P.seq == 0u && !g.force_general && P.exact_redo_list >= 0;
+}
+
 inline LatticePath choose_lattice_path(const LatticeProblem& P, const GridDesc& g, bool pipelining_possible)
 {
     LatticePath L;
-    const bool topo = P.topo != nullptr;
+    const bool topo = P.topo != nullptr && !P.topo->batch, topo_batch = P.topo != nullptr && P.topo->batch;
     const long long B = g.B;
     const bool big = P.total_atoms >= PIPELINE_MIN_ATOMS;
     const bool chain_pays = pipelining_possible && big && P.total_atoms > 1024LL * B;
@@ -245,14 +261,13 @@
                       (P.direct == 2 || (P.direct != 0 && P.prepass_mode < 0 && L.team && !(L.ligand_items && P.tile_team <= 0 && hist_fits)));
     const bool per_item = !topo && !solo && hist_fits && P.prepass_mode != 0 &&
                           (P.prepass_mode == 1 || (P.total_atoms <= 4096LL * B && !chain_pays));
-    L.prepass = topo ? LatticePath::PRE_CHAIN_TOPO : solo ? LatticePath::PRE_SOLO : per_item ? LatticePath::PRE_ITEMS : LatticePath::PRE_CHAIN;
+    L.prepass = topo ? LatticePath::PRE_CHAIN_TOPO : solo ? LatticePath::PRE_SOLO : per_item ? LatticePath::PRE_ITEMS
+              : topo_batch ? LatticePath::PRE_CHAIN_TOPO : LatticePath::PRE_CHAIN;
     L.pipelined_wanted = big && !per_item && !solo;
     L.spill = solo ? (unsigned)P.total_atoms : P.spill_cap > 0 ? P.spill_cap : (unsigned)std::max<long long>(1024, P.total_atoms / (8LL * B));
     L.direct_slots = (unsigned long long)((size_t)g.B * (size_t)g.cstride) * (unsigned)L.direct_cap + (unsigned long long)L.spill * (unsigned)g.B;
-    L.fix_jobs = topo ? (unsigned)(B * P.topo->n_wide) : per_item ? (unsigned)g.B : P.total_atoms > 0 ? (unsigned)ceil_div(P.total_atoms, 256) : 0u;
-    L.fix_waves = L.fix_jobs < 8192u ? L.fix_jobs : 8192u;
+    choose_exact_fixup(L, P, g);
     L.dense_wgs = g.force_general ? 0u : (unsigned)(tile_waves < 4096ull ? tile_waves : 4096ull);
-    L.split_exact_fixup = topo && P.topo->n_wide != 0u && P.seq == 0u && !g.force_general && P.exact_redo_list >= 0;
     L.redo_cap = P.exact_redo_list > 0 && (unsigned)P.exact_redo_list < REDO_CAP ? (unsigned)P.exact_redo_list : REDO_CAP;
     return L;
 }
@@ -260,10 +275,12 @@
 inline void settle_lattice_path(LatticePath& L, const LatticeProblem& P, GridDesc& g, bool set_is_pipelined)
 {
     g.prepass_hurry = !(set_is_pipelined && !g.pbc && (double)g.B * (double)g.V >= 4.0 * (double)P.total_atoms) ? 1 : 0;
-    const bool direct_big = L.prepass == LatticePath::PRE_CHAIN && L.direct_geom &&
+    const bool chain_or_batch = L.prepass == LatticePath::PRE_CHAIN || (L.topo() && P.topo->batch);
+    const bool direct_big = chain_or_batch && L.direct_geom &&
                             (P.direct == 1 || (P.direct < 0 && !set_is_pipelined && P.total_atoms >= PIPELINE_MIN_ATOMS));
     L.direct_layout = (L.solo() || direct_big) && L.direct_slots <= 0xFFFF0000ull;
     L.direct_first = L.direct_layout && !L.solo();
+    if (L.direct_first && L.topo()) { L.prepass = LatticePath::PRE_CHAIN; choose_exact_fixup(L, P, g); }
     L.small_scan = !L.direct_layout && (size_t)g.B * (size_t)g.cstride <= SMALL_PREPASS_MAX_CELLS &&
                    (unsigned)ceil_div(P.total_atoms > 0 ? P.total_atoms : 1, 256) <= SMALL_PREPASS_MAX_BLOCKS;
     L.flavour = L.team ? TILES_TEAM : (set_is_pipelined ? TILES_LEAN : TILES_PLAIN);
@@ -490,28 +507,57 @@
 }
 
 template <class BE>
-int run_lattice(BE& be, const LatticeProblem& P, std::string& err)
-{
+int run_lattice(BE& be, const LatticeProblem& P_in, std::string& err)
+{
+    LatticeProblem P = P_in;
     GridDesc g;
     int st = plan_lattice(P, g, err);
     if (st) return st;
     if (P.B == 0 || g.V == 0) return ST_OK;
+    size_t topo_wide_lo = 0;
     if (const TopologyDev* t = P.topo) {
         if (t->overflow || g.force_general || g.reach_tau > 0.f) {
             err = "a topology call takes the class-sorted path only: not with more than 15 distinct sigmas, force_general or a value tolerance (use the plain entry point)";
             return ST_EINVAL;
         }
-        if (t->C != P.C || t->voxelsize != P.voxelsize || t->n <= 0 || P.total_atoms != (long long)P.B * t->n) {
+        if (t->C != P.C || t->voxelsize != P.voxelsize || t->n <= 0 || (!t->batch && P.total_atoms != (long long)P.B * t->n)) {
             err = "the topology was built for another channel count / voxel size, or the call is not n_items x its atom count long";
             return ST_EINVAL;
         }
-        if ((unsigned long long)g.B * t->n_wide > 0xffffffffull) { err = "too many (item, wide atom) fix-up jobs (>= 2^32): split the batch"; return ST_EINVAL; }
-        g.topo_n = t->n; g.topo_wide = t->n_wide;
+        if (t->batch) {
+            const long long i0 = P.topo_first_item;
+            if (i0 < 0 || i0 + P.B > (long long)t->n_items || P.total_atoms != t->h_offsets[i0 + P.B] - t->h_offsets[i0]) {
+                err = "the call is not a range of the batch topology's items: first item + n_items beyond its items, or another atom count";
+                return ST_EINVAL;
+            }
+            g.topo_base = t->h_offsets[i0]; g.topo_offsets = t->offsets + i0; g.topo_n = t->max_item;
+            const unsigned* w0 = std::lower_bound(t->h_wide_list, t->h_wide_list + t->n_wide, (unsigned)g.topo_base);
+            const unsigned* w1 = std::lower_bound(w0, t->h_wide_list + t->n_wide, (unsigned)(g.topo_base + P.total_atoms));
+            topo_wide_lo = (size_t)(w0 - t->h_wide_list); g.topo_wide = (unsigned)(w1 - w0);
+        } else {
+            if ((unsigned long long)g.B * t->n_wide > 0xffffffffull) { err = "too many (item, wide atom) fix-up jobs (>= 2^32): split the batch"; return ST_EINVAL; }
+            g.topo_n = t->n; g.topo_wide = t->n_wide;
+        }
     }
     LatticePath L = choose_lattice_path(P, g, be.pipelining_possible());
     g.cls_per_item = L.per_item() ? 1 : 0;
     const int set = be.acquire_set(L.pipelined_wanted);
     settle_lattice_path(L, P, g, be.set_is_pipelined(set));
+    TopologyDev range;
+    if (P.topo != nullptr && P.topo->batch) {
+        const TopologyDev* t = P.topo;
+        const size_t a0 = (size_t)g.topo_base;
+        const void* sig0 = (const char*)t->sigmas + a0 * (size_t)t->C * (t->sigmas_f64 ? 8 : 4);
+        if (L.topo()) {
+            range = *t;
+            range.ids = t->ids + a0 * (size_t)t->G; range.cw = t->cw + a0 * (size_t)t->G; range.sigmas = sig0;
+            range.wide_list = t->wide_list + topo_wide_lo;
+            P.topo = &range;
+        } else {
+            P.topo = nullptr; P.sigmas = sig0; P.sigmas_f64 = t->sigmas_f64;
+            g.topo_n = 0; g.topo_wide = 0u; g.topo_offsets = nullptr; g.topo_base = 0;
+        }
+    }
     if (L.solo() && !L.direct_layout) { err = "internal: the one-launch pre-pass does not fit its record slots"; return ST_EINVAL; }
 
     LatticeWorkspace W;
diff --git a/moleculekit_amd/distributed.py b/moleculekit_amd/distributed.py
--- a/moleculekit_amd/distributed.py
+++ b/moleculekit_amd/distributed.py
@@ -148,6 +148,29 @@
             if self._topo is None:
                 self._d["sigmas"] = self._d["sigmas"].repeat(self.n_local, 1).contiguous()
                 self._shared = False
+        elif (compute is None and self.n_local > 0 and int(self._offs_host[-1]) > 0 and os.environ.get("MKAMD_BATCH_TOPOLOGY", "1") != "0"
+              and not self._items_repeat_one_molecule(sig)):
+            from . import _lib
+            tctx = self._ctx or _lib.default_context(self.device.index if self.device.index is not None else 0)
+            if not getattr(tctx, "_force_general", False) and not getattr(tctx, "_value_tol", 0.0):
+                torch.cuda.current_stream(self.device).synchronize()
+                try:
+                    topo = _lib.Topology(tctx, self._d["sigmas"], self.voxelsize, atom_offsets=self._offs_host)
+                    if topo.used_for(0, self.n_local, self.nvoxels, periodic=self._d["box"] is not None, max_images=self.max_images,
+                                     promised=self.pipelined):
+                        self._topo = topo
+                    else:
+                        topo.close()
+                except ValueError:
+                    self._topo = None
+
+    def _items_repeat_one_molecule(self, sig):
+        sizes = np.diff(self._offs_host)
+        n0 = int(sizes[0])
+        if self.n_local < 2 or n0 <= 0 or not np.all(sizes == n0) or sig.ndim != 2 or sig.shape[0] != n0 * self.n_local:
+            return False
+        rows = sig.reshape(self.n_local, n0, -1)
+        return all(np.array_equal(rows[0], r) for r in rows[1:])
 
     @classmethod
     def from_host(cls, coords, atom_offsets, sigmas, origins, nvoxels, voxelsize, box=None, balance_by_atoms=True, **kw):
@@ -196,7 +219,7 @@
         copy.synchronize()
         return out
 
-    def _run(self, coords, offs, sigmas, origins, box, out=None):
+    def _run(self, coords, offs, sigmas, origins, box, first_item=0, out=None):
         if self._compute is not None:
             t = lambda x: None if x is None else x.numpy()
             res = self._compute(t(coords), t(offs), t(sigmas), t(origins), self.nvoxels, self.voxelsize, t(box))
@@ -210,7 +233,8 @@
         if self.pipelined:
             ctx.promise_inputs(None)
         return batch.voxelize_lattice_torch(coords, offs, None if self._topo is not None else sigmas, origins, self.nvoxels, self.voxelsize,
-                                            box=box, max_images=self.max_images, out=out, ctx=ctx, topology=self._topo)
+                                            box=box, max_images=self.max_images, out=out, ctx=ctx, topology=self._topo,
+                                            topology_first_item=first_item if self._topo is not None and self._topo.n_items else 0)
 
     def _items(self, lo, hi):
         import torch
@@ -225,7 +249,7 @@
                 offs = torch.as_tensor(self._offs_host[lo:hi + 1] - a0, device=self.device)
                 self._chunk_offs[(lo, hi)] = offs
         sig = d["sigmas"] if self._shared else d["sigmas"][a0:a1]
-        return d["coords"][a0:a1], offs, sig, d["origins"][lo:hi], None if d["box"] is None else d["box"][lo:hi]
+        return d["coords"][a0:a1], offs, sig, d["origins"][lo:hi], None if d["box"] is None else d["box"][lo:hi], lo
 
     def voxelize(self, out=None):
         return self._run(*self._items(0, self.n_local), out=out)
```

Measured after the change: 265,600 Mvoxel-channels/s (median of 6 runs). +4.8%, better.
